# PantoMatrix/PantoMatrix

Hardware: NVIDIA H100
Metric: motion_frames_per_sec (higher is better)
Workload: dtype fp16x3 (two fp16 operand planes, 3 products, f32 accumulate)

## Files before the change

### include/pm_emage.h

```cpp
#ifndef PM_EMAGE_H
#define PM_EMAGE_H
#include <stdint.h>
#ifdef __cplusplus
extern "C" {
#endif

#define PM_ABI_VERSION 6
#define PM_FMT_F16 0x100
#define PM_TC_TILE_SHIFT 16
#define PM_TC_STORE_LOOP (1 << 24)
int pm_abi_version(void);
int pm_memset_async(void* ptr, int value, long long bytes, void* stream);
int pm_device_cc(void);

int pm_tapgemm_f32(const float* A, long long a_bs, int lda, int batch, int rows_in, int cin,
                   const float* W, const float* bias, int taps, int stride, int pad,
                   int rows_out, int cout,
                   const float* residual, long long r_bs, int ldr,
                   int act, float slope,
                   float* out, long long o_bs, int ldo, void* stream);

int pm_tapgemm_tc(const uint16_t* A, long long a_ps, long long a_bs, int lda, int batch, int rows_in, int cin,
                  const uint16_t* W, long long w_ps, int w_rows, int ldw, int taps, int pad, int nsplit,
                  const float* bias, int rows_out, int cout,
                  const float* residual, long long r_bs, int ldr,
                  int act, int act_cols, float slope, float acc_scale,
                  float* out_f32, long long o_bs, int ldo,
                  uint16_t* out_bf16, long long ob_ps, long long ob_bs, int ldob, int out_nsplit,
                  const void* prefetch, long long prefetch_bytes, void* stream);

int pm_split_bf16(const float* x, long long x_bs, int ldx, int batch, int rows, int ch,
                  uint16_t* out, long long o_ps, long long o_bs, int ldo, int nsplit, void* stream);

int pm_wav_stem_f32(const float* audio, long long a_bs, long long a_ws, int batch, int windows, int n_samples,
                    const float* w1, const float* b1, const float* wd, const float* bd, int cout,
                    int ksize, int stride, int pad, int rows_out, float slope,
                    float* y1, float* sc,
                    uint16_t* planes, long long p_ps, int p_ld, int p_nsplit, void* stream);

int pm_add_layernorm_f32(const float* x, const float* r, const float* gamma, const float* beta,
                         float* out, long long rows, int ch, float eps,
                         uint16_t* planes, long long p_ps, int p_ld, int p_nsplit, void* stream);

int pm_attention_f32(const float* Q, int ldq, const float* K, int ldk, const float* V, int ldv,
                     float* O, int ldo, int batch, int heads, int tq, int tk, int head_dim,
                     uint16_t* planes, long long p_ps, int p_ld, int p_nsplit, void* stream);

int pm_attention_tc(const uint16_t* Q, long long q_ps, long long q_bs, int ldq, int q_cols, int q_col0,
                    const uint16_t* K, long long k_ps, long long k_bs, int ldk, int k_cols, int k_col0,
                    const uint16_t* V, long long v_ps, long long v_bs, int ldv, int v_cols, int v_col0,
                    float* O, int ldo, int batch, int heads, int tq, int tk, int head_dim,
                    uint16_t* planes, long long p_ps, int p_ld, int p_nsplit, void* stream);

int pm_add_rows_f32(const float* x, const float* pe, const float* spk, int first, int second,
                    float* out, int batch, int rows, int ch,
                    uint16_t* planes, long long p_ps, int p_ld, int p_nsplit, void* stream);
int pm_add2_f32(const float* a, long long lda, const float* b, long long ldb, float* out, long long ldo,
                long long rows, long long ch,
                uint16_t* planes, long long p_ps, int p_ld, int p_nsplit, void* stream);

int pm_window_input_f32(const float* motion, const float* mask, const float* seed, const float* mask_embedding,
                        float* out, int batch, int total_len, int start, int win_len, int pre, int ch, long long seed_bs,
                        uint16_t* planes, long long p_ps, int p_ld, int p_nsplit, void* stream);

int pm_l2_argmin_f32(const float* z, long long rows, int rows_per_batch, long long z_bs,
                     const float* codebook, const float* e2, int n_codes, int e_dim, long long* index, void* stream);
int pm_l2_argmin_tc(const float* z, long long rows, int rows_per_batch, long long z_bs,
                    const float* codebook, const float* e2, int n_codes, int e_dim, long long* index, int max_ctas,
                    void* stream);
int pm_l2_argmin_simt_f32(const float* z, long long rows, int rows_per_batch, long long z_bs,
                          const float* codebook, const float* e2, int n_codes, int e_dim, long long* index, void* stream);
int pm_row_argmax_f32(const float* x, long long rows, int ch, int ldx, int rows_per_batch, long long x_bs,
                      long long* index, int* nonfinite, void* stream);
int pm_gather_rows_f32(const float* codebook, long long n_table, const long long* index, long long rows, int ch,
                       float* out, uint16_t* planes, long long p_ps, int p_ld, int p_nsplit, void* stream);
int pm_row_sqnorm_f32(const float* x, int rows, int ch, float* out, void* stream);

int pm_pose_compose_f32(const float* face, const float* upper, const float* hands, const float* lower,
                        float* expression, float* axis_angle, float* motion4inf, long long bt, void* stream);

int pm_global_trans_f32(const float* rec, int ld, int vel_off, const float* ref_trans, int ref_bs, float dt,
                        float* trans, int batch, int t, void* stream);

int pm_resample_poly_f32(const void* pcm, int is_int16, long long in_bs, int batch, long long n_in, int channels,
                         const float* bank, int up, int down, int taps, long long n_pre_remove,
                         float* out, long long out_bs, void* stream);

int pm_lstm_bidir_f32(const float* xproj, long long x_bs, int ldx, const float* whh,
                      float* y, long long y_bs, int ldy, unsigned int* barrier,
                      int batch, int t, int hidden, void* stream);
int pm_lstm_cond_f32(const float* spk, long long n_spk, int spk_dim, const long long* speaker_id,
                     const float* seed, long long seed_bs, int seed_ld, int seed_len, int seed_frames, int pose_dims,
                     float* out, long long o_bs, int ldo, int batch, int t, void* stream);
int pm_rot6d_to_aa_f32(const float* rot6d, long long rows, int n_sel, const int* slot, float* out, void* stream);
int pm_softmax2_mix_f32(const float* sel, const float* c1, const float* c2, float* out, long long rows, int ch, int ldo,
                        void* stream);

int pm_smplx_fk_f32(const float* poses, long long pose_bs, long long pose_ts,
                    const float* betas, long long b_bs,
                    const float* expr, long long e_bs, long long e_ts,
                    const float* transl, long long t_bs, long long t_ts,
                    long long joint_mask, int batch, int t,
                    const float* j_template, const float* j_dirs, const float* pose_mean,
                    const int* parents, const int* level_order, const int* level_start, int n_levels,
                    float* joints, float* rel_transforms, float* feat, int ld_feat,
                    uint16_t* planes, long long p_ps, int p_ld, int p_nsplit, void* stream);
int pm_smplx_skin_f32(float* verts, long long ld, long long rows, int n_verts,
                      const int* row_ptr, const int* col, const float* val, const float* rel_transforms,
                      const float* transl, long long t_bs, long long t_ts, int t, void* stream);
int pm_motion_rep_f32(const float* poses, long long pose_bs, long long pose_ts, const float* joints,
                      int batch, int t, float dt, float two_dt, float* rep15d, void* stream);

int pm_mesh_vertex_f32(const float* verts0, long long v0_fs, const float* verts1, long long v1_fs,
                       int n_verts, int frames, float scale0, float ox0, float oy0, float oz0,
                       float scale1, float ox1, float oy1, float oz1, const int* faces,
                       const int* vf_ptr, const int* vf_face, int* xy, float* depth, float* normal,
                       int views, void* stream);
int pm_mesh_raster(const int* xy, const float* depth, int n_verts, const int* faces, int n_faces,
                   int frames, unsigned long long* vis, int views, void* stream);
int pm_mesh_shade_u8(const unsigned long long* vis, const int* xy, const float* normal, int n_verts,
                     const int* faces, int frames, unsigned char* out, long long out_fs, int views, void* stream);
int pm_time_upsample_f32(const float* x, long long x_bs, long long x_ts, int batch, int t, int channels, int k,
                         float* out, void* stream);

int pm_png_count(const unsigned char* frames, long long f_fs, int n_frames, int h, int w, long long* row_bits,
                 unsigned long long* row_adler, void* stream);
int pm_png_scan(int n_frames, int h, int w, long long* row_bits, const unsigned long long* row_adler,
                unsigned char* data, long long cap, long long* nbytes, void* stream);
int pm_png_emit(const unsigned char* frames, long long f_fs, int n_frames, int h, int w, const long long* row_off,
                unsigned char* data, long long cap, void* stream);
int pm_png_crc(int n_frames, int h, int w, unsigned char* data, long long cap, const long long* nbytes, void* stream);

int pm_h264_encode(const unsigned char* frames, long long f_fs, int n_frames, int clip_len, int h, int w, int qp,
                   unsigned char* scratch, long long slice_cap, int* slice_bytes, void* stream);
int pm_h264_encode_gop(const unsigned char* frames, long long f_fs, int n_frames, int clip_len, int h, int w, int qp,
                       unsigned char* scratch, long long slice_cap, int* slice_bytes, int gop, unsigned char* recon,
                       long long recon_stride, void* stream);
int pm_h264_encode_me(const unsigned char* frames, long long f_fs, int n_frames, int clip_len, int h, int w, int qp,
                      unsigned char* scratch, long long slice_cap, int* slice_bytes, int gop, unsigned char* recon,
                      long long recon_stride, int search, short* mv, long long mv_len, void* stream);
int pm_h264_gather(int n_frames, int h, int w, const unsigned char* scratch, long long slice_cap,
                   const int* slice_bytes, unsigned char* data, long long cap, long long* nbytes, void* stream);

int pm_flac_analyse(const void* pcm, long long clip_stride, int batch, int n, int channels, int bps, int* rec,
                    void* stream);
int pm_flac_emit(const void* pcm, long long clip_stride, int batch, int n, int channels, int bps, int rate,
                 const int* rec, unsigned char* data, long long cap, long long* nbytes, void* stream);

#ifdef __cplusplus
}
#endif
#endif
```

### pantomatrix_b200/_lib.py

```python
from __future__ import annotations

import ctypes as C
import os

_HERE = os.path.dirname(os.path.abspath(__file__))
LIB_PATH = os.environ.get("PM_EMAGE_LIB") or os.path.join(_HERE, "libpm_emage.so")

_p = C.c_void_p
_i = C.c_int
_ll = C.c_longlong
_f = C.c_float

SIGNATURES = {
    "pm_abi_version": [],
    "pm_device_cc": [],
    "pm_tapgemm_f32": [_p, _ll, _i, _i, _i, _i, _p, _p, _i, _i, _i, _i, _i, _p, _ll, _i, _i, _f, _p, _ll, _i, _p],
    "pm_tapgemm_tc": [_p, _ll, _ll, _i, _i, _i, _i, _p, _ll, _i, _i, _i, _i, _i, _p, _i, _i, _p, _ll, _i,
                      _i, _i, _f, _f, _p, _ll, _i, _p, _ll, _ll, _i, _i, _p, _ll, _p],
    "pm_split_bf16": [_p, _ll, _i, _i, _i, _i, _p, _ll, _ll, _i, _i, _p],
    "pm_wav_stem_f32": [_p, _ll, _ll, _i, _i, _i, _p, _p, _p, _p, _i, _i, _i, _i, _i, _f, _p, _p, _p, _ll, _i, _i, _p],
    "pm_add_layernorm_f32": [_p, _p, _p, _p, _p, _ll, _i, _f, _p, _ll, _i, _i, _p],
    "pm_attention_f32": [_p, _i, _p, _i, _p, _i, _p, _i, _i, _i, _i, _i, _i, _p, _ll, _i, _i, _p],
    "pm_attention_tc": [_p, _ll, _ll, _i, _i, _i, _p, _ll, _ll, _i, _i, _i, _p, _ll, _ll, _i, _i, _i,
                        _p, _i, _i, _i, _i, _i, _i, _p, _ll, _i, _i, _p],
    "pm_add_rows_f32": [_p, _p, _p, _i, _i, _p, _i, _i, _i, _p, _ll, _i, _i, _p],
    "pm_add2_f32": [_p, _ll, _p, _ll, _p, _ll, _ll, _ll, _p, _ll, _i, _i, _p],
    "pm_window_input_f32": [_p, _p, _p, _p, _p, _i, _i, _i, _i, _i, _i, _ll, _p, _ll, _i, _i, _p],
    "pm_l2_argmin_f32": [_p, _ll, _i, _ll, _p, _p, _i, _i, _p, _p],
    "pm_row_argmax_f32": [_p, _ll, _i, _i, _i, _ll, _p, _p, _p],
    "pm_l2_argmin_tc": [_p, _ll, _i, _ll, _p, _p, _i, _i, _p, _i, _p],
    "pm_l2_argmin_simt_f32": [_p, _ll, _i, _ll, _p, _p, _i, _i, _p, _p],
    "pm_memset_async": [_p, _i, _ll, _p],
    "pm_gather_rows_f32": [_p, _ll, _p, _ll, _i, _p, _p, _ll, _i, _i, _p],
    "pm_row_sqnorm_f32": [_p, _i, _i, _p, _p],
    "pm_pose_compose_f32": [_p, _p, _p, _p, _p, _p, _p, _ll, _p],
    "pm_global_trans_f32": [_p, _i, _i, _p, _i, _f, _p, _i, _i, _p],
    "pm_lstm_bidir_f32": [_p, _ll, _i, _p, _p, _ll, _i, _p, _i, _i, _i, _p],
    "pm_lstm_cond_f32": [_p, _ll, _i, _p, _p, _ll, _i, _i, _i, _i, _p, _ll, _i, _i, _i, _p],
    "pm_rot6d_to_aa_f32": [_p, _ll, _i, _p, _p, _p],
    "pm_softmax2_mix_f32": [_p, _p, _p, _p, _ll, _i, _i, _p],
    "pm_resample_poly_f32": [_p, _i, _ll, _i, _ll, _i, _p, _i, _i, _i, _ll, _p, _ll, _p],
    "pm_smplx_fk_f32": [_p, _ll, _ll, _p, _ll, _p, _ll, _ll, _p, _ll, _ll, _ll, _i, _i, _p, _p, _p, _p, _p, _p, _i,
                        _p, _p, _p, _i, _p, _ll, _i, _i, _p],
    "pm_smplx_skin_f32": [_p, _ll, _ll, _i, _p, _p, _p, _p, _p, _ll, _ll, _i, _p],
    "pm_motion_rep_f32": [_p, _ll, _ll, _p, _i, _i, _f, _f, _p, _p],
    "pm_mesh_vertex_f32": [_p, _ll, _p, _ll, _i, _i, _f, _f, _f, _f, _f, _f, _f, _f, _p, _p, _p, _p, _p, _p, _i, _p],
    "pm_mesh_raster": [_p, _p, _i, _p, _i, _i, _p, _i, _p],
    "pm_mesh_shade_u8": [_p, _p, _p, _i, _p, _i, _p, _ll, _i, _p],
    "pm_time_upsample_f32": [_p, _ll, _ll, _i, _i, _i, _i, _p, _p],
    "pm_png_count": [_p, _ll, _i, _i, _i, _p, _p, _p],
    "pm_png_scan": [_i, _i, _i, _p, _p, _p, _ll, _p, _p],
    "pm_png_emit": [_p, _ll, _i, _i, _i, _p, _p, _ll, _p],
    "pm_png_crc": [_i, _i, _i, _p, _ll, _p, _p],
    "pm_h264_encode": [_p, _ll, _i, _i, _i, _i, _i, _p, _ll, _p, _p],
    "pm_h264_encode_gop": [_p, _ll, _i, _i, _i, _i, _i, _p, _ll, _p, _i, _p, _ll, _p],
    "pm_h264_encode_me": [_p, _ll, _i, _i, _i, _i, _i, _p, _ll, _p, _i, _p, _ll, _i, _p, _ll, _p],
    "pm_h264_gather": [_i, _i, _i, _p, _ll, _p, _p, _ll, _p, _p],
    "pm_flac_analyse": [_p, _ll, _i, _i, _i, _i, _p, _p],
    "pm_flac_emit": [_p, _ll, _i, _i, _i, _i, _i, _p, _p, _ll, _p, _p],
}

_lib = None


class PmError(RuntimeError):
    pass


def load() -> C.CDLL:
    global _lib
    if _lib is None:
        if not os.path.exists(LIB_PATH):
            raise PmError(
                f"{LIB_PATH} not found: build it with `python -m pantomatrix_b200.build` "
                "(there is no CPU or PyTorch fallback for the EMAGE hot path)")
        lib = C.CDLL(LIB_PATH)
        for name, args in SIGNATURES.items():
            fn = getattr(lib, name)
            fn.argtypes = args
            fn.restype = C.c_int
        _lib = lib
    return _lib


def call(name: str, *args) -> None:
    rc = getattr(load(), name)(*args)
    if rc != 0:
        kind = "bad argument / unsupported shape" if rc < 0 else "cudaError"
        raise PmError(f"{name} failed: {kind} {rc}")
```

### pantomatrix_b200/csrc/pm_attention_tc.cu

```cuda
#include "pm_common.cuh"
#include "pm_tc_ptx.cuh"
#include "../../include/pm_emage.h"

namespace {

constexpr int T = 64;
constexpr int HD = 192;
constexpr int KB = HD / 64;
constexpr int BLK = T * 128;
constexpr int NTHREADS = 128;
constexpr float P_SCALE = 1024.f;

struct Smem {
  static constexpr int Q = 0;
  static constexpr int K = Q + 2 * KB * BLK;
  static constexpr int V = K + 2 * KB * BLK;
  static constexpr int P = V + 2 * KB * BLK;
  static constexpr int BARS = P + 2 * BLK;
  static constexpr int TOTAL = BARS + (KB + 1) * 8;
};

#ifdef PM_ATTN_TIMING
__device__ unsigned long long pm_attn_stamps[16];
#define AT_STAMP(i) do { if (blockIdx.x == 0 && (threadIdx.x & 31) == 0) pm_attn_stamps[i] = (unsigned long long)clock64(); } while (0)
#else
#define AT_STAMP(i) do {} while (0)
#endif

struct AttnParams {
  int heads, tq, tk;
  int qc0, kc0, vc0;
  float scale;
  float* out; int ldo;
  PmPlanes planes;
};

__global__ void __launch_bounds__(NTHREADS, 1) attention_tc_kernel(const __grid_constant__ CUtensorMap map_q,
                                                                   const __grid_constant__ CUtensorMap map_k,
                                                                   const __grid_constant__ CUtensorMap map_v,
                                                                   const AttnParams p) {
  extern __shared__ __align__(1024) uint8_t smem_raw[];
  uint8_t* sm = reinterpret_cast<uint8_t*>((reinterpret_cast<uintptr_t>(smem_raw) + 1023) & ~uintptr_t(1023));
  const uint32_t sm_u = smem_u32(sm);
  const uint32_t bars = sm_u + Smem::BARS;
  const uint32_t qk_full = bars, v_full = bars + 8 * KB;
  const int warp = threadIdx.x >> 5, lane = threadIdx.x & 31;
  const int b = blockIdx.x / p.heads, h = blockIdx.x % p.heads;
  if (warp == 0) AT_STAMP(0);

  if (threadIdx.x == 0) {
    for (int kb = 0; kb < KB; ++kb) mbar_init(qk_full + 8 * kb, 1);
    mbar_init(v_full, 1);
    asm volatile("fence.mbarrier_init.release.cluster;" ::: "memory");
  }
  __syncthreads();
  if (warp == 0) AT_STAMP(1);
  if (warp == 0) {
    if (elect_one()) {
      asm volatile("prefetch.tensormap [%0];" ::"l"(&map_q) : "memory");
      asm volatile("prefetch.tensormap [%0];" ::"l"(&map_k) : "memory");
      asm volatile("prefetch.tensormap [%0];" ::"l"(&map_v) : "memory");
      for (int kb = 0; kb < KB; ++kb) {
        mbar_expect_tx(qk_full + 8 * kb, 4 * BLK);
        for (int pl = 0; pl < 2; ++pl) {
          tma_load_4d(sm_u + Smem::Q + (pl * KB + kb) * BLK, &map_q, qk_full + 8 * kb, p.qc0 + h * HD + kb * 64, 0, b, pl);
          tma_load_4d(sm_u + Smem::K + (pl * KB + kb) * BLK, &map_k, qk_full + 8 * kb, p.kc0 + h * HD + kb * 64, 0, b, pl);
        }
      }
      mbar_expect_tx(v_full, 2 * KB * BLK);
      for (int pl = 0; pl < 2; ++pl)
        for (int nb = 0; nb < KB; ++nb)
          tma_load_4d(sm_u + Smem::V + (pl * KB + nb) * BLK, &map_v, v_full, p.vc0 + h * HD + nb * 64, 0, b, pl);
    }
    __syncwarp();
  }

  const int r0 = warp * 16 + (lane >> 2), t2 = 2 * (lane & 3);
  const int pa[3] = {0, 1, 0}, pb[3] = {1, 0, 0};

  float sr[32];
#pragma unroll
  for (int i = 0; i < 32; ++i) sr[i] = 0.f;
#pragma unroll
  for (int kb = 0; kb < KB; ++kb) {
    mbar_wait(qk_full + 8 * kb, 0);
    if (warp == 0) AT_STAMP(8 + kb);
    wgmma_fence();
#pragma unroll
    for (int t = 0; t < 3; ++t)
#pragma unroll
      for (int k = 0; k < 4; ++k)
        wgmma_m64n64k16<false>(sr, gmma_desc(GMMA_DESC_K_SW128, sm_u + Smem::Q + (pa[t] * KB + kb) * BLK + 32 * k),
                               gmma_desc(GMMA_DESC_K_SW128, sm_u + Smem::K + (pb[t] * KB + kb) * BLK + 32 * k));
    wgmma_commit();
  }
  wgmma_wait<0>();
  wgmma_fence_regs(sr);
  if (warp == 0) AT_STAMP(2);

  float inv[2];
  {
    const float sl2 = p.scale * 1.4426950408889634f;
#pragma unroll
    for (int hr = 0; hr < 2; ++hr) {
      float m = -INFINITY;
#pragma unroll
      for (int i = 0; i < 8; ++i)
#pragma unroll
        for (int u = 0; u < 2; ++u) {
          const int j = 8 * i + t2 + u;
          const float v = j < p.tk ? sr[4 * i + 2 * hr + u] * sl2 : -INFINITY;
          sr[4 * i + 2 * hr + u] = v;
          m = fmaxf(m, v);
        }
      m = fmaxf(m, __shfl_xor_sync(0xffffffffu, m, 1));
      m = fmaxf(m, __shfl_xor_sync(0xffffffffu, m, 2));
      float sum = 0.f;
#pragma unroll
      for (int i = 0; i < 8; ++i)
#pragma unroll
        for (int u = 0; u < 2; ++u) {
          const int j = 8 * i + t2 + u;
          float e = 0.f;
          if (j < p.tk) asm("ex2.approx.ftz.f32 %0, %1;" : "=f"(e) : "f"(sr[4 * i + 2 * hr + u] - m));
          sum += e;
          sr[4 * i + 2 * hr + u] = e * P_SCALE;
        }
      sum += __shfl_xor_sync(0xffffffffu, sum, 1);
      sum += __shfl_xor_sync(0xffffffffu, sum, 2);
      inv[hr] = 1.f / (sum * (P_SCALE * PM_F16_ACT_SCALE));
    }
#pragma unroll
    for (int hr = 0; hr < 2; ++hr) {
      const int row = r0 + 8 * hr;
      const uint32_t dst = sm_u + Smem::P + (row >> 3) * 1024 + (row & 7) * 128;
#pragma unroll
      for (int i = 0; i < 8; ++i) {
        const float a0 = sr[4 * i + 2 * hr], a1 = sr[4 * i + 2 * hr + 1];
        const float f0 = pm_f16_head(a0), f1 = pm_f16_head(a1);
        const __half2 h0 = __floats2half2_rn(f0, f1);
        const __half2 h1 = __floats2half2_rn(a0 - f0, a1 - f1);
        const uint32_t off = (uint32_t)(((i ^ (row & 7)) << 4) + 2 * t2);
        asm volatile("st.shared.b32 [%0], %1;" ::"r"(dst + off), "r"(*reinterpret_cast<const uint32_t*>(&h0)) : "memory");
        asm volatile("st.shared.b32 [%0], %1;" ::"r"(dst + BLK + off), "r"(*reinterpret_cast<const uint32_t*>(&h1)) : "memory");
      }
    }
    fence_proxy_async_smem();
    __syncthreads();
    if (warp == 0) AT_STAMP(3);
  }

  float orr[96];
#pragma unroll
  for (int i = 0; i < 96; ++i) orr[i] = 0.f;
  mbar_wait(v_full, 0);
  wgmma_fence();
  {
    constexpr uint64_t DESC_MN = gmma_desc_mn_sw128(BLK);
#pragma unroll
    for (int t = 0; t < 3; ++t)
#pragma unroll
      for (int k = 0; k < 4; ++k)
        wgmma_m64n192k16<false, 1>(orr, gmma_desc(GMMA_DESC_K_SW128, sm_u + Smem::P + pa[t] * BLK + 32 * k),
                                   gmma_desc(DESC_MN, sm_u + Smem::V + pb[t] * KB * BLK + 2048 * k));
  }
  wgmma_commit();
  wgmma_wait<0>();
  wgmma_fence_regs(orr);
  if (warp == 0) AT_STAMP(4);

  const bool pair_ok = p.planes.ptr && ((p.planes.ld & 1) == 0) && ((p.planes.ps & 1) == 0) &&
                       ((reinterpret_cast<uintptr_t>(p.planes.ptr) & 3) == 0);
#pragma unroll
  for (int hr = 0; hr < 2; ++hr) {
    const int row = r0 + 8 * hr;
    if (row >= p.tq) continue;
    const long long grow = (long long)b * p.tq + row;
    __half* const prow = reinterpret_cast<__half*>(p.planes.ptr) + grow * p.planes.ld + h * HD;
    float* const frow = p.out ? p.out + grow * p.ldo + h * HD : nullptr;
#pragma unroll
    for (int i = 0; i < HD / 8; ++i) {
      const int c = 8 * i + t2;
      const float x0 = orr[4 * i + 2 * hr] * inv[hr], x1 = orr[4 * i + 2 * hr + 1] * inv[hr];
      if (frow) *reinterpret_cast<float2*>(frow + c) = make_float2(x0, x1);
      if (p.planes.ptr) {
        if (pair_ok) {
          const float a0 = x0 * PM_F16_ACT_SCALE, a1 = x1 * PM_F16_ACT_SCALE;
          const bool two = p.planes.nsplit > 1;
          const float f0 = two ? pm_f16_head(a0) : a0, f1 = two ? pm_f16_head(a1) : a1;
          *reinterpret_cast<__half2*>(prow + c) = __floats2half2_rn(f0, f1);
          if (two) *reinterpret_cast<__half2*>(prow + p.planes.ps + c) = __floats2half2_rn(a0 - f0, a1 - f1);
        } else {
          pm_store_planes_t<true>(p.planes, grow, h * HD + c, x0);
          pm_store_planes_t<true>(p.planes, grow, h * HD + c + 1, x1);
        }
      }
    }
  }
  if (warp == 0) AT_STAMP(5);
#ifdef PM_ATTN_TIMING
  __syncthreads();
#endif
  if (warp == 0) AT_STAMP(7);
}

constexpr size_t kSmem = Smem::TOTAL + 1024;

bool plane_map(CUtensorMap* m, const uint16_t* base, long long ps, long long bs, int ld, int cols, int rows, int batch) {
  cuuint64_t dims[4] = {(cuuint64_t)cols, (cuuint64_t)rows, (cuuint64_t)batch, 2};
  cuuint64_t strides[3] = {(cuuint64_t)ld * 2, (cuuint64_t)bs * 2, (cuuint64_t)ps * 2};
  cuuint32_t box[4] = {64, (cuuint32_t)T, 1, 1};
  return encode_map(m, base, 4, dims, strides, box, true);
}

}

extern "C" int pm_attention_tc(const uint16_t* Q, long long q_ps, long long q_bs, int ldq, int q_cols, int q_col0,
                               const uint16_t* K, long long k_ps, long long k_bs, int ldk, int k_cols, int k_col0,
                               const uint16_t* V, long long v_ps, long long v_bs, int ldv, int v_cols, int v_col0,
                               float* O, int ldo, int batch, int heads, int tq, int tk, int head_dim,
                               uint16_t* planes, long long p_ps, int p_ld, int p_nsplit, void* stream) {
  PM_REQUIRE(Q && K && V && (O || planes) && batch >= 0 && heads > 0);
  PM_TAKE_FMT(p_nsplit, f16);
  PM_REQUIRE(!planes || (f16 && p_nsplit <= 2));
  PM_REQUIRE(pm_planes_ok(planes, p_ps, p_ld, p_nsplit, heads * head_dim, false));
  if (head_dim != HD || tq > T || tk > T || tq <= 0 || tk <= 0) return PM_EUNSUPPORTED;
  PM_REQUIRE(!O || (ldo & 3) == 0);
  for (const void* ptr : {(const void*)Q, (const void*)K, (const void*)V}) PM_REQUIRE((reinterpret_cast<uintptr_t>(ptr) & 15) == 0);
  PM_REQUIRE((ldq & 7) == 0 && (ldk & 7) == 0 && (ldv & 7) == 0 && (q_ps & 7) == 0 && (k_ps & 7) == 0 && (v_ps & 7) == 0);
  PM_REQUIRE(batch <= 1 || ((q_bs & 7) == 0 && (k_bs & 7) == 0 && (v_bs & 7) == 0));
  PM_REQUIRE(q_col0 >= 0 && k_col0 >= 0 && v_col0 >= 0 && q_col0 + heads * HD <= q_cols && k_col0 + heads * HD <= k_cols &&
             v_col0 + heads * HD <= v_cols && q_cols <= ldq && k_cols <= ldk && v_cols <= ldv);
  if (batch == 0) return PM_OK;
  CUtensorMap mq, mk, mv;
  if (!plane_map(&mq, Q, q_ps, q_bs, ldq, q_cols, tq, batch) || !plane_map(&mk, K, k_ps, k_bs, ldk, k_cols, tk, batch) ||
      !plane_map(&mv, V, v_ps, v_bs, ldv, v_cols, tk, batch))
    return PM_EBADARG;
  AttnParams p;
  p.heads = heads; p.tq = tq; p.tk = tk; p.qc0 = q_col0; p.kc0 = k_col0; p.vc0 = v_col0;
  p.scale = 1.0f / (sqrtf((float)head_dim) * PM_F16_ACT_SCALE * PM_F16_ACT_SCALE);
  p.out = O; p.ldo = ldo;
  p.planes = PmPlanes{reinterpret_cast<__nv_bfloat16*>(planes), p_ps, p_ld, p_nsplit};
  static unsigned long long configured = 0;
  if (pm_first_use_on_device(configured)) {
    cudaError_t e = cudaFuncSetAttribute(attention_tc_kernel, cudaFuncAttributeMaxDynamicSharedMemorySize, (int)kSmem);
    if (e != cudaSuccess) { configured = 0; return (int)e; }
  }
  attention_tc_kernel<<<batch * heads, NTHREADS, kSmem, (cudaStream_t)stream>>>(mq, mk, mv, p);
  PM_LAUNCH_CHECK();
}

#ifdef PM_ATTN_TIMING
extern "C" int pm_attn_timing_read(unsigned long long* host) {
  cudaError_t e = cudaDeviceSynchronize();
  if (e != cudaSuccess) return (int)e;
  return (int)cudaMemcpyFromSymbol(host, pm_attn_stamps, sizeof(unsigned long long) * 16);
}
#endif
```

### pantomatrix_b200/csrc/pm_audio.cu

```cuda
#include "pm_common.cuh"
#include "../../include/pm_emage.h"

namespace {

constexpr int kThreads = 256;
constexpr int kMaxStage = 16384;
constexpr long long kTileOutputs = 4096;

template <bool I16, int C>
__device__ __forceinline__ float pm_mix(const void* clip, long long i, int channels) {
  if constexpr (C > 0) channels = C;
  const long long e = i * channels;
  auto at = [&](int c) -> float {
    if constexpr (I16) return (float)__ldg(reinterpret_cast<const int16_t*>(clip) + e + c) * (1.0f / 32768.0f);
    else return __ldg(reinterpret_cast<const float*>(clip) + e + c);
  };
  if constexpr (C == 1) return __fadd_rn(0.0f, at(0));
  if constexpr (C == 2) return __fmul_rn(__fadd_rn(__fadd_rn(0.0f, at(0)), at(1)), 0.5f);
  if (channels == 1) return __fadd_rn(0.0f, at(0));
  float s;
  if (channels == 8) {
    s = __fadd_rn(__fadd_rn(__fadd_rn(at(0), at(1)), __fadd_rn(at(2), at(3))),
                  __fadd_rn(__fadd_rn(at(4), at(5)), __fadd_rn(at(6), at(7))));
    s = __fadd_rn(0.0f, s);
  } else {
    s = 0.0f;
    for (int c = 0; c < channels; ++c) s = __fadd_rn(s, at(c));
  }
  return __fdiv_rn(s, (float)channels);
}

template <bool I16, int C = 0>
__device__ __forceinline__ float pm_mix_or_zero(const void* clip, long long i, long long n_in, int channels) {
  return (i >= 0 && i < n_in) ? pm_mix<I16, C>(clip, i, channels) : 0.0f;
}

constexpr int kStageUnroll = 8;
template <bool I16, int C>
__device__ __forceinline__ void pm_stage(float* stage, const void* clip, long long lo, long long hi, long long n_in,
                                         int channels) {
  for (long long base = lo + threadIdx.x; base <= hi; base += (long long)kThreads * kStageUnroll) {
    float v[kStageUnroll];
#pragma unroll
    for (int u = 0; u < kStageUnroll; ++u) v[u] = pm_mix_or_zero<I16, C>(clip, base + u * kThreads, n_in, channels);
#pragma unroll
    for (int u = 0; u < kStageUnroll; ++u)
      if (base + u * kThreads <= hi) stage[base + u * kThreads - lo] = v[u];
  }
}

template <bool I16, bool STAGED>
__global__ void __launch_bounds__(kThreads)
resample_poly_kernel(const void* __restrict__ pcm, long long in_bs, long long n_in, int channels,
                     const float* __restrict__ bank, int up, int down, int taps, long long n_pre_remove,
                     float* __restrict__ out, long long out_bs, long long n_out, int rows) {
  extern __shared__ float stage[];
  const int b = blockIdx.y;
  const void* clip = I16 ? (const void*)(reinterpret_cast<const int16_t*>(pcm) + b * in_bs)
                         : (const void*)(reinterpret_cast<const float*>(pcm) + b * in_bs);
  float* y = out + b * out_bs;
  const long long m0 = (long long)blockIdx.x * up * rows;
  const long long m_end = min(m0 + (long long)up * rows, n_out);
  const long long lo = (m0 + n_pre_remove) * down / up - (taps - 1);
  const long long hi = (m_end - 1 + n_pre_remove) * down / up;
  if constexpr (STAGED) {
    if (channels == 1) pm_stage<I16, 1>(stage, clip, lo, hi, n_in, channels);
    else if (channels == 2) pm_stage<I16, 2>(stage, clip, lo, hi, n_in, channels);
    else pm_stage<I16, 0>(stage, clip, lo, hi, n_in, channels);
    __syncthreads();
  }
  const int lane = threadIdx.x & 31, warp = threadIdx.x >> 5;
  const int groups = (rows + 31) >> 5;
  for (int unit = warp; unit < up * groups; unit += kThreads / 32) {
    const int r = unit / groups;
    const int g = (unit - r * groups) * 32 + lane;
    const long long m = m0 + r + (long long)up * g;
    if (g >= rows || m >= m_end) continue;
    const long long t = (m + n_pre_remove) * down;
    const long long q = t / up;
    const float* h = bank + (t - q * up) * taps;
    float acc = 0.0f;
    if constexpr (STAGED) {
      const float* x = stage + (q - lo);
#pragma unroll 4
      for (int j = taps - 1; j >= 0; --j) acc = fmaf(__ldg(h + j), x[-j], acc);
    } else {
      for (int j = taps - 1; j >= 0; --j) acc = fmaf(__ldg(h + j), pm_mix_or_zero<I16>(clip, q - j, n_in, channels), acc);
    }
    y[m] = acc;
  }
}

template <bool I16, bool STAGED>
int launch(const void* pcm, long long in_bs, int batch, long long n_in, int channels, const float* bank, int up,
           int down, int taps, long long n_pre_remove, float* out, long long out_bs, long long n_out, int rows,
           size_t smem, cudaStream_t st) {
  static unsigned long long configured = 0;
  auto kern = resample_poly_kernel<I16, STAGED>;
  if (STAGED && pm_first_use_on_device(configured)) {
    const cudaError_t e = cudaFuncSetAttribute(kern, cudaFuncAttributeMaxDynamicSharedMemorySize, kMaxStage * 4);
    if (e != cudaSuccess) return (int)e;
  }
  const long long tiles = (n_out + (long long)up * rows - 1) / ((long long)up * rows);
  kern<<<dim3((unsigned)tiles, (unsigned)batch), kThreads, smem, st>>>(pcm, in_bs, n_in, channels, bank, up, down, taps,
                                                                       n_pre_remove, out, out_bs, n_out, rows);
  PM_LAUNCH_CHECK();
}

}

extern "C" int pm_resample_poly_f32(const void* pcm, int is_int16, long long in_bs, int batch, long long n_in,
                                    int channels, const float* bank, int up, int down, int taps,
                                    long long n_pre_remove, float* out, long long out_bs, void* stream) {
  if (channels < 1 || channels > 8) return PM_EUNSUPPORTED;
  PM_REQUIRE(batch >= 0 && batch <= 65535 && n_in >= 0);
  PM_REQUIRE(up >= 1 && down >= 1 && taps >= 1 && n_pre_remove >= 0);
  PM_REQUIRE(is_int16 == 0 || is_int16 == 1);
  if (n_in == 0 || batch == 0) return PM_OK;
  PM_REQUIRE(pcm && bank && out);
  const long long n_out = (n_in * up + down - 1) / down;
  PM_REQUIRE(batch <= 1 || (in_bs >= n_in * channels && out_bs >= n_out));
  long long rows = (kTileOutputs + up - 1) / up;
  rows = (rows + 31) / 32 * 32;
  const auto span = [&](long long g) { return g * down + taps + 1; };
  while (rows > 32 && span(rows) > kMaxStage) rows -= 32;
  while (rows > 1 && span(rows) > kMaxStage) --rows;
  const bool staged = span(rows) <= kMaxStage;
  if (!staged) rows = 32;
  PM_REQUIRE((n_out + (long long)up * rows - 1) / ((long long)up * rows) <= 0x7fffffffLL);
  const size_t smem = staged ? (size_t)span(rows) * sizeof(float) : 0;
  cudaStream_t st = (cudaStream_t)stream;
  const int r = (int)rows;
  if (is_int16) {
    return staged ? launch<true, true>(pcm, in_bs, batch, n_in, channels, bank, up, down, taps, n_pre_remove, out, out_bs, n_out, r, smem, st)
                  : launch<true, false>(pcm, in_bs, batch, n_in, channels, bank, up, down, taps, n_pre_remove, out, out_bs, n_out, r, smem, st);
  }
  return staged ? launch<false, true>(pcm, in_bs, batch, n_in, channels, bank, up, down, taps, n_pre_remove, out, out_bs, n_out, r, smem, st)
                : launch<false, false>(pcm, in_bs, batch, n_in, channels, bank, up, down, taps, n_pre_remove, out, out_bs, n_out, r, smem, st);
}
```

### pantomatrix_b200/csrc/pm_common.cuh

```cuda
#pragma once
#include <cuda_bf16.h>
#include <cuda_fp16.h>
#include <cuda_runtime.h>
#include <stdint.h>

#define PM_OK 0
#define PM_EBADARG (-1)
#define PM_EUNSUPPORTED (-2)

#define PM_LAUNCH_CHECK()                                  \
  do {                                                     \
    cudaError_t _e = cudaGetLastError();                   \
    return _e == cudaSuccess ? PM_OK : (int)_e;            \
  } while (0)

#define PM_REQUIRE(cond) \
  do {                   \
    if (!(cond)) return PM_EBADARG; \
  } while (0)

static inline int pm_cdiv(long long a, long long b) { return (int)((a + b - 1) / b); }

static inline bool pm_first_use_on_device(unsigned long long& mask) {
  int d = 0;
  if (cudaGetDevice(&d) != cudaSuccess || d < 0 || d >= 64) return true;
  if ((mask >> d) & 1ull) return false;
  mask |= 1ull << d;
  return true;
}

enum PmAct { PM_ACT_NONE = 0, PM_ACT_RELU = 1, PM_ACT_LEAKY = 2 };

__device__ __forceinline__ float pm_act(float v, int act, float slope) {
  if (act == PM_ACT_RELU) return v > 0.f ? v : 0.f;
  if (act == PM_ACT_LEAKY) return v > 0.f ? v : v * slope;
  return v;
}

__device__ __forceinline__ void pm_put_bits(unsigned* w, long long pos, unsigned v, int nb) {
  if (nb == 0) return;
  const unsigned long long x = (unsigned long long)v << (64 - (int)(pos & 31) - nb);
  atomicOr(w + (pos >> 5), __byte_perm((unsigned)(x >> 32), 0, 0x0123));
  if ((unsigned)x) atomicOr(w + (pos >> 5) + 1, __byte_perm((unsigned)x, 0, 0x0123));
}

__device__ __forceinline__ float pm_warp_sum(float v) {
#pragma unroll
  for (int o = 16; o > 0; o >>= 1) v += __shfl_xor_sync(0xffffffffu, v, o);
  return v;
}

__device__ __forceinline__ float pm_warp_max(float v) {
#pragma unroll
  for (int o = 16; o > 0; o >>= 1) v = fmaxf(v, __shfl_xor_sync(0xffffffffu, v, o));
  return v;
}

struct PmPlanes {
  __nv_bfloat16* ptr;
  long long ps;
  int ld;
  int nsplit;
};

__device__ __forceinline__ void pm_split3(float v, __nv_bfloat16 (&p)[3]) {
  p[0] = __float2bfloat16_rn(v);
  float r = v - __bfloat162float(p[0]);
  p[1] = __float2bfloat16_rn(r);
  r -= __bfloat162float(p[1]);
  p[2] = __float2bfloat16_rn(r);
}

#ifndef PM_FMT_F16
#define PM_FMT_F16 0x100
#endif
#define PM_F16_ACT_SCALE 64.0f
#define PM_TAKE_FMT(nsplit_var, flag_var)                          \
  const bool flag_var = ((nsplit_var) & PM_FMT_F16) != 0;          \
  (nsplit_var) &= 0xff

__device__ __forceinline__ float pm_f16_head(float v) {
  return __uint_as_float((__float_as_uint(v) + 0x00001000u) & 0xFFFFE000u);
}

template <bool F16, int NS = 0>
__device__ __forceinline__ void pm_split_pair_t(float x, float y, int nsplit, uint32_t (&w)[3]) {
  if constexpr (NS > 0) nsplit = NS;
  if constexpr (F16) {
    x = __fmul_rn(x, PM_F16_ACT_SCALE);
    y = __fmul_rn(y, PM_F16_ACT_SCALE);
    if (nsplit == 2) {
      const float fx = pm_f16_head(x), fy = pm_f16_head(y);
      const __half2 a = __floats2half2_rn(fx, fy), b = __floats2half2_rn(x - fx, y - fy);
      w[0] = *reinterpret_cast<const uint32_t*>(&a);
      w[1] = *reinterpret_cast<const uint32_t*>(&b);
      return;
    }
#pragma unroll
    for (int pl = 0; pl < 3; ++pl) {
      if (pl < nsplit) {
        const __half2 h = __floats2half2_rn(x, y);
        w[pl] = *reinterpret_cast<const uint32_t*>(&h);
        x -= __low2float(h); y -= __high2float(h);
      }
    }
  } else {
#pragma unroll
    for (int pl = 0; pl < 3; ++pl) {
      if (pl < nsplit) {
        const __nv_bfloat162 h = __floats2bfloat162_rn(x, y);
        w[pl] = *reinterpret_cast<const uint32_t*>(&h);
        x -= __low2float(h); y -= __high2float(h);
      }
    }
  }
}

template <bool F16>
__device__ __forceinline__ void pm_store_planes_t(const PmPlanes& P, long long row, int c, float v) {
  uint16_t* o = reinterpret_cast<uint16_t*>(P.ptr) + row * P.ld + c;
  uint32_t w[3];
  pm_split_pair_t<F16>(v, 0.f, P.nsplit, w);
#pragma unroll
  for (int pl = 0; pl < 3; ++pl)
    if (pl < P.nsplit) o[(long long)pl * P.ps] = (uint16_t)w[pl];
}
__device__ __forceinline__ void pm_store_planes(const PmPlanes& P, long long row, int c, float v) {
  pm_store_planes_t<false>(P, row, c, v);
}

template <bool F16>
__device__ __forceinline__ void pm_store_planes4_t(const PmPlanes& P, long long row, int c, float4 v) {
  __nv_bfloat16* o = P.ptr + row * P.ld + c;
  uint32_t lo[3], hi[3];
  pm_split_pair_t<F16>(v.x, v.y, P.nsplit, lo);
  pm_split_pair_t<F16>(v.z, v.w, P.nsplit, hi);
#pragma unroll
  for (int pl = 0; pl < 3; ++pl)
    if (pl < P.nsplit) *reinterpret_cast<uint2*>(o + (long long)pl * P.ps) = make_uint2(lo[pl], hi[pl]);
}
__device__ __forceinline__ void pm_store_planes4(const PmPlanes& P, long long row, int c, float4 v) {
  pm_store_planes4_t<false>(P, row, c, v);
}

static inline bool pm_planes_ok(const void* ptr, long long ps, int ld, int nsplit, int ch, bool vec4) {
  if (!ptr) return true;
  if (nsplit < 1 || nsplit > 3 || ld < ch) return false;
  if (vec4 && ((ld & 3) || (ps & 3) || (reinterpret_cast<uintptr_t>(ptr) & 7))) return false;
  return true;
}
```

### pantomatrix_b200/csrc/pm_elementwise.cu

```cuda
#include "pm_common.cuh"
#include "../../include/pm_emage.h"

namespace {

constexpr int STEM_ROWS = 192;
constexpr int STEM_THREADS = 256;

template <bool F16>
__device__ __forceinline__ void stem_store_planes2(const PmPlanes& P, long long row, int c, float a, float b) {
  if constexpr (F16) {
    if (P.nsplit == 2) {
      __half* o = reinterpret_cast<__half*>(P.ptr) + row * P.ld + c;
      a *= PM_F16_ACT_SCALE; b *= PM_F16_ACT_SCALE;
      const float a0 = pm_f16_head(a), b0 = pm_f16_head(b);
      *reinterpret_cast<__half2*>(o) = __floats2half2_rn(a0, b0);
      *reinterpret_cast<__half2*>(o + P.ps) = __floats2half2_rn(a - a0, b - b0);
      return;
    }
  }
  pm_store_planes_t<F16>(P, row, c, a);
  pm_store_planes_t<F16>(P, row, c + 1, b);
}

template <int KS, int COUT, bool F16>
__global__ void __launch_bounds__(STEM_THREADS, 2) wav_stem_kernel(
    const float* __restrict__ audio, long long a_bs, long long a_ws, int batch, int n_samples,
    const float* __restrict__ w1, const float* __restrict__ b1, const float* __restrict__ wd,
    const float* __restrict__ bd, int stride, int pad, int rows_out, float slope,
    float* __restrict__ y1, float* __restrict__ sc, const PmPlanes P) {
  extern __shared__ float sx[];
  constexpr int LPR = COUT / 2;
  constexpr int RW = 32 / LPR;
  constexpr int RPI = 3 * RW * (STEM_THREADS / 32);
  static_assert(STEM_ROWS % RPI == 0, "tile must be whole iterations");
  const int seq = blockIdx.y;
  const int w = seq / batch, b = seq % batch;
  const float* __restrict__ x = audio + (long long)b * a_bs + (long long)w * a_ws;
  const int l0 = blockIdx.x * STEM_ROWS;
  const int span = (STEM_ROWS - 1) * stride + KS;
  for (int i = threadIdx.x; i < span; i += STEM_THREADS) {
    const int s = l0 * stride - pad + i;
    sx[i] = (s >= 0 && s < n_samples) ? x[s] : 0.f;
  }
  const int lane = threadIdx.x & 31, warp = threadIdx.x >> 5;
  const int cp = lane % LPR, rs = lane / LPR;
  const int c0 = 2 * cp;
  float wa0[KS], wa1[KS], wb0[KS], wb1[KS];
#pragma unroll
  for (int k = 0; k < KS; ++k) {
    wa0[k] = __ldg(w1 + c0 * KS + k);
    wa1[k] = __ldg(w1 + (c0 + 1) * KS + k);
    wb0[k] = __ldg(wd + c0 * KS + k);
    wb1[k] = __ldg(wd + (c0 + 1) * KS + k);
  }
  const float ba0 = __ldg(b1 + c0), ba1 = __ldg(b1 + c0 + 1), bb0 = __ldg(bd + c0), bb1 = __ldg(bd + c0 + 1);
  __syncthreads();
#pragma unroll 1
  for (int it = 0; it < STEM_ROWS / RPI; ++it) {
    const int r0 = (it * (STEM_THREADS / 32) + warp) * 3 * RW + rs * 3;
    if (l0 + r0 >= rows_out) continue;
    const float* xr = sx + r0 * stride;
    float acc[3][4];
#pragma unroll
    for (int j = 0; j < 3; ++j) acc[j][0] = acc[j][1] = acc[j][2] = acc[j][3] = 0.f;
    if (stride == 5) {
      float xv[2 * 5 + KS];
#pragma unroll
      for (int i = 0; i < 2 * 5 + KS; ++i) xv[i] = xr[i];
#pragma unroll
      for (int j = 0; j < 3; ++j) {
#pragma unroll
        for (int k = 0; k < KS; ++k) {
          const float v = xv[5 * j + k];
          acc[j][0] = fmaf(v, wa0[k], acc[j][0]);
          acc[j][1] = fmaf(v, wa1[k], acc[j][1]);
          acc[j][2] = fmaf(v, wb0[k], acc[j][2]);
          acc[j][3] = fmaf(v, wb1[k], acc[j][3]);
        }
      }
    } else {
#pragma unroll
      for (int j = 0; j < 3; ++j) {
#pragma unroll
        for (int k = 0; k < KS; ++k) {
          const float v = xr[j * stride + k];
          acc[j][0] = fmaf(v, wa0[k], acc[j][0]);
          acc[j][1] = fmaf(v, wa1[k], acc[j][1]);
          acc[j][2] = fmaf(v, wb0[k], acc[j][2]);
          acc[j][3] = fmaf(v, wb1[k], acc[j][3]);
        }
      }
    }
#pragma unroll
    for (int j = 0; j < 3; ++j) {
      const int l = l0 + r0 + j;
      if (l >= rows_out) break;
      float a0 = acc[j][0] + ba0, a1 = acc[j][1] + ba1;
      a0 = a0 > 0.f ? a0 : a0 * slope;
      a1 = a1 > 0.f ? a1 : a1 * slope;
      const long long row = (long long)seq * rows_out + l;
      *reinterpret_cast<float2*>(sc + row * COUT + c0) = make_float2(acc[j][2] + bb0, acc[j][3] + bb1);
      if (y1) *reinterpret_cast<float2*>(y1 + row * COUT + c0) = make_float2(a0, a1);
      if (P.ptr) stem_store_planes2<F16>(P, row, c0, a0, a1);
    }
  }
}

template <int VEC, bool F16>
__global__ void __launch_bounds__(256) add_layernorm_kernel(
    const float* __restrict__ x, const float* __restrict__ r, const float* __restrict__ gamma,
    const float* __restrict__ beta, float* __restrict__ out, long long rows, float eps, PmPlanes P) {
  const int lane = threadIdx.x & 31;
  const long long row = (long long)blockIdx.x * (blockDim.x >> 5) + (threadIdx.x >> 5);
  if (row >= rows) return;
  constexpr int CH = VEC * 128;
  const float4* __restrict__ xr = reinterpret_cast<const float4*>(x + row * CH);
  const float4* __restrict__ rr = r ? reinterpret_cast<const float4*>(r + row * CH) : nullptr;
  float4 v[VEC];
  float s = 0.f;
#pragma unroll
  for (int i = 0; i < VEC; ++i) {
    v[i] = xr[lane + 32 * i];
    if (rr) {
      const float4 t = rr[lane + 32 * i];
      v[i].x += t.x; v[i].y += t.y; v[i].z += t.z; v[i].w += t.w;
    }
    s += (v[i].x + v[i].y) + (v[i].z + v[i].w);
  }
  const float mean = pm_warp_sum(s) * (1.f / CH);
  float q = 0.f;
#pragma unroll
  for (int i = 0; i < VEC; ++i) {
    const float a = v[i].x - mean, b = v[i].y - mean, c = v[i].z - mean, d = v[i].w - mean;
    q += (a * a + b * b) + (c * c + d * d);
  }
  const float rstd = rsqrtf(pm_warp_sum(q) * (1.f / CH) + eps);
  const float4* __restrict__ g4 = reinterpret_cast<const float4*>(gamma);
  const float4* __restrict__ b4 = reinterpret_cast<const float4*>(beta);
  float4* __restrict__ o4 = out ? reinterpret_cast<float4*>(out + row * CH) : nullptr;
#pragma unroll
  for (int i = 0; i < VEC; ++i) {
    const float4 g = g4[lane + 32 * i], bb = b4[lane + 32 * i];
    float4 o;
    o.x = (v[i].x - mean) * rstd * g.x + bb.x;
    o.y = (v[i].y - mean) * rstd * g.y + bb.y;
    o.z = (v[i].z - mean) * rstd * g.z + bb.z;
    o.w = (v[i].w - mean) * rstd * g.w + bb.w;
    if (o4) o4[lane + 32 * i] = o;
    if (P.ptr) pm_store_planes4_t<F16>(P, row, (lane + 32 * i) * 4, o);
  }
}

__device__ __forceinline__ float4 pick_row(int code, const float* pe, const float* spk, int b, int t, int ch, int c4) {
  if (code == 1) return reinterpret_cast<const float4*>(pe + (long long)t * ch)[c4];
  if (code == 2) return reinterpret_cast<const float4*>(spk + (long long)b * ch)[c4];
  return make_float4(0.f, 0.f, 0.f, 0.f);
}

template <bool F16>
__global__ void __launch_bounds__(256) add_rows_kernel(
    const float* __restrict__ x, const float* __restrict__ pe, const float* __restrict__ spk,
    int first, int second, float* __restrict__ out, int batch, int rows, int ch, PmPlanes P) {
  const int ch4 = ch >> 2;
  const long long total = (long long)batch * rows * ch4;
  for (long long i = (long long)blockIdx.x * blockDim.x + threadIdx.x; i < total;
       i += (long long)gridDim.x * blockDim.x) {
    const int c4 = (int)(i % ch4);
    const long long bt = i / ch4;
    const int t = (int)(bt % rows), b = (int)(bt / rows);
    float4 v = x ? reinterpret_cast<const float4*>(x)[i] : make_float4(0.f, 0.f, 0.f, 0.f);
    if (first) {
      const float4 a = pick_row(first, pe, spk, b, t, ch, c4);
      v.x += a.x; v.y += a.y; v.z += a.z; v.w += a.w;
    }
    if (second) {
      const float4 a = pick_row(second, pe, spk, b, t, ch, c4);
      v.x += a.x; v.y += a.y; v.z += a.z; v.w += a.w;
    }
    if (out) reinterpret_cast<float4*>(out)[i] = v;
    if (P.ptr) pm_store_planes4_t<F16>(P, bt, c4 * 4, v);
  }
}

template <bool F16>
__global__ void __launch_bounds__(256) add2_kernel(const float* __restrict__ a, long long lda,
                                                   const float* __restrict__ b, long long ldb,
                                                   float* __restrict__ out, long long ldo, long long rows,
                                                   long long ch, long long nv, PmPlanes P) {
  const long long i0 = (long long)blockIdx.x * blockDim.x + threadIdx.x, step = (long long)gridDim.x * blockDim.x;
  for (long long i = i0; i < rows * nv; i += step) {
    const long long r = rows == 1 ? 0 : i / nv, c = (i - r * nv) * 4;
    const float4 u = *reinterpret_cast<const float4*>(a + r * lda + c);
    const float4 v = *reinterpret_cast<const float4*>(b + r * ldb + c);
    const float4 o = make_float4(u.x + v.x, u.y + v.y, u.z + v.z, u.w + v.w);
    if (out) *reinterpret_cast<float4*>(out + r * ldo + c) = o;
    if (P.ptr) pm_store_planes4_t<F16>(P, r, (int)c, o);
  }
  const long long nt = ch - 4 * nv;
  for (long long i = i0; i < rows * nt; i += step) {
    const long long r = i / nt, c = 4 * nv + (i - r * nt);
    const float o = a[r * lda + c] + b[r * ldb + c];
    if (out) out[r * ldo + c] = o;
    if (P.ptr) pm_store_planes_t<F16>(P, r, (int)c, o);
  }
}

template <bool F16>
__global__ void __launch_bounds__(256) window_input_kernel(
    const float* __restrict__ motion, const float* __restrict__ mask, const float* __restrict__ seed,
    const float* __restrict__ mask_embedding, float* __restrict__ out,
    int batch, int total_len, int start, int win_len, int pre, int ch, long long seed_bs, PmPlanes P) {
  const long long total = (long long)batch * win_len * ch;
  for (long long i = (long long)blockIdx.x * blockDim.x + threadIdx.x; i < total;
       i += (long long)gridDim.x * blockDim.x) {
    const int c = (int)(i % ch);
    const long long bf = i / ch;
    const int f = (int)(bf % win_len), b = (int)(bf / win_len);
    const long long src = ((long long)b * total_len + start + f) * ch + c;
    float m = mask ? mask[src] : 1.f;
    float v = motion ? motion[src] : ((c < ch - 7 && (c % 6 == 0 || c % 6 == 4)) ? 1.f : 0.f);
    if (f < pre) {
      if (m != 0.f && seed) v = seed[(long long)b * seed_bs + (long long)f * ch + c];
      m = 0.f;
    }
    const float o = (m == 1.f) ? mask_embedding[c] : v;
    if (out) out[i] = o;
    if (P.ptr) pm_store_planes_t<F16>(P, bf, c, o);
  }
}

inline int grid_for(long long work, int threads) {
  long long g = (work + threads - 1) / threads;
  const long long cap = 148LL * 16;
  return (int)(g < 1 ? 1 : (g > cap ? cap : g));
}

}

extern "C" int pm_wav_stem_f32(const float* audio, long long a_bs, long long a_ws, int batch, int windows,
                               int n_samples, const float* w1, const float* b1, const float* wd,
                               const float* bd, int cout, int ksize, int stride, int pad, int rows_out,
                               float slope, float* y1, float* sc,
                               uint16_t* planes, long long p_ps, int p_ld, int p_nsplit, void* stream) {
  PM_REQUIRE(audio && w1 && b1 && wd && bd && sc && (y1 || planes));
  PM_REQUIRE(batch > 0 && windows > 0 && n_samples > 0 && cout > 0 && stride > 0 && rows_out > 0);
  PM_TAKE_FMT(p_nsplit, f16);
  PM_REQUIRE(pm_planes_ok(planes, p_ps, p_ld, p_nsplit, cout, false));
  PM_REQUIRE(!planes || ((p_ld & 1) == 0 && (p_ps & 1) == 0 && (reinterpret_cast<uintptr_t>(planes) & 3) == 0));
  PM_REQUIRE((reinterpret_cast<uintptr_t>(sc) & 7) == 0 && (!y1 || (reinterpret_cast<uintptr_t>(y1) & 7) == 0));
  if (ksize != 15 || (cout != 32 && cout != 64)) return PM_EUNSUPPORTED;
  PM_REQUIRE((long long)batch * windows <= 65535);
  const size_t smem = (size_t)((STEM_ROWS - 1) * stride + ksize) * sizeof(float);
  PM_REQUIRE(smem <= 48 * 1024);
  const PmPlanes P{reinterpret_cast<__nv_bfloat16*>(planes), p_ps, p_ld, planes ? p_nsplit : 0};
  dim3 grid(pm_cdiv(rows_out, STEM_ROWS), batch * windows);
  cudaStream_t st = (cudaStream_t)stream;
#define PM_STEM(CO, F)                                                                                          \
  wav_stem_kernel<15, CO, F><<<grid, STEM_THREADS, smem, st>>>(audio, a_bs, a_ws, batch, n_samples, w1, b1, wd, bd, \
                                                               stride, pad, rows_out, slope, y1, sc, P)
  if (cout == 64) { if (f16) PM_STEM(64, true); else PM_STEM(64, false); }
  else { if (f16) PM_STEM(32, true); else PM_STEM(32, false); }
#undef PM_STEM
  PM_LAUNCH_CHECK();
}

extern "C" int pm_add_layernorm_f32(const float* x, const float* r, const float* gamma, const float* beta,
                                    float* out, long long rows, int ch, float eps,
                                    uint16_t* planes, long long p_ps, int p_ld, int p_nsplit, void* stream) {
  PM_REQUIRE(x && gamma && beta && (out || planes) && rows >= 0);
  PM_TAKE_FMT(p_nsplit, f16);
  PM_REQUIRE(pm_planes_ok(planes, p_ps, p_ld, p_nsplit, ch, true));
  const PmPlanes P{reinterpret_cast<__nv_bfloat16*>(planes), p_ps, p_ld, p_nsplit};
  if (rows == 0) return PM_OK;
  const int warps = 8;
  const unsigned grid = (unsigned)((rows + warps - 1) / warps);
  cudaStream_t st = (cudaStream_t)stream;
  switch (ch) {
    case 256:
      if (f16) add_layernorm_kernel<2, true><<<grid, warps * 32, 0, st>>>(x, r, gamma, beta, out, rows, eps, P);
      else add_layernorm_kernel<2, false><<<grid, warps * 32, 0, st>>>(x, r, gamma, beta, out, rows, eps, P);
      break;
    case 512:
      if (f16) add_layernorm_kernel<4, true><<<grid, warps * 32, 0, st>>>(x, r, gamma, beta, out, rows, eps, P);
      else add_layernorm_kernel<4, false><<<grid, warps * 32, 0, st>>>(x, r, gamma, beta, out, rows, eps, P);
      break;
    case 768:
      if (f16) add_layernorm_kernel<6, true><<<grid, warps * 32, 0, st>>>(x, r, gamma, beta, out, rows, eps, P);
      else add_layernorm_kernel<6, false><<<grid, warps * 32, 0, st>>>(x, r, gamma, beta, out, rows, eps, P);
      break;
    case 1024:
      if (f16) add_layernorm_kernel<8, true><<<grid, warps * 32, 0, st>>>(x, r, gamma, beta, out, rows, eps, P);
      else add_layernorm_kernel<8, false><<<grid, warps * 32, 0, st>>>(x, r, gamma, beta, out, rows, eps, P);
      break;
    default: return PM_EUNSUPPORTED;
  }
  PM_LAUNCH_CHECK();
}

extern "C" int pm_add_rows_f32(const float* x, const float* pe, const float* spk, int first, int second,
                               float* out, int batch, int rows, int ch,
                               uint16_t* planes, long long p_ps, int p_ld, int p_nsplit, void* stream) {
  PM_REQUIRE((out || planes) && batch >= 0 && rows >= 0 && ch > 0 && (ch & 3) == 0);
  PM_TAKE_FMT(p_nsplit, f16);
  PM_REQUIRE(pm_planes_ok(planes, p_ps, p_ld, p_nsplit, ch, true));
  const PmPlanes P{reinterpret_cast<__nv_bfloat16*>(planes), p_ps, p_ld, p_nsplit};
  PM_REQUIRE(first >= 0 && first <= 2 && second >= 0 && second <= 2);
  PM_REQUIRE((first != 1 && second != 1) || pe);
  PM_REQUIRE((first != 2 && second != 2) || spk);
  const long long total = (long long)batch * rows * (ch >> 2);
  if (total == 0) return PM_OK;
  if (f16) add_rows_kernel<true><<<grid_for(total, 256), 256, 0, (cudaStream_t)stream>>>(x, pe, spk, first, second, out,
                                                                                  batch, rows, ch, P);
  else add_rows_kernel<false><<<grid_for(total, 256), 256, 0, (cudaStream_t)stream>>>(x, pe, spk, first, second, out,
                                                                               batch, rows, ch, P);
  PM_LAUNCH_CHECK();
}

extern "C" int pm_add2_f32(const float* a, long long lda, const float* b, long long ldb, float* out, long long ldo,
                           long long rows, long long ch,
                           uint16_t* planes, long long p_ps, int p_ld, int p_nsplit, void* stream) {
  PM_REQUIRE(a && b && (out || planes) && rows >= 0 && ch > 0);
  PM_REQUIRE(rows <= 1 || (lda >= ch && ldb >= ch && (!out || ldo >= ch)));
  PM_REQUIRE(!planes || ((ch & 3) == 0 && ch <= 0x7fffffffLL));
  PM_TAKE_FMT(p_nsplit, f16);
  PM_REQUIRE(pm_planes_ok(planes, p_ps, p_ld, p_nsplit, (int)(planes ? ch : 1), true));
  const PmPlanes P{reinterpret_cast<__nv_bfloat16*>(planes), p_ps, p_ld, p_nsplit};
  if (rows == 0) return PM_OK;
  const auto a16 = [](const void* p) { return (reinterpret_cast<uintptr_t>(p) & 15) == 0; };
  const bool vec = a16(a) && a16(b) && (!out || a16(out)) &&
                   (rows == 1 || ((lda & 3) == 0 && (ldb & 3) == 0 && (!out || (ldo & 3) == 0)));
  const long long nv = vec ? ch / 4 : 0;
  const int grid = grid_for(rows * (nv + (ch - 4 * nv)), 256);
  cudaStream_t st = (cudaStream_t)stream;
  if (f16) add2_kernel<true><<<grid, 256, 0, st>>>(a, lda, b, ldb, out, ldo, rows, ch, nv, P);
  else add2_kernel<false><<<grid, 256, 0, st>>>(a, lda, b, ldb, out, ldo, rows, ch, nv, P);
  PM_LAUNCH_CHECK();
}

extern "C" int pm_window_input_f32(const float* motion, const float* mask, const float* seed,
                                   const float* mask_embedding, float* out, int batch, int total_len,
                                   int start, int win_len, int pre, int ch, long long seed_bs,
                                   uint16_t* planes, long long p_ps, int p_ld, int p_nsplit, void* stream) {
  PM_REQUIRE(mask_embedding && (out || planes));
  PM_TAKE_FMT(p_nsplit, f16);
  PM_REQUIRE(pm_planes_ok(planes, p_ps, p_ld, p_nsplit, ch, false));
  const PmPlanes P{reinterpret_cast<__nv_bfloat16*>(planes), p_ps, p_ld, p_nsplit};
  PM_REQUIRE(batch >= 0 && win_len >= 0 && start >= 0 && start + win_len <= total_len && pre >= 0 && ch > 0);
  const long long total = (long long)batch * win_len * ch;
  if (total == 0) return PM_OK;
  if (f16) window_input_kernel<true><<<grid_for(total, 256), 256, 0, (cudaStream_t)stream>>>(
      motion, mask, seed, mask_embedding, out, batch, total_len, start, win_len, pre, ch, seed_bs, P);
  else window_input_kernel<false><<<grid_for(total, 256), 256, 0, (cudaStream_t)stream>>>(
      motion, mask, seed, mask_embedding, out, batch, total_len, start, win_len, pre, ch, seed_bs, P);
  PM_LAUNCH_CHECK();
}
```

### pantomatrix_b200/csrc/pm_misc.cu

```cuda
#include "pm_common.cuh"
#include "../../include/pm_emage.h"

extern "C" int pm_abi_version(void) { return PM_ABI_VERSION; }

extern "C" int pm_memset_async(void* ptr, int value, long long bytes, void* stream) {
  PM_REQUIRE(ptr && bytes >= 0);
  if (bytes == 0) return PM_OK;
  const cudaError_t e = cudaMemsetAsync(ptr, value, (size_t)bytes, (cudaStream_t)stream);
  return e == cudaSuccess ? PM_OK : (int)e;
}

extern "C" int pm_device_cc(void) {
  int dev = 0, major = 0, minor = 0;
  if (cudaGetDevice(&dev) != cudaSuccess) return -1;
  if (cudaDeviceGetAttribute(&major, cudaDevAttrComputeCapabilityMajor, dev) != cudaSuccess) return -1;
  if (cudaDeviceGetAttribute(&minor, cudaDevAttrComputeCapabilityMinor, dev) != cudaSuccess) return -1;
  return major * 10 + minor;
}
```

### pantomatrix_b200/csrc/pm_pose.cu

```cuda
#include "pm_common.cuh"
#include "../../include/pm_emage.h"

namespace {

__constant__ int8_t kJointPart[55] = {
    1, 1, 1, 0, 1, 1, 0, 1, 1, 0, 1, 1, 0, 0, 0, 0, 0, 0, 0, 0, 0, 0, 3, 4, 4,
    2, 2, 2, 2, 2, 2, 2, 2, 2, 2, 2, 2, 2, 2, 2, 2, 2, 2, 2, 2, 2, 2, 2, 2, 2, 2, 2, 2, 2, 2};
__constant__ int8_t kJointSlot[55] = {
    0, 1, 2, 0, 3, 4, 1, 5, 6, 2, 7, 8, 3, 4, 5, 6, 7, 8, 9, 10, 11, 12, 0, 0, 0,
    0, 1, 2, 3, 4, 5, 6, 7, 8, 9, 10, 11, 12, 13, 14, 15, 16, 17, 18, 19, 20, 21, 22, 23, 24, 25, 26, 27, 28, 29};

__device__ __forceinline__ float sqrt_pos(float x) { return x > 0.f ? sqrtf(x) : 0.f; }
__device__ __forceinline__ float sign_like(float a, float b) { return ((a < 0.f) != (b < 0.f)) ? -a : a; }

__device__ __forceinline__ float sin_half_over_angle(float half, float ang) {
  return fabsf(ang) < 1e-6f ? 0.5f - (ang * ang) / 48.f : sinf(half) / ang;
}

__device__ void rot6d_to_aa(const float d[6], float aa[3]) {
  float n1 = fmaxf(sqrtf(d[0] * d[0] + d[1] * d[1] + d[2] * d[2]), 1e-12f);
  const float b1x = d[0] / n1, b1y = d[1] / n1, b1z = d[2] / n1;
  const float dot = b1x * d[3] + b1y * d[4] + b1z * d[5];
  float b2x = d[3] - dot * b1x, b2y = d[4] - dot * b1y, b2z = d[5] - dot * b1z;
  float n2 = fmaxf(sqrtf(b2x * b2x + b2y * b2y + b2z * b2z), 1e-12f);
  b2x /= n2; b2y /= n2; b2z /= n2;
  const float b3x = b1y * b2z - b1z * b2y;
  const float b3y = b1z * b2x - b1x * b2z;
  const float b3z = b1x * b2y - b1y * b2x;
  const float m00 = b1x, m11 = b2y, m22 = b3z;
  const float w = 0.5f * sqrt_pos(1.f + m00 + m11 + m22);
  float x = 0.5f * sqrt_pos(1.f + m00 - m11 - m22);
  float y = 0.5f * sqrt_pos(1.f - m00 + m11 - m22);
  float z = 0.5f * sqrt_pos(1.f - m00 - m11 + m22);
  x = sign_like(x, b3y - b2z);
  y = sign_like(y, b1z - b3x);
  z = sign_like(z, b2x - b1y);
  const float n = sqrtf(x * x + y * y + z * z);
  const float half = atan2f(n, w);
  const float ang = 2.f * half;
  const float s = sin_half_over_angle(half, ang);
  aa[0] = x / s; aa[1] = y / s; aa[2] = z / s;
}

__device__ void aa_to_rot6d(const float aa[3], float o[6]) {
  const float ang = sqrtf(aa[0] * aa[0] + aa[1] * aa[1] + aa[2] * aa[2]);
  const float half = 0.5f * ang;
  const float s = sin_half_over_angle(half, ang);
  const float r = cosf(half), i = aa[0] * s, j = aa[1] * s, k = aa[2] * s;
  const float two_s = 2.0f / (r * r + i * i + j * j + k * k);
  o[0] = 1.f - two_s * (j * j + k * k);
  o[1] = two_s * (i * j - k * r);
  o[2] = two_s * (i * k + j * r);
  o[3] = two_s * (i * j + k * r);
  o[4] = 1.f - two_s * (i * i + k * k);
  o[5] = two_s * (j * k - i * r);
}

__global__ void __launch_bounds__(256) pose_compose_kernel(
    const float* __restrict__ face, const float* __restrict__ upper, const float* __restrict__ hands,
    const float* __restrict__ lower, float* __restrict__ expression, float* __restrict__ axis_angle,
    float* __restrict__ motion4inf, long long bt) {
  const long long total = bt * 64;
  for (long long i = (long long)blockIdx.x * blockDim.x + threadIdx.x; i < total;
       i += (long long)gridDim.x * blockDim.x) {
    const long long r = i >> 6;
    const int w = (int)(i & 63);
    if (w < 55) {
      const int part = kJointPart[w], slot = kJointSlot[w];
      const float* src = nullptr;
      if (part == 0 && upper) src = upper + r * 78 + slot * 6;
      else if (part == 1 && lower) src = lower + r * 61 + slot * 6;
      else if (part == 2 && hands) src = hands + r * 180 + slot * 6;
      else if (part == 3 && face) src = face + r * 106;
      float aa[3] = {0.f, 0.f, 0.f};
      if (src) {
        float d[6];
#pragma unroll
        for (int c = 0; c < 6; ++c) d[c] = src[c];
        rot6d_to_aa(d, aa);
      }
      float o[6];
      aa_to_rot6d(aa, o);
#pragma unroll
      for (int c = 0; c < 3; ++c) axis_angle[r * 165 + w * 3 + c] = aa[c];
#pragma unroll
      for (int c = 0; c < 6; ++c) motion4inf[r * 337 + w * 6 + c] = o[c];
    } else if (w == 55) {
#pragma unroll
      for (int c = 0; c < 7; ++c) motion4inf[r * 337 + 330 + c] = lower ? lower[r * 61 + 54 + c] : 0.f;
    } else {
      for (int c = w - 56; c < 100; c += 8) expression[r * 100 + c] = face ? face[r * 106 + 6 + c] : 0.f;
    }
  }
}

__global__ void __launch_bounds__(64) global_trans_kernel(const float* __restrict__ rec, int ld, int vel_off,
                                                          const float* __restrict__ ref_trans, int ref_bs, float dt,
                                                          float* __restrict__ trans, int t) {
  const int b = blockIdx.x;
  const float* __restrict__ v = rec + (long long)b * t * ld + vel_off;
  float* __restrict__ o = trans + (long long)b * t * 3;
  if (threadIdx.x < 2) {
    const int ax = threadIdx.x * 2;
    float pos = ref_trans[(long long)b * ref_bs + ax];
    o[ax] = pos;
    for (int i = 1; i < t; ++i) {
      pos = v[(long long)(i - 1) * ld + ax] * dt + pos;
      o[(long long)i * 3 + ax] = pos;
    }
  } else {
    for (int i = threadIdx.x - 2; i < t; i += blockDim.x - 2) o[(long long)i * 3 + 1] = v[(long long)i * ld + 1];
  }
}

__global__ void __launch_bounds__(256) rot6d_to_aa_kernel(const float* __restrict__ rot6d, long long rows, int n_sel,
                                                          const int* __restrict__ slot, float* __restrict__ out) {
  const long long total = rows * 55;
  for (long long i = (long long)blockIdx.x * blockDim.x + threadIdx.x; i < total; i += (long long)gridDim.x * blockDim.x) {
    const long long r = i / 55;
    const int j = (int)(i % 55);
    const int sl = slot[j];
    float aa[3] = {0.f, 0.f, 0.f};
    if (sl >= 0) {
      float d[6];
#pragma unroll
      for (int c = 0; c < 6; ++c) d[c] = rot6d[(r * n_sel + sl) * 6 + c];
      rot6d_to_aa(d, aa);
    }
#pragma unroll
    for (int c = 0; c < 3; ++c) out[r * 165 + j * 3 + c] = aa[c];
  }
}

__global__ void __launch_bounds__(256) softmax2_mix_kernel(const float* __restrict__ sel, const float* __restrict__ c1,
                                                           const float* __restrict__ c2, float* __restrict__ out,
                                                           long long rows, int ch, int ldo) {
  const long long total = rows * ch;
  for (long long i = (long long)blockIdx.x * blockDim.x + threadIdx.x; i < total; i += (long long)gridDim.x * blockDim.x) {
    const long long r = i / ch;
    const int c = (int)(i % ch);
    const float a = sel[2 * r], b = sel[2 * r + 1];
    const float m = fmaxf(a, b);
    const float ea = expf(a - m), eb = expf(b - m);
    const float s = ea + eb;
    out[r * ldo + c] = (ea / s) * c1[i] + (eb / s) * c2[i];
  }
}

__global__ void __launch_bounds__(256) motion_rep_kernel(const float* __restrict__ poses, long long pose_bs,
                                                         long long pose_ts, const float* __restrict__ joints,
                                                         long long rows, int t, float dt, float two_dt,
                                                         float* __restrict__ rep) {
  const long long total = rows * 55;
  for (long long i = (long long)blockIdx.x * blockDim.x + threadIdx.x; i < total; i += (long long)gridDim.x * blockDim.x) {
    const long long r = i / 55;
    const int j = (int)(i % 55);
    const long long b = r / t;
    const int tt = (int)(r % t);
    const int hi = tt + 1 < t ? tt + 1 : tt, lo = tt > 0 ? tt - 1 : tt;
    const float den = (tt == 0 || tt == t - 1) ? dt : two_dt;
    const float* jh = joints + ((b * t + hi) * 55 + j) * 3;
    const float* jl = joints + ((b * t + lo) * 55 + j) * 3;
    const float* p = poses + b * pose_bs + (long long)tt * pose_ts + 3 * j;
    const float* ph = poses + b * pose_bs + (long long)hi * pose_ts + 3 * j;
    const float* pl = poses + b * pose_bs + (long long)lo * pose_ts + 3 * j;
    float* o = rep + r * 825 + j * 15;
    const float aa[3] = {p[0], p[1], p[2]};
    float r6[6];
    aa_to_rot6d(aa, r6);
#pragma unroll
    for (int c = 0; c < 3; ++c) {
      o[c] = joints[(r * 55 + j) * 3 + c];
      o[3 + c] = (jh[c] - jl[c]) / den;
      o[12 + c] = (ph[c] - pl[c]) / den;
    }
#pragma unroll
    for (int c = 0; c < 6; ++c) o[6 + c] = r6[c];
  }
}

}

extern "C" int pm_motion_rep_f32(const float* poses, long long pose_bs, long long pose_ts, const float* joints,
                                 int batch, int t, float dt, float two_dt, float* rep15d, void* stream) {
  PM_REQUIRE(poses && joints && rep15d && batch >= 0 && t >= 2 && dt > 0.f && two_dt > 0.f);
  const long long rows = (long long)batch * t;
  if (rows == 0) return PM_OK;
  long long g = (rows * 55 + 255) / 256;
  if (g > 148 * 16) g = 148 * 16;
  motion_rep_kernel<<<(unsigned)g, 256, 0, (cudaStream_t)stream>>>(poses, pose_bs, pose_ts, joints, rows, t, dt, two_dt,
                                                                  rep15d);
  PM_LAUNCH_CHECK();
}

extern "C" int pm_rot6d_to_aa_f32(const float* rot6d, long long rows, int n_sel, const int* slot, float* out, void* stream) {
  PM_REQUIRE(rot6d && slot && out && rows >= 0 && n_sel > 0 && n_sel <= 55);
  if (rows == 0) return PM_OK;
  long long g = (rows * 55 + 255) / 256;
  if (g > 148 * 16) g = 148 * 16;
  rot6d_to_aa_kernel<<<(unsigned)g, 256, 0, (cudaStream_t)stream>>>(rot6d, rows, n_sel, slot, out);
  PM_LAUNCH_CHECK();
}

extern "C" int pm_softmax2_mix_f32(const float* sel, const float* c1, const float* c2, float* out, long long rows,
                                   int ch, int ldo, void* stream) {
  PM_REQUIRE(sel && c1 && c2 && out && rows >= 0 && ch > 0 && ldo >= ch);
  if (rows == 0) return PM_OK;
  long long g = (rows * ch + 255) / 256;
  if (g > 148 * 16) g = 148 * 16;
  softmax2_mix_kernel<<<(unsigned)g, 256, 0, (cudaStream_t)stream>>>(sel, c1, c2, out, rows, ch, ldo);
  PM_LAUNCH_CHECK();
}

extern "C" int pm_pose_compose_f32(const float* face, const float* upper, const float* hands, const float* lower,
                                   float* expression, float* axis_angle, float* motion4inf, long long bt,
                                   void* stream) {
  PM_REQUIRE(expression && axis_angle && motion4inf && bt >= 0);
  if (bt == 0) return PM_OK;
  long long g = (bt * 64 + 255) / 256;
  if (g > 148 * 16) g = 148 * 16;
  pose_compose_kernel<<<(unsigned)g, 256, 0, (cudaStream_t)stream>>>(face, upper, hands, lower, expression,
                                                                    axis_angle, motion4inf, bt);
  PM_LAUNCH_CHECK();
}

extern "C" int pm_global_trans_f32(const float* rec, int ld, int vel_off, const float* ref_trans, int ref_bs, float dt,
                                   float* trans, int batch, int t, void* stream) {
  PM_REQUIRE(rec && ref_trans && trans && batch >= 0 && t >= 0 && ld >= vel_off + 3 && ref_bs >= 0);
  if (batch == 0 || t == 0) return PM_OK;
  global_trans_kernel<<<batch, 64, 0, (cudaStream_t)stream>>>(rec, ld, vel_off, ref_trans, ref_bs, dt, trans, t);
  PM_LAUNCH_CHECK();
}
```

### pantomatrix_b200/csrc/pm_tapgemm_tc.cu

```cuda
#include <cuda.h>
#include <stdio.h>
#include <stdlib.h>

#include <cstring>
#include <type_traits>
#include "pm_common.cuh"
#include "../../include/pm_emage.h"


namespace {

constexpr int BM = 128;
constexpr int BK = 64;
constexpr int MMA_K = 16;
constexpr int A_TILE_BYTES = BM * BK * 2;
constexpr int PRODUCER_THREADS = 128;
constexpr int CONSUMER_THREADS = 256;
constexpr int NUM_THREADS = PRODUCER_THREADS + CONSUMER_THREADS;
constexpr int PRODUCER_REGS = 40, CONSUMER_REGS = 232;
static_assert(PRODUCER_THREADS * PRODUCER_REGS + CONSUMER_THREADS * CONSUMER_REGS == (65536 / NUM_THREADS & ~7) * NUM_THREADS,
              "the setmaxnreg split must use exactly the launch's register pool");
constexpr int STAMP_WARP = PRODUCER_THREADS / 32;
constexpr int MAX_STAGES = 8;
constexpr int RING_KB = 200;

struct TcParams {
  int taps, pad, nsplit, kblocks;
  int rows_out, cout, batch;
  int R, NB;
  int w_rows;
  const float* bias;
  const float* residual; long long r_bs; int ldr;
  int res_tma;
  int tma_out;
  int act, act_cols; float slope;
  float* out_f32; long long o_bs; int ldo;
  __nv_bfloat16* out_bf16; long long ob_ps, ob_bs; int ldob; int out_nsplit;
  int stages;
  int res_slot0, rot;
  const uint8_t* prefetch; long long prefetch_bytes;
  float acc_scale;
};

#ifdef PM_TC_TIMING
__device__ unsigned long long pm_tc_stamps[4096 * 8];
#define PM_STAMP(i)                                                                                              \
  do {                                                                                                           \
    if ((threadIdx.x & 31) == 0) {                                                                               \
      const unsigned cta_ = (blockIdx.z * gridDim.y + blockIdx.y) * gridDim.x + blockIdx.x;                      \
      if (cta_ < 4096) pm_tc_stamps[cta_ * 8 + (i)] = (unsigned long long)clock64();                             \
    }                                                                                                            \
  } while (0)
#else
#define PM_STAMP(i) do {} while (0)
#endif

#include "pm_tc_ptx.cuh"

template <int BN, bool F16>
__device__ __forceinline__ void mma_k16(float (&d)[BN / 2], uint64_t a, uint64_t b) {
  static_assert(BN == 64 || BN == 128, "64- or 128-column tiles (see pm_tapgemm_tc)");
  if constexpr (BN == 64) wgmma_m64n64k16<!F16>(d, a, b);
  else wgmma_m64n128k16<!F16>(d, a, b);
}

template <int BN, bool F16, int NSPLIT>
__device__ __forceinline__ void mma_kblock(float (&main)[BN / 2], float (&corr)[BN / 2], uint64_t a0, uint64_t w0) {
  constexpr uint64_t A_PL = A_TILE_BYTES >> 4, W_PL = (BN * BK * 2) >> 4, K_ST = (MMA_K * 2) >> 4;
  if constexpr (NSPLIT == 3) {
#pragma unroll
    for (int k = 0; k < BK / MMA_K; ++k) mma_k16<BN, F16>(corr, a0 + k * K_ST, w0 + 2 * W_PL + k * K_ST);
#pragma unroll
    for (int k = 0; k < BK / MMA_K; ++k) mma_k16<BN, F16>(corr, a0 + A_PL + k * K_ST, w0 + W_PL + k * K_ST);
#pragma unroll
    for (int k = 0; k < BK / MMA_K; ++k) mma_k16<BN, F16>(corr, a0 + 2 * A_PL + k * K_ST, w0 + k * K_ST);
  }
  if constexpr (NSPLIT >= 2) {
#pragma unroll
    for (int k = 0; k < BK / MMA_K; ++k) mma_k16<BN, F16>(corr, a0 + k * K_ST, w0 + W_PL + k * K_ST);
#pragma unroll
    for (int k = 0; k < BK / MMA_K; ++k) mma_k16<BN, F16>(corr, a0 + A_PL + k * K_ST, w0 + k * K_ST);
  }
#pragma unroll
  for (int k = 0; k < BK / MMA_K; ++k) mma_k16<BN, F16>(main, a0 + k * K_ST, w0 + k * K_ST);
}

template <int BN, bool F16, int NSPLIT>
__global__ void __launch_bounds__(NUM_THREADS, 1) tapgemm_tc_kernel(const __grid_constant__ CUtensorMap map_a,
                                                                  const __grid_constant__ CUtensorMap map_w,
                                                                  const __grid_constant__ CUtensorMap map_r,
                                                                  const __grid_constant__ CUtensorMap map_o,
                                                                  const __grid_constant__ CUtensorMap map_p,
                                                                  const TcParams p) {
  constexpr int W_TILE_BYTES = BN * BK * 2;
  constexpr int NACC = BN / 2;
  constexpr int ST = BN + 8;
  constexpr int RES_BYTES = BM * BN * 4;

  extern __shared__ __align__(1024) uint8_t smem_raw[];
  uint8_t* tiles = smem_raw + ((1024u - (smem_u32(smem_raw) & 1023u)) & 1023u);
  const int stage_bytes = p.nsplit * (A_TILE_BYTES + W_TILE_BYTES);
  const int ring_bytes = p.stages * stage_bytes > BM * ST * 4 ? p.stages * stage_bytes : BM * ST * 4;
  uint64_t* bars = reinterpret_cast<uint64_t*>(tiles + ring_bytes);
  uint64_t* full_bar = bars;
  uint64_t* empty_bar = bars + MAX_STAGES;
  uint64_t* epi_bar = bars + 2 * MAX_STAGES;
  float* bias_s = reinterpret_cast<float*>(bars + 2 * MAX_STAGES + 2);

  const int warp = threadIdx.x >> 5, lane = threadIdx.x & 31;
  if (warp == STAMP_WARP) PM_STAMP(0);
  const int l0 = blockIdx.x * p.R;
  const int n0 = blockIdx.y * BN;
  const int b0 = blockIdx.z * p.NB;
  const int n_iter = p.taps * p.kblocks;

  if (threadIdx.x == 0) {
    asm volatile("prefetch.tensormap [%0];" ::"l"(&map_a) : "memory");
    asm volatile("prefetch.tensormap [%0];" ::"l"(&map_w) : "memory");
    if (p.res_tma) asm volatile("prefetch.tensormap [%0];" ::"l"(&map_r) : "memory");
    if (p.tma_out && p.out_f32) asm volatile("prefetch.tensormap [%0];" ::"l"(&map_o) : "memory");
    if (p.tma_out && p.out_nsplit) asm volatile("prefetch.tensormap [%0];" ::"l"(&map_p) : "memory");
    for (int s = 0; s < p.stages; ++s) {
      mbar_init(smem_u32(&full_bar[s]), 1);
      mbar_init(smem_u32(&empty_bar[s]), 2);
    }
    mbar_init(smem_u32(epi_bar), p.res_tma ? 2 : 1);
    asm volatile("fence.mbarrier_init.release.cluster;" ::: "memory");
  }
  __syncthreads();
  if (warp == STAMP_WARP) PM_STAMP(1);

  if (warp < PRODUCER_THREADS / 32) {
    setmaxnreg_dec<PRODUCER_REGS>();
    if (warp == 1 && lane == 0 && p.prefetch) {
      const long long ncta = (long long)gridDim.x * gridDim.y * gridDim.z;
      const long long cta = ((long long)blockIdx.z * gridDim.y + blockIdx.y) * gridDim.x + blockIdx.x;
      long long share = ((p.prefetch_bytes + ncta - 1) / ncta + 127) & ~127LL;
      long long off = cta * share;
      long long end = off + share < p.prefetch_bytes ? off + share : p.prefetch_bytes;
      end &= ~15LL;
      for (; off < end; off += 16384) {
        const uint32_t n = (uint32_t)(end - off < 16384 ? end - off : 16384);
        asm volatile("cp.async.bulk.prefetch.L2.global [%0], %1;" ::"l"(p.prefetch + off), "r"(n) : "memory");
      }
    }
    if (warp == 2) {
      for (int c = lane; c < BN; c += 32) bias_s[c] = p.bias && n0 + c < p.cout ? __ldg(p.bias + n0 + c) : 0.f;
      __syncwarp();
      if (lane == 0) mbar_arrive(smem_u32(epi_bar));
    }
    if (warp != 0) return;
    const uint32_t tx = (uint32_t)stage_bytes;
    int s = 0, q = p.rot, tap = 0, kb = 0;
    uint32_t ph = 0;
    for (int it = 0; it < n_iter; ++it) {
      mbar_wait_fast(smem_u32(&empty_bar[s]), ph ^ 1u);
      if (elect_one()) {
        const uint32_t bar = smem_u32(&full_bar[s]);
        uint8_t* st = tiles + (size_t)q * stage_bytes;
        mbar_expect_tx(bar, tx);
        for (int pl = 0; pl < p.nsplit; ++pl) {
          tma_load_4d(smem_u32(st + pl * A_TILE_BYTES), &map_a, bar, kb * BK, l0 + tap - p.pad, b0, pl);
          tma_load_3d(smem_u32(st + p.nsplit * A_TILE_BYTES + pl * W_TILE_BYTES), &map_w, bar, kb * BK, tap * p.w_rows + n0, pl);
        }
      }
      __syncwarp();
      if (++s == p.stages) { s = 0; ph ^= 1u; }
      if (++q == p.stages) q = 0;
      if (++kb == p.kblocks) { kb = 0; ++tap; }
    }
    if (p.res_tma) {
      for (int j = p.res_slot0; j < p.stages; ++j) {
        mbar_wait_fast(smem_u32(&empty_bar[s]), ph ^ 1u);
        if (++s == p.stages) { s = 0; ph ^= 1u; }
      }
      if (elect_one()) {
        const uint32_t bar = smem_u32(epi_bar);
        mbar_expect_tx(bar, (uint32_t)RES_BYTES);
        const int nbox = p.tma_out ? BN / 32 : 1;
        for (int j = 0; j < nbox; ++j)
          tma_load_3d(smem_u32(tiles + ring_bytes - RES_BYTES + j * (RES_BYTES / nbox)), &map_r, bar, n0 + j * (BN / nbox), l0, b0);
      }
      __syncwarp();
    }
    return;
  }

  setmaxnreg_inc<CONSUMER_REGS>();
  const int ct = threadIdx.x - PRODUCER_THREADS;
  const int wg = ct >> 7;
  float acc0[NACC], acc1[NACC], accc[NACC];
#pragma unroll
  for (int i = 0; i < NACC; ++i) { acc0[i] = 0.f; acc1[i] = 0.f; accc[i] = 0.f; }
  {
    const uint32_t tiles_u32 = smem_u32(tiles);
    int s = 0, q = p.rot;
    uint32_t ph = 0;
    int prev = -1;
    auto kblock = [&](float (&main)[NACC]) {
      mbar_wait_fast(smem_u32(&full_bar[s]), ph);
      if (prev < 0 && warp == STAMP_WARP) PM_STAMP(2);
      const uint32_t a_base = tiles_u32 + (uint32_t)q * (uint32_t)stage_bytes + (uint32_t)wg * (64 * 128);
      const uint32_t w_base = tiles_u32 + (uint32_t)q * (uint32_t)stage_bytes + (uint32_t)(NSPLIT * A_TILE_BYTES);
      wgmma_fence();
      mma_kblock<BN, F16, NSPLIT>(main, accc, gmma_desc(GMMA_DESC_K_SW128, a_base), gmma_desc(GMMA_DESC_K_SW128, w_base));
      wgmma_commit();
      wgmma_wait<1>();
      if (prev >= 0 && ct % 128 == 0) mbar_arrive(smem_u32(&empty_bar[prev]));
      prev = s;
      if (++s == p.stages) { s = 0; ph ^= 1u; }
      if (++q == p.stages) q = 0;
    };
    int it = 0;
    for (; it + 1 < n_iter; it += 2) {
      kblock(acc0);
      kblock(acc1);
    }
    if (it < n_iter) kblock(acc0);
    if (warp == STAMP_WARP) PM_STAMP(3);
    wgmma_wait<0>();
    if (warp == STAMP_WARP) PM_STAMP(4);
    wgmma_fence_regs(acc0);
    wgmma_fence_regs(acc1);
    wgmma_fence_regs(accc);
  }
  named_bar_sync(1, CONSUMER_THREADS);
  if (p.tma_out) {
    const int wq = warp & 3, t4 = lane & 3, sw = lane >> 2;
    const int r0 = wg * 64 + wq * 16 + sw;
    const float act_slope = p.act == PM_ACT_NONE ? 1.f : (p.act == PM_ACT_RELU ? 0.f : p.slope);
    const float* res_s = reinterpret_cast<const float*>(tiles + ring_bytes - RES_BYTES);
    auto off32 = [&](int r, int i) { return (i >> 2) * (BM * 32) + r * 32 + (((2 * (i & 3) + (t4 >> 1)) ^ sw) << 2) + 2 * (t4 & 1); };
    mbar_wait_fast(smem_u32(epi_bar), 0);
#pragma unroll
    for (int i = 0; i < NACC / 4; ++i) {
      const int c = 8 * i + 2 * t4, n = n0 + c;
      const float2 bc = *reinterpret_cast<const float2*>(bias_s + c);
#pragma unroll
      for (int h = 0; h < 2; ++h) {
        const int j = 4 * i + 2 * h;
        float v0 = acc0[j] + acc1[j], v1 = acc0[j + 1] + acc1[j + 1];
        v0 += accc[j];
        v1 += accc[j + 1];
        if constexpr (F16) { v0 = __fmul_rn(v0, p.acc_scale); v1 = __fmul_rn(v1, p.acc_scale); }
        if (p.bias) { v0 += bc.x; v1 += bc.y; }
        if (p.residual) {
          const float2 t = *reinterpret_cast<const float2*>(res_s + off32(r0 + 8 * h, i));
          v0 += t.x; v1 += t.y;
        }
        acc0[j] = v0 < 0.f ? (n < p.act_cols ? act_slope : 1.f) * v0 : v0;
        acc0[j + 1] = v1 < 0.f ? (n + 1 < p.act_cols ? act_slope : 1.f) * v1 : v1;
      }
    }
    float* of_s = reinterpret_cast<float*>(tiles);
    uint8_t* pl_s = tiles + (p.out_f32 ? BM * BN * 4 : 0);
    constexpr int PLANE_BYTES = BM * BN * 2;
    if (p.out_f32) {
#pragma unroll
      for (int i = 0; i < NACC / 4; ++i)
#pragma unroll
        for (int h = 0; h < 2; ++h)
          *reinterpret_cast<float2*>(of_s + off32(r0 + 8 * h, i)) = make_float2(acc0[4 * i + 2 * h], acc0[4 * i + 2 * h + 1]);
      fence_proxy_async_smem();
      named_bar_sync(1, CONSUMER_THREADS);
      if (ct == 0) {
        for (int j = 0; j < BN / 32 && n0 + 32 * j < p.cout; ++j)
          tma_store_3d(&map_o, smem_u32(of_s + j * (BM * 32)), n0 + 32 * j, l0, b0);
        bulk_commit();
      }
    }
    auto planes = [&](auto ons) {
      constexpr int ONS = decltype(ons)::value;
#pragma unroll
      for (int i = 0; i < NACC / 4; ++i)
#pragma unroll
        for (int h = 0; h < 2; ++h) {
          uint32_t w[3];
          pm_split_pair_t<F16, ONS>(acc0[4 * i + 2 * h], acc0[4 * i + 2 * h + 1], p.out_nsplit, w);
          const int o = (i >> 3) * (BM * 128) + (r0 + 8 * h) * 128 + (((i & 7) ^ sw) << 4) + 4 * t4;
#pragma unroll
          for (int pl = 0; pl < 3; ++pl)
            if (pl < (ONS ? ONS : p.out_nsplit)) *reinterpret_cast<uint32_t*>(pl_s + pl * PLANE_BYTES + o) = w[pl];
        }
    };
    if (p.out_nsplit) {
      if (p.out_nsplit == NSPLIT) planes(std::integral_constant<int, NSPLIT>{});
      else planes(std::integral_constant<int, 0>{});
      fence_proxy_async_smem();
      named_bar_sync(1, CONSUMER_THREADS);
      if (ct == 0) {
        for (int pl = 0; pl < p.out_nsplit; ++pl)
          for (int j = 0; j < BN / 64 && n0 + 64 * j < p.cout; ++j)
            tma_store_4d(&map_p, smem_u32(pl_s + pl * PLANE_BYTES + j * (BM * 128)), n0 + 64 * j, l0, b0, pl);
        bulk_commit();
      }
    }
    if (warp == STAMP_WARP) PM_STAMP(5);
    if (ct == 0) bulk_wait_read0();
    if (warp == STAMP_WARP) PM_STAMP(6);
    return;
  }
  {
    const int wq = warp & 3, t4 = lane & 3;
    const int r0 = wg * 64 + wq * 16 + (lane >> 2);
    float* stg = reinterpret_cast<float*>(tiles);
#pragma unroll
    for (int i = 0; i < NACC / 4; ++i) {
      const int c = 8 * i + 2 * t4;
#pragma unroll
      for (int h = 0; h < 2; ++h) {
        float v0 = acc0[4 * i + 2 * h] + acc1[4 * i + 2 * h];
        float v1 = acc0[4 * i + 2 * h + 1] + acc1[4 * i + 2 * h + 1];
        v0 += accc[4 * i + 2 * h];
        v1 += accc[4 * i + 2 * h + 1];
        if constexpr (F16) { v0 *= p.acc_scale; v1 *= p.acc_scale; }
        *reinterpret_cast<float2*>(stg + (r0 + 8 * h) * ST + c) = make_float2(v0, v1);
      }
    }
  }
  named_bar_sync(1, CONSUMER_THREADS);

  const bool vec_f = p.out_f32 && ((p.ldo & 3) == 0) && ((reinterpret_cast<uintptr_t>(p.out_f32) & 15) == 0) && ((p.o_bs & 3) == 0);
  const bool vec_b = p.out_bf16 && ((p.ldob & 3) == 0) && ((reinterpret_cast<uintptr_t>(p.out_bf16) & 7) == 0) &&
                     ((p.ob_bs & 3) == 0) && ((p.ob_ps & 3) == 0);
  const bool all_vec = (!p.out_f32 || vec_f) && (!p.residual || p.res_tma) && (!p.out_bf16 || vec_b);
  const float act_slope = p.act == PM_ACT_NONE ? 1.f : (p.act == PM_ACT_RELU ? 0.f : p.slope);
  const int r_shift = 31 - __clz(p.R);
  constexpr int C4 = BN / 4;
  const float* stg = reinterpret_cast<const float*>(tiles);
  const float* res_s = reinterpret_cast<const float*>(tiles + ring_bytes - RES_BYTES);
  mbar_wait_fast(smem_u32(epi_bar), 0);
#pragma unroll 1
  for (int item = ct; item < BM * C4; item += CONSUMER_THREADS) {
    const int rt = item / C4, c = (item % C4) * 4;
    const int b = b0 + (rt >> r_shift), l = l0 + (rt & (p.R - 1));
    const int n = n0 + c;
    if (b >= p.batch || l >= p.rows_out || n >= p.cout) continue;
    const float4 x4 = *reinterpret_cast<const float4*>(stg + rt * ST + c);
    const long long of = (long long)b * p.o_bs + (long long)l * p.ldo;
    const long long orr = (long long)b * p.r_bs + (long long)l * p.ldr;
    const PmPlanes P{p.out_bf16 ? p.out_bf16 + (long long)b * p.ob_bs + (long long)l * p.ldob : nullptr,
                     p.ob_ps, p.ldob, p.out_nsplit};
    if (all_vec && n + 4 <= p.cout) {
      float4 x = x4;
      if (p.bias) {
        const float4 t = *reinterpret_cast<const float4*>(bias_s + c);
        x.x += t.x; x.y += t.y; x.z += t.z; x.w += t.w;
      }
      if (p.residual) {
        const float4 t = *reinterpret_cast<const float4*>(res_s + rt * BN + c);
        x.x += t.x; x.y += t.y; x.z += t.z; x.w += t.w;
      }
      x.x = x.x < 0.f ? (n < p.act_cols ? act_slope : 1.f) * x.x : x.x;
      x.y = x.y < 0.f ? (n + 1 < p.act_cols ? act_slope : 1.f) * x.y : x.y;
      x.z = x.z < 0.f ? (n + 2 < p.act_cols ? act_slope : 1.f) * x.z : x.z;
      x.w = x.w < 0.f ? (n + 3 < p.act_cols ? act_slope : 1.f) * x.w : x.w;
      if (p.out_f32) *reinterpret_cast<float4*>(p.out_f32 + of + n) = x;
      if (P.ptr) pm_store_planes4_t<F16>(P, 0, n, x);
    } else {
      const float xs[4] = {x4.x, x4.y, x4.z, x4.w};
#pragma unroll
      for (int k = 0; k < 4; ++k) {
        if (n + k >= p.cout) break;
        float y = xs[k];
        if (p.bias) y += bias_s[c + k];
        if (p.residual) y += p.residual[orr + n + k];
        y = y < 0.f ? (n + k < p.act_cols ? act_slope : 1.f) * y : y;
        if (p.out_f32) p.out_f32[of + n + k] = y;
        if (P.ptr) pm_store_planes_t<F16>(P, 0, n + k, y);
      }
    }
  }
  if (warp == STAMP_WARP) PM_STAMP(5);
#ifdef PM_TC_TIMING
  named_bar_sync(1, CONSUMER_THREADS);
#endif
  if (warp == STAMP_WARP) PM_STAMP(6);
}

template <bool VEC, bool F16>
__global__ void __launch_bounds__(256) split_bf16_kernel(const float* __restrict__ x, long long x_bs, int ldx, int rows,
                                                         int ch, __nv_bfloat16* __restrict__ out, long long o_ps,
                                                         long long o_bs, int ldo, int nsplit) {
  const int b = blockIdx.y;
  const float* __restrict__ xb = x + (long long)b * x_bs;
  __nv_bfloat16* __restrict__ ob = out + (long long)b * o_bs;
  if (VEC) {
    const int ch4 = ch >> 2;
    const long long total = (long long)rows * ch4;
    for (long long i = (long long)blockIdx.x * blockDim.x + threadIdx.x; i < total; i += (long long)gridDim.x * blockDim.x) {
      const int r = (int)(i / ch4), c4 = (int)(i - (long long)r * ch4);
      const float4 v = *reinterpret_cast<const float4*>(xb + (long long)r * ldx + 4 * c4);
      const PmPlanes P{ob, o_ps, ldo, nsplit};
      pm_store_planes4_t<F16>(P, r, 4 * c4, v);
    }
  } else {
    const long long total = (long long)rows * ch;
    for (long long i = (long long)blockIdx.x * blockDim.x + threadIdx.x; i < total; i += (long long)gridDim.x * blockDim.x) {
      const int r = (int)(i / ch), c = (int)(i - (long long)r * ch);
      const PmPlanes P{ob, o_ps, ldo, nsplit};
      pm_store_planes_t<F16>(P, r, c, xb[(long long)r * ldx + c]);
    }
  }
}

constexpr int stage_bytes_of(int bn, int nsplit) { return nsplit * (A_TILE_BYTES + bn * BK * 2); }
constexpr int stages_of(int bn, int nsplit) {
  return RING_KB * 1024 / stage_bytes_of(bn, nsplit) < MAX_STAGES ? RING_KB * 1024 / stage_bytes_of(bn, nsplit) : MAX_STAGES;
}
constexpr int ring_bytes_of(int bn, int nsplit) { return stages_of(bn, nsplit) * stage_bytes_of(bn, nsplit); }
constexpr bool tma_out_fits(int bn, int nsplit, bool f32, int out_nsplit, bool residual) {
  return (f32 ? BM * bn * 4 : 0) + out_nsplit * BM * bn * 2 + (residual ? BM * bn * 4 : 0) <= ring_bytes_of(bn, nsplit);
}

template <int BN, bool F16, int NSPLIT>
int launch(const CUtensorMap& ma, const CUtensorMap& mw, const CUtensorMap& mr, const CUtensorMap& mo,
           const CUtensorMap& mp, TcParams& p, dim3 grid, cudaStream_t st) {
  constexpr int stage_bytes = stage_bytes_of(BN, NSPLIT);
  constexpr int stages = stages_of(BN, NSPLIT);
  static_assert(stages >= 2, "the operand ring needs two stages");
  constexpr int staging = BM * (BN + 8) * 4, res_bytes = BM * BN * 4;
  static_assert(staging + res_bytes <= stages * stage_bytes && res_bytes <= (stages - 1) * stage_bytes,
                "staging and residual tiles must fit the ring side by side");
  static_assert(tma_out_fits(BN, NSPLIT, true, 2, true), "fp32, two plane and residual tiles must fit the ring");
  static_assert(BN * 4 * BM % 1024 == 0 && stage_bytes % 1024 == 0, "128B-swizzled TMA boxes need 1024-byte alignment");
  p.stages = stages;
  p.res_slot0 = (stages * stage_bytes - res_bytes) / stage_bytes;
  p.rot = (p.res_slot0 - 1 - (p.taps * p.kblocks - 1) % stages + stages) % stages;
  const size_t smem = (size_t)stages * stage_bytes + 1024  + (2 * MAX_STAGES + 2) * sizeof(uint64_t) + BN * sizeof(float);
  static unsigned long long configured = 0;
  if (pm_first_use_on_device(configured)) {
    cudaError_t e = cudaFuncSetAttribute(tapgemm_tc_kernel<BN, F16, NSPLIT>, cudaFuncAttributeMaxDynamicSharedMemorySize, 227 * 1024);
    if (e != cudaSuccess) { configured = 0; return (int)e; }
  }
  tapgemm_tc_kernel<BN, F16, NSPLIT><<<grid, NUM_THREADS, smem, st>>>(ma, mw, mr, mo, mp, p);
  PM_LAUNCH_CHECK();
}

template <int BN>
int launch_fmt(const CUtensorMap* m, TcParams& p, dim3 grid, cudaStream_t st, bool f16) {
  if (f16) {
    if (p.nsplit == 1) return launch<BN, true, 1>(m[0], m[1], m[2], m[3], m[4], p, grid, st);
    if (p.nsplit == 2) return launch<BN, true, 2>(m[0], m[1], m[2], m[3], m[4], p, grid, st);
    return launch<BN, true, 3>(m[0], m[1], m[2], m[3], m[4], p, grid, st);
  }
  if (p.nsplit == 1) return launch<BN, false, 1>(m[0], m[1], m[2], m[3], m[4], p, grid, st);
  if (p.nsplit == 2) return launch<BN, false, 2>(m[0], m[1], m[2], m[3], m[4], p, grid, st);
  return launch<BN, false, 3>(m[0], m[1], m[2], m[3], m[4], p, grid, st);
}

int pick_bn(long long row_tiles, int cout, int w_rows, int sms) {
  if (cout <= 64 || w_rows % 128) return 64;
  const long long waves64 = (row_tiles * pm_cdiv(cout, 64) + sms - 1) / sms;
  const long long waves128 = (row_tiles * pm_cdiv(cout, 128) + sms - 1) / sms;
  return waves128 * 14 <= waves64 * 10 ? 128 : 64;
}

}

extern "C" int pm_tapgemm_tc(const uint16_t* A, long long a_ps, long long a_bs, int lda, int batch, int rows_in, int cin,
                             const uint16_t* W, long long w_ps, int w_rows, int ldw, int taps, int pad, int nsplit,
                             const float* bias, int rows_out, int cout,
                             const float* residual, long long r_bs, int ldr,
                             int act, int act_cols, float slope, float acc_scale,
                             float* out_f32, long long o_bs, int ldo,
                             uint16_t* out_bf16, long long ob_ps, long long ob_bs, int ldob, int out_nsplit,
                             const void* prefetch, long long prefetch_bytes, void* stream) {
  PM_REQUIRE(A && W && (out_f32 || out_bf16));
  const int tile = (nsplit >> PM_TC_TILE_SHIFT) & 0xff;
  const bool store_loop = (nsplit & PM_TC_STORE_LOOP) != 0;
  PM_TAKE_FMT(nsplit, f16);
  PM_TAKE_FMT(out_nsplit, out_f16);
  PM_REQUIRE(!out_bf16 || out_f16 == f16);
  PM_REQUIRE(f16 || acc_scale == 1.0f);
  PM_REQUIRE(!prefetch || (prefetch_bytes >= 0 && (reinterpret_cast<uintptr_t>(prefetch) & 15) == 0));
  PM_REQUIRE(batch > 0 && rows_in > 0 && rows_out > 0 && cin > 0 && cout > 0 && taps > 0);
  PM_REQUIRE(nsplit >= 1 && nsplit <= 3 && (!out_bf16 || (out_nsplit >= 1 && out_nsplit <= 3)));
  PM_REQUIRE(act >= PM_ACT_NONE && act <= PM_ACT_LEAKY);
  PM_REQUIRE((reinterpret_cast<uintptr_t>(A) & 15) == 0 && (reinterpret_cast<uintptr_t>(W) & 15) == 0);
  PM_REQUIRE((lda & 7) == 0 && (ldw & 7) == 0 && lda >= cin && ldw >= cin && w_rows >= cout);
  PM_REQUIRE(batch == 1 || (a_bs & 7) == 0);
  PM_REQUIRE(nsplit == 1 || ((a_ps & 7) == 0 && (w_ps & 7) == 0));
  PM_REQUIRE(!out_f32 || ldo >= cout);
  PM_REQUIRE(!out_bf16 || ldob >= cout);
  PM_REQUIRE(!residual || ldr >= cout);

  int R = 128;
  if (rows_out <= 64 && batch > 1) { R = 16; while (R < rows_out) R <<= 1; }
  const int NB = 128 / R;
  PM_REQUIRE(tile <= 2 && w_rows % 64 == 0 && (tile != 2 || w_rows % 128 == 0));
  int BNsel = tile == 1 ? 64 : 128;
  if (tile == 0) {
    int dev = 0, sms = 0;
    cudaError_t e = cudaGetDevice(&dev);
    if (e == cudaSuccess) e = cudaDeviceGetAttribute(&sms, cudaDevAttrMultiProcessorCount, dev);
    if (e != cudaSuccess) return (int)e;
    BNsel = pick_bn((long long)pm_cdiv(rows_out, R) * pm_cdiv(batch, NB), cout, w_rows, sms);
  }

  TcParams p;
  p.taps = taps; p.pad = pad; p.nsplit = nsplit; p.kblocks = (cin + BK - 1) / BK;
  p.rows_out = rows_out; p.cout = cout; p.batch = batch; p.R = R; p.NB = NB; p.w_rows = w_rows;
  p.bias = bias; p.residual = residual; p.r_bs = r_bs; p.ldr = ldr;
  p.act = act; p.act_cols = act_cols <= 0 ? cout : act_cols; p.slope = slope;
  p.out_f32 = out_f32; p.o_bs = o_bs; p.ldo = ldo;
  p.out_bf16 = reinterpret_cast<__nv_bfloat16*>(out_bf16); p.ob_ps = ob_ps; p.ob_bs = ob_bs; p.ldob = ldob;
  p.out_nsplit = out_bf16 ? out_nsplit : 0;
  p.stages = 0;
  p.prefetch = static_cast<const uint8_t*>(prefetch);
  p.prefetch_bytes = prefetch ? prefetch_bytes : 0;
  p.acc_scale = acc_scale;
  CUtensorMap m[5];
  std::memset(m, 0, sizeof(m));
  CUtensorMap &ma = m[0], &mw = m[1], &mr = m[2], &mo = m[3], &mp = m[4];
  {
    const long long bs_el = batch > 1 ? a_bs : (long long)rows_in * lda;
    const long long ps_el = nsplit > 1 ? a_ps : bs_el * batch;
    cuuint64_t dims[4] = {(cuuint64_t)cin, (cuuint64_t)rows_in, (cuuint64_t)batch, (cuuint64_t)nsplit};
    cuuint64_t strides[3] = {(cuuint64_t)lda * 2, (cuuint64_t)bs_el * 2, (cuuint64_t)ps_el * 2};
    cuuint32_t box[4] = {(cuuint32_t)BK, (cuuint32_t)R, (cuuint32_t)NB, 1};
    if (!encode_map(&ma, A, 4, dims, strides, box, f16)) return PM_EBADARG;
  }
  {
    const long long ps_el = nsplit > 1 ? w_ps : (long long)taps * w_rows * ldw;
    cuuint64_t dims[3] = {(cuuint64_t)cin, (cuuint64_t)taps * w_rows, (cuuint64_t)nsplit};
    cuuint64_t strides[2] = {(cuuint64_t)ldw * 2, (cuuint64_t)ps_el * 2};
    cuuint32_t box[3] = {(cuuint32_t)BK, (cuuint32_t)BNsel, 1};
    if (!encode_map(&mw, W, 3, dims, strides, box, f16)) return PM_EBADARG;
  }
  const bool res_ok = residual && (reinterpret_cast<uintptr_t>(residual) & 15) == 0 && (ldr & 3) == 0 && (batch == 1 || (r_bs & 3) == 0);
  bool tma_out = !store_loop && (!residual || res_ok) && tma_out_fits(BNsel, nsplit, out_f32, p.out_nsplit, residual);
  if (tma_out && out_f32) {
    tma_out = (reinterpret_cast<uintptr_t>(out_f32) & 15) == 0 && (ldo & 3) == 0 && (batch == 1 || (o_bs & 3) == 0);
    const long long bs_el = batch > 1 ? o_bs : (long long)rows_out * ldo;
    cuuint64_t dims[3] = {(cuuint64_t)cout, (cuuint64_t)rows_out, (cuuint64_t)batch};
    cuuint64_t strides[2] = {(cuuint64_t)ldo * 4, (cuuint64_t)bs_el * 4};
    cuuint32_t box[3] = {32, (cuuint32_t)R, (cuuint32_t)NB};
    tma_out = tma_out && encode_tiled(&mo, CU_TENSOR_MAP_DATA_TYPE_FLOAT32, CU_TENSOR_MAP_SWIZZLE_128B, out_f32, 3, dims, strides, box);
  }
  if (tma_out && out_bf16) {
    tma_out = (reinterpret_cast<uintptr_t>(out_bf16) & 15) == 0 && (ldob & 7) == 0 && (batch == 1 || (ob_bs & 7) == 0) &&
              (out_nsplit == 1 || (ob_ps & 7) == 0);
    const long long bs_el = batch > 1 ? ob_bs : (long long)rows_out * ldob;
    const long long ps_el = out_nsplit > 1 ? ob_ps : bs_el * batch;
    cuuint64_t dims[4] = {(cuuint64_t)cout, (cuuint64_t)rows_out, (cuuint64_t)batch, (cuuint64_t)out_nsplit};
    cuuint64_t strides[3] = {(cuuint64_t)ldob * 2, (cuuint64_t)bs_el * 2, (cuuint64_t)ps_el * 2};
    cuuint32_t box[4] = {64, (cuuint32_t)R, (cuuint32_t)NB, 1};
    tma_out = tma_out && encode_map(&mp, out_bf16, 4, dims, strides, box, f16);
  }
  p.res_tma = false;
  for (int swz = tma_out; res_ok && !p.res_tma && swz >= 0; --swz) {
    const long long bs_el = batch > 1 ? r_bs : (long long)rows_out * ldr;
    cuuint64_t dims[3] = {(cuuint64_t)cout, (cuuint64_t)rows_out, (cuuint64_t)batch};
    cuuint64_t strides[2] = {(cuuint64_t)ldr * 4, (cuuint64_t)bs_el * 4};
    cuuint32_t box[3] = {swz ? 32u : (cuuint32_t)BNsel, (cuuint32_t)R, (cuuint32_t)NB};
    p.res_tma = encode_tiled(&mr, CU_TENSOR_MAP_DATA_TYPE_FLOAT32, swz ? CU_TENSOR_MAP_SWIZZLE_128B : CU_TENSOR_MAP_SWIZZLE_NONE,
                             residual, 3, dims, strides, box);
    if (!p.res_tma) tma_out = false;
  }
  p.tma_out = tma_out;
  dim3 grid(pm_cdiv(rows_out, R), pm_cdiv(cout, BNsel), pm_cdiv(batch, NB));
  PM_REQUIRE(grid.z <= 65535 && grid.y <= 65535);
  const cudaStream_t st = (cudaStream_t)stream;
  if (BNsel == 128) return launch_fmt<128>(m, p, grid, st, f16);
  return launch_fmt<64>(m, p, grid, st, f16);
}

#ifdef PM_TC_TIMING
extern "C" int pm_tc_timing_reset() {
  cudaError_t e = cudaDeviceSynchronize();
  if (e != cudaSuccess) return (int)e;
  void* d = nullptr;
  e = cudaGetSymbolAddress(&d, pm_tc_stamps);
  if (e != cudaSuccess) return (int)e;
  return (int)cudaMemset(d, 0, sizeof(unsigned long long) * 4096 * 8);
}
extern "C" int pm_tc_timing_read(unsigned long long* host) {
  cudaError_t e = cudaDeviceSynchronize();
  if (e != cudaSuccess) return (int)e;
  return (int)cudaMemcpyFromSymbol(host, pm_tc_stamps, sizeof(unsigned long long) * 4096 * 8);
}
#endif

extern "C" int pm_split_bf16(const float* x, long long x_bs, int ldx, int batch, int rows, int ch,
                             uint16_t* out, long long o_ps, long long o_bs, int ldo, int nsplit, void* stream) {
  PM_TAKE_FMT(nsplit, f16);
  PM_REQUIRE(x && out && batch >= 0 && rows >= 0 && ch > 0 && ldx >= ch && ldo >= ch && nsplit >= 1 && nsplit <= 3);
  if ((long long)batch * rows == 0) return PM_OK;
  PM_REQUIRE(batch <= 65535);
  const bool vec = (ch & 3) == 0 && (ldx & 3) == 0 && (x_bs & 3) == 0 && (ldo & 3) == 0 && (o_bs & 3) == 0 &&
                   (o_ps & 3) == 0 && (reinterpret_cast<uintptr_t>(x) & 15) == 0 && (reinterpret_cast<uintptr_t>(out) & 7) == 0;
  const long long work = (long long)rows * (vec ? ch / 4 : ch);
  long long gx = (work + 255) / 256;
  const long long cap = batch >= 132 * 4 ? 1 : (132 * 8 + batch - 1) / batch;
  if (gx > cap) gx = cap;
  dim3 grid((unsigned)gx, batch);
  __nv_bfloat16* o = reinterpret_cast<__nv_bfloat16*>(out);
  cudaStream_t st = (cudaStream_t)stream;
  if (f16) {
    if (vec) split_bf16_kernel<true, true><<<grid, 256, 0, st>>>(x, x_bs, ldx, rows, ch, o, o_ps, o_bs, ldo, nsplit);
    else split_bf16_kernel<false, true><<<grid, 256, 0, st>>>(x, x_bs, ldx, rows, ch, o, o_ps, o_bs, ldo, nsplit);
  } else {
    if (vec) split_bf16_kernel<true, false><<<grid, 256, 0, st>>>(x, x_bs, ldx, rows, ch, o, o_ps, o_bs, ldo, nsplit);
    else split_bf16_kernel<false, false><<<grid, 256, 0, st>>>(x, x_bs, ldx, rows, ch, o, o_ps, o_bs, ldo, nsplit);
  }
  PM_LAUNCH_CHECK();
}
```

### pantomatrix_b200/csrc/pm_vq.cu

```cuda
#include "pm_common.cuh"
#include "../../include/pm_emage.h"

namespace {

constexpr int ED = 256;
constexpr int EDP = ED + 1;
constexpr int RT = 64;
constexpr int CT = 64;
constexpr int NT = 256;

__global__ void __launch_bounds__(NT) l2_argmin_kernel(
    const float* __restrict__ z, long long rows, int rows_per_batch, long long z_bs, const float* __restrict__ codebook,
    const float* __restrict__ e2, int n_codes, long long* __restrict__ index) {
  extern __shared__ float smem[];
  float* Zs = smem;
  float* Es = Zs + RT * EDP;
  float* z2s = Es + CT * EDP;
  const int tid = threadIdx.x;
  const long long r0 = (long long)blockIdx.x * RT;

  for (int i = tid; i < RT * (ED / 4); i += NT) {
    const int r = i / (ED / 4), c4 = i % (ED / 4);
    float4 v = make_float4(0.f, 0.f, 0.f, 0.f);
    if (r0 + r < rows) {
      const unsigned g = (unsigned)(r0 + r), gb = g / (unsigned)rows_per_batch;
      const float* zr = rows_per_batch == 0x7fffffff ? z + (r0 + r) * ED
                                                     : z + (long long)gb * z_bs + (long long)(g - gb * (unsigned)rows_per_batch) * ED;
      v = *reinterpret_cast<const float4*>(zr + c4 * 4);
    }
    float* d = Zs + r * EDP + c4 * 4;
    d[0] = v.x; d[1] = v.y; d[2] = v.z; d[3] = v.w;
  }
  __syncthreads();
  {
    const int warp = tid >> 5, lane = tid & 31;
    for (int r = warp; r < RT; r += NT / 32) {
      float s = 0.f;
#pragma unroll
      for (int i = 0; i < ED / 32; ++i) { const float v = Zs[r * EDP + lane + 32 * i]; s = fmaf(v, v, s); }
      s = pm_warp_sum(s);
      if (lane == 0) z2s[r] = s;
    }
  }

  const int ti = tid >> 4, tj = tid & 15;
  float best[4];
  int bestk[4];
#pragma unroll
  for (int a = 0; a < 4; ++a) { best[a] = INFINITY; bestk[a] = 0x7fffffff; }

  for (int k0 = 0; k0 < n_codes; k0 += CT) {
    __syncthreads();
    for (int i = tid; i < CT * (ED / 4); i += NT) {
      const int r = i / (ED / 4), c4 = i % (ED / 4);
      const float4 v = *reinterpret_cast<const float4*>(codebook + (long long)(k0 + r) * ED + c4 * 4);
      float* d = Es + r * EDP + c4 * 4;
      d[0] = v.x; d[1] = v.y; d[2] = v.z; d[3] = v.w;
    }
    __syncthreads();
    float acc[4][4];
#pragma unroll
    for (int a = 0; a < 4; ++a)
#pragma unroll
      for (int c = 0; c < 4; ++c) acc[a][c] = 0.f;
    const float* zp = Zs + (ti * 4) * EDP;
    const float* ep = Es + (tj * 4) * EDP;
#pragma unroll 4
    for (int d = 0; d < ED; ++d) {
      float zv[4], ev[4];
#pragma unroll
      for (int a = 0; a < 4; ++a) { zv[a] = zp[a * EDP + d]; ev[a] = ep[a * EDP + d]; }
#pragma unroll
      for (int a = 0; a < 4; ++a)
#pragma unroll
        for (int c = 0; c < 4; ++c) acc[a][c] = fmaf(zv[a], ev[c], acc[a][c]);
    }
#pragma unroll
    for (int c = 0; c < 4; ++c) {
      const int k = k0 + tj * 4 + c;
      const float ek = __ldg(e2 + k);
#pragma unroll
      for (int a = 0; a < 4; ++a) {
        const float dist = __fsub_rn(__fadd_rn(z2s[ti * 4 + a], ek), __fmul_rn(2.f, acc[a][c]));
        if (dist < best[a] || (dist == best[a] && k < bestk[a])) { best[a] = dist; bestk[a] = k; }
      }
    }
  }
#pragma unroll
  for (int a = 0; a < 4; ++a) {
#pragma unroll
    for (int o = 8; o > 0; o >>= 1) {
      const float ob = __shfl_xor_sync(0xffffffffu, best[a], o);
      const int ok = __shfl_xor_sync(0xffffffffu, bestk[a], o);
      if (ob < best[a] || (ob == best[a] && ok < bestk[a])) { best[a] = ob; bestk[a] = ok; }
    }
    const long long r = r0 + ti * 4 + a;
    if (tj == 0 && r < rows) index[r] = bestk[a] == 0x7fffffff ? 0 : bestk[a];
  }
}

constexpr size_t kL2Smem = (size_t)(RT * EDP + CT * EDP + RT) * sizeof(float);

__global__ void __launch_bounds__(256) row_argmax_kernel(const float* __restrict__ x, long long rows, int ch,
                                                         int ldx, int rows_per_batch, long long x_bs,
                                                         long long* __restrict__ index, int* __restrict__ nonfinite) {
  const int lane = threadIdx.x & 31;
  const long long row = (long long)blockIdx.x * (blockDim.x >> 5) + (threadIdx.x >> 5);
  if (row >= rows) return;
  const unsigned rb = (unsigned)row / (unsigned)rows_per_batch;
  const float* __restrict__ xr = rows_per_batch == 0x7fffffff ? x + row * ldx
                                                              : x + (long long)rb * x_bs + (long long)((unsigned)row - rb * (unsigned)rows_per_batch) * ldx;
  float best = -INFINITY;
  int bk = 0x7fffffff;
  bool bad = false;
  for (int c = lane; c < ch; c += 32) {
    const float v = xr[c];
    bad |= !isfinite(v);
    if (v > best || bk == 0x7fffffff) { best = v; bk = c; }
  }
  if (nonfinite && __any_sync(0xffffffffu, bad) && lane == 0) atomicExch(nonfinite, 1);
#pragma unroll
  for (int o = 16; o > 0; o >>= 1) {
    const float ob = __shfl_xor_sync(0xffffffffu, best, o);
    const int ok = __shfl_xor_sync(0xffffffffu, bk, o);
    if (ob > best || (ob == best && ok < bk)) { best = ob; bk = ok; }
  }
  if (lane == 0) index[row] = bk;
}

template <bool F16>
__global__ void __launch_bounds__(256) gather_rows_kernel(const float* __restrict__ codebook, long long n_table,
                                                          const long long* __restrict__ index, long long rows,
                                                          int ch4, float* __restrict__ out, PmPlanes P) {
  const long long total = rows * ch4;
  for (long long i = (long long)blockIdx.x * blockDim.x + threadIdx.x; i < total;
       i += (long long)gridDim.x * blockDim.x) {
    const long long r = i / ch4;
    const int c4 = (int)(i % ch4);
    long long k = index[r];
    k = k < 0 ? 0 : (k >= n_table ? n_table - 1 : k);
    const float4 v = reinterpret_cast<const float4*>(codebook)[k * ch4 + c4];
    if (out) reinterpret_cast<float4*>(out)[i] = v;
    if (P.ptr) pm_store_planes4_t<F16>(P, r, c4 * 4, v);
  }
}

__global__ void __launch_bounds__(256) row_sqnorm_kernel(const float* __restrict__ x, int rows, int ch,
                                                         float* __restrict__ out) {
  const int lane = threadIdx.x & 31;
  const int row = blockIdx.x * (blockDim.x >> 5) + (threadIdx.x >> 5);
  if (row >= rows) return;
  float s = 0.f;
  for (int c = lane; c < ch; c += 32) { const float v = x[(long long)row * ch + c]; s = fmaf(v, v, s); }
  s = pm_warp_sum(s);
  if (lane == 0) out[row] = s;
}

}

extern "C" int pm_l2_argmin_simt_f32(const float* z, long long rows, int rows_per_batch, long long z_bs,
                                     const float* codebook, const float* e2,
                                     int n_codes, int e_dim, long long* index, void* stream) {
  PM_REQUIRE(z && codebook && e2 && index && rows >= 0);
  if (rows_per_batch <= 0 || z_bs == (long long)rows_per_batch * ED) { rows_per_batch = 0x7fffffff; z_bs = 0; }
  PM_REQUIRE((z_bs & 3) == 0 && (rows_per_batch == 0x7fffffff || rows < 0x7fffffffLL));
  if (e_dim != ED || n_codes <= 0 || n_codes % CT != 0) return PM_EUNSUPPORTED;
  if (rows == 0) return PM_OK;
  {
    cudaError_t e = cudaFuncSetAttribute(l2_argmin_kernel, cudaFuncAttributeMaxDynamicSharedMemorySize, (int)kL2Smem);
    if (e != cudaSuccess) return (int)e;
  }
  const long long grid = (rows + RT - 1) / RT;
  PM_REQUIRE(grid <= 0x7fffffffLL);
  l2_argmin_kernel<<<(unsigned)grid, NT, kL2Smem, (cudaStream_t)stream>>>(z, rows, rows_per_batch, z_bs, codebook, e2, n_codes, index);
  PM_LAUNCH_CHECK();
}

extern "C" int pm_l2_argmin_f32(const float* z, long long rows, int rows_per_batch, long long z_bs,
                                const float* codebook, const float* e2,
                                int n_codes, int e_dim, long long* index, void* stream) {
  if (n_codes == 256 && e_dim == 256 && z && codebook && (reinterpret_cast<uintptr_t>(z) & 15) == 0 &&
      (reinterpret_cast<uintptr_t>(codebook) & 15) == 0)
    return pm_l2_argmin_tc(z, rows, rows_per_batch, z_bs, codebook, e2, n_codes, e_dim, index, 0, stream);
  return pm_l2_argmin_simt_f32(z, rows, rows_per_batch, z_bs, codebook, e2, n_codes, e_dim, index, stream);
}

extern "C" int pm_row_argmax_f32(const float* x, long long rows, int ch, int ldx, int rows_per_batch, long long x_bs,
                                 long long* index, int* nonfinite, void* stream) {
  PM_REQUIRE(x && index && rows >= 0 && ch > 0 && ldx >= ch);
  if (rows == 0) return PM_OK;
  if (rows_per_batch <= 0 || x_bs == (long long)rows_per_batch * ldx) { rows_per_batch = 0x7fffffff; x_bs = 0; }
  PM_REQUIRE(rows_per_batch == 0x7fffffff || rows < 0x7fffffffLL);
  row_argmax_kernel<<<(unsigned)((rows + 7) / 8), 256, 0, (cudaStream_t)stream>>>(x, rows, ch, ldx, rows_per_batch, x_bs,
                                                                                  index, nonfinite);
  PM_LAUNCH_CHECK();
}

extern "C" int pm_gather_rows_f32(const float* codebook, long long n_table, const long long* index, long long rows, int ch,
                                  float* out, uint16_t* planes, long long p_ps, int p_ld, int p_nsplit,
                                  void* stream) {
  PM_REQUIRE(codebook && index && (out || planes) && rows >= 0 && n_table > 0 && ch > 0 && (ch & 3) == 0);
  PM_TAKE_FMT(p_nsplit, f16);
  PM_REQUIRE(pm_planes_ok(planes, p_ps, p_ld, p_nsplit, ch, true));
  const PmPlanes P{reinterpret_cast<__nv_bfloat16*>(planes), p_ps, p_ld, p_nsplit};
  if (rows == 0) return PM_OK;
  long long g = (rows * (ch >> 2) + 255) / 256;
  if (g > 148 * 16) g = 148 * 16;
  if (f16) gather_rows_kernel<true><<<(unsigned)g, 256, 0, (cudaStream_t)stream>>>(codebook, n_table, index, rows, ch >> 2, out, P);
  else gather_rows_kernel<false><<<(unsigned)g, 256, 0, (cudaStream_t)stream>>>(codebook, n_table, index, rows, ch >> 2, out, P);
  PM_LAUNCH_CHECK();
}

extern "C" int pm_row_sqnorm_f32(const float* x, int rows, int ch, float* out, void* stream) {
  PM_REQUIRE(x && out && rows >= 0 && ch > 0);
  if (rows == 0) return PM_OK;
  row_sqnorm_kernel<<<(rows + 7) / 8, 256, 0, (cudaStream_t)stream>>>(x, rows, ch, out);
  PM_LAUNCH_CHECK();
}
```

### pantomatrix_b200/csrc/pm_vq_tc.cu

```cuda
#include "pm_common.cuh"
#include "pm_tc_ptx.cuh"
#include "../../include/pm_emage.h"

namespace {

constexpr int ED = 256;
constexpr int NC = 256;
constexpr int TM = 128;
constexpr int CONSUMER_WARPS = 8, LOAD_WARPS = 4;
constexpr int NTHREADS = 32 * (CONSUMER_WARPS + LOAD_WARPS);
constexpr int KB_A = TM * 128;
constexpr int KB_B = NC * 128;
constexpr int MAXC = 8;

#ifdef PM_VQ_TIMING
__device__ unsigned long long pm_vq_stamps[16];
#define VQ_T(var) const long long var = clock64()
#define VQ_ADD(i, t0)                                                                                     \
  do {                                                                                                    \
    if (blockIdx.x == 0 && (threadIdx.x & 31) == 0) atomicAdd(&pm_vq_stamps[i], (unsigned long long)(clock64() - (t0))); \
  } while (0)
#define VQ_CNT(i, n)                                                                                      \
  do {                                                                                                    \
    if (blockIdx.x == 0 && (threadIdx.x & 31) == 0) atomicAdd(&pm_vq_stamps[i], (unsigned long long)(n)); \
  } while (0)
#else
#define VQ_T(var) do {} while (0)
#define VQ_ADD(i, t0) do {} while (0)
#define VQ_CNT(i, n) do {} while (0)
#endif

struct Smem {
  static constexpr int B = 0;
  static constexpr int A = B + 4 * KB_B;
  static constexpr int E2 = A + 4 * KB_A;
  static constexpr int INFO = E2 + NC * 4;
  static constexpr int CAND = INFO + 2 * TM * 8;
  static constexpr int CNT = CAND + TM * MAXC;
  static constexpr int BARS = CNT + TM * 4;
  static constexpr int MISC = BARS + 2 * 8;
  static constexpr int TOTAL = MISC + 16;
};

__device__ __forceinline__ uint32_t sw128(int row, int byte_in_row) {
  return (uint32_t)((row >> 3) * 1024 + (row & 7) * 128 + ((((byte_in_row >> 4) ^ (row & 7)) << 4) | (byte_in_row & 15)));
}
__device__ __forceinline__ void sts64(uint32_t addr, uint32_t a, uint32_t b) {
  asm volatile("st.shared.v2.b32 [%0], {%1, %2};" ::"r"(addr), "r"(a), "r"(b) : "memory");
}
__device__ __forceinline__ void sts8(uint32_t addr, uint32_t v) {
  asm volatile("st.shared.u8 [%0], %1;" ::"r"(addr), "r"(v) : "memory");
}
__device__ __forceinline__ uint32_t lds8(uint32_t addr) {
  uint32_t v;
  asm volatile("ld.shared.u8 %0, [%1];" : "=r"(v) : "r"(addr) : "memory");
  return v;
}
__device__ __forceinline__ float lds32f(uint32_t addr) {
  float v;
  asm volatile("ld.shared.f32 %0, [%1];" : "=f"(v) : "r"(addr) : "memory");
  return v;
}
__device__ __forceinline__ float2 lds64f(uint32_t addr) {
  float2 v;
  asm volatile("ld.shared.v2.f32 {%0, %1}, [%2];" : "=f"(v.x), "=f"(v.y) : "r"(addr) : "memory");
  return v;
}
__device__ __forceinline__ uint32_t pack_h2(float a, float b) {
  const __half2 h = __floats2half2_rn(a, b);
  return *reinterpret_cast<const uint32_t*>(&h);
}
__device__ __forceinline__ float pow2i(int s) { return __uint_as_float((uint32_t)(s + 127) << 23); }
__device__ __forceinline__ int scale_exp(float m) {
  const int ex = (int)(__float_as_uint(m) >> 23) & 0xFF;
  if (ex == 0 || ex == 255) return 0;
  int s = 140 - ex;
  return s < -100 ? -100 : (s > 100 ? 100 : s);
}

__global__ void __launch_bounds__(NTHREADS, 1) l2_argmin_tc_kernel(
    const float* __restrict__ z, long long rows, int rows_per_batch, long long z_bs, const float* __restrict__ codebook,
    const float* __restrict__ e2, long long* __restrict__ index) {
  auto row_ptr = [&](long long g) -> const float* {
    if (rows_per_batch == 0) return z + g * ED;
    const unsigned gb = (unsigned)g / (unsigned)rows_per_batch, gl = (unsigned)g - gb * (unsigned)rows_per_batch;
    return z + (long long)gb * z_bs + (long long)gl * ED;
  };
  extern __shared__ __align__(1024) uint8_t smem_raw[];
  uint8_t* sm = reinterpret_cast<uint8_t*>((reinterpret_cast<uintptr_t>(smem_raw) + 1023) & ~uintptr_t(1023));
  const uint32_t sm_u = smem_u32(sm);
  float* e2s = reinterpret_cast<float*>(sm + Smem::E2);
  const uint32_t e2s_u = sm_u + Smem::E2, info_u = sm_u + Smem::INFO, cands_u = sm_u + Smem::CAND;
  int* cnt = reinterpret_cast<int*>(sm + Smem::CNT);
  const uint32_t bars = sm_u + Smem::BARS;
  const uint32_t a_full = bars, a_empty = bars + 8;
  float* misc_f = reinterpret_cast<float*>(sm + Smem::MISC);

  const int tid = threadIdx.x, warp = tid >> 5, lane = tid & 31;
  const long long n_tiles = (rows + TM - 1) / TM;
  VQ_T(t_kernel);

  if (tid == 0) {
    mbar_init(a_full, LOAD_WARPS);
    mbar_init(a_empty, 2);
    asm volatile("fence.mbarrier_init.release.cluster;" ::: "memory");
  }
  if (warp == 0) {
    float m = 0.f;
    for (int k = lane; k < NC; k += 32) { const float v = __ldg(e2 + k); e2s[k] = v; m = fmaxf(m, v); }
    m = pm_warp_max(m);
    if (lane == 0) misc_f[0] = m;
  }
  __syncthreads();
  const float e2max = misc_f[0];
  const float emax = sqrtf(e2max);
  const int s_cb = scale_exp(emax);
  {
    const float sc = pow2i(s_cb);
    for (int i = tid; i < NC * (ED / 4); i += NTHREADS) {
      const int k = i >> 6, c4 = i & 63;
      const float4 v = __ldg(reinterpret_cast<const float4*>(codebook) + i);
      const int kb = c4 >> 4, byte = (c4 & 15) * 8;
      sts64(sm_u + Smem::B + kb * KB_B + sw128(k, byte), pack_h2(v.x * sc, v.y * sc), pack_h2(v.z * sc, v.w * sc));
    }
  }
  fence_proxy_async_smem();
  __syncthreads();

  if (warp >= CONSUMER_WARPS) {
    const int lw = warp - CONSUMER_WARPS;
    const float bound_c = 2.0f * 0.0009765625f * 1.02f * emax;
    const float inv_cb = pow2i(-s_cb);
    const bool dense = rows_per_batch == 0;
    auto batch_base = [&](long long tl, int q) { return z + (tl * TM + lw * 32 + q * 8) * ED; };
    int it = 0;
    for (long long tile = blockIdx.x; tile < n_tiles; tile += gridDim.x, ++it) {
      const long long r0 = tile * TM;
      const int slot = it & 1;
      const bool full = dense && r0 + TM <= rows;
      if (lane == 0) {
        const long long nt = tile + gridDim.x;
        if (dense && nt * TM + TM <= rows)
          asm volatile("cp.async.bulk.prefetch.L2.global [%0], %1;" ::"l"(batch_base(nt, 0)), "r"(32 * ED * 4) : "memory");
      }
#pragma unroll 1
      for (int q = 0; q < 4; ++q) {
        const int rb = lw * 32 + q * 8;
        VQ_T(t_ld);
        float4 v[8][2];
        if (full) {
          const float4* p = reinterpret_cast<const float4*>(batch_base(tile, q)) + lane;
#pragma unroll
          for (int j = 0; j < 8; ++j) {
            v[j][0] = ldg_stream4(p + j * (ED / 4));
            v[j][1] = ldg_stream4(p + j * (ED / 4) + 32);
          }
        } else {
#pragma unroll
          for (int j = 0; j < 8; ++j) {
            const long long g = r0 + rb + j;
            if (g < rows) {
              const float4* p = reinterpret_cast<const float4*>(row_ptr(g));
              v[j][0] = ldg_stream4(p + lane);
              v[j][1] = ldg_stream4(p + 32 + lane);
            } else {
              v[j][0] = v[j][1] = make_float4(0.f, 0.f, 0.f, 0.f);
            }
          }
        }
        float ss[8];
#pragma unroll
        for (int j = 0; j < 8; ++j) {
          const float4 a = v[j][0], b = v[j][1];
          ss[j] = fmaf(a.x, a.x, fmaf(a.y, a.y, fmaf(a.z, a.z, fmaf(a.w, a.w, fmaf(b.x, b.x, fmaf(b.y, b.y, fmaf(b.z, b.z, b.w * b.w)))))));
        }
        {
          const bool h16 = lane & 16, h8 = lane & 8, h4 = lane & 4;
#pragma unroll
          for (int i = 0; i < 4; ++i) {
            const float recv = __shfl_xor_sync(0xffffffffu, h16 ? ss[i] : ss[i + 4], 16);
            ss[i] = (h16 ? ss[i + 4] : ss[i]) + recv;
          }
#pragma unroll
          for (int i = 0; i < 2; ++i) {
            const float recv = __shfl_xor_sync(0xffffffffu, h8 ? ss[i] : ss[i + 2], 8);
            ss[i] = (h8 ? ss[i + 2] : ss[i]) + recv;
          }
          const float recv = __shfl_xor_sync(0xffffffffu, h4 ? ss[0] : ss[1], 4);
          ss[0] = (h4 ? ss[1] : ss[0]) + recv;
          ss[0] += __shfl_xor_sync(0xffffffffu, ss[0], 2);
          ss[0] += __shfl_xor_sync(0xffffffffu, ss[0], 1);
        }
        const float ss_own = ss[0];
        int s_own = 0;
        {
          const int ex = (int)(__float_as_uint(ss_own) >> 23) & 0xFF;
          if (ex != 0 && ex != 255) {
            s_own = 13 - ((ex - 127) >> 1);
            s_own = s_own < -100 ? -100 : (s_own > 100 ? 100 : s_own);
          }
        }
        const float sc_own = pow2i(s_own);
        if (lw == 0) VQ_ADD(0, t_ld);
        VQ_T(t_we);
        if (q == 0) mbar_wait_relaxed<20>(a_empty, (uint32_t)(it & 1) ^ 1u);
        if (lw == 0) VQ_ADD(1, t_we);
        VQ_T(t_cv);
        if ((lane & 3) == 0) {
          const float mult = -2.0f * pow2i(-s_own) * inv_cb;
          const float tau = 2.0f * bound_c * sqrtf(ss_own) + 2.4e-7f * 16.f * (ss_own + e2max);
          sts64(info_u + (uint32_t)(slot * TM + rb + (lane >> 2)) * 8, __float_as_uint(mult), __float_as_uint(tau));
        }
        const uint32_t dst0 = sm_u + Smem::A + (lane >> 4) * KB_A + (uint32_t)((rb >> 3) * 1024);
#pragma unroll
        for (int j = 0; j < 8; ++j) {
          const float sc = __shfl_sync(0xffffffffu, sc_own, 4 * j);
          const uint32_t dst = dst0 + (uint32_t)(j * 128 + ((((lane & 15) >> 1) ^ j) << 4) + (lane & 1) * 8);
          sts64(dst, pack_h2(v[j][0].x * sc, v[j][0].y * sc), pack_h2(v[j][0].z * sc, v[j][0].w * sc));
          sts64(dst + 2 * KB_A, pack_h2(v[j][1].x * sc, v[j][1].y * sc), pack_h2(v[j][1].z * sc, v[j][1].w * sc));
        }
        if (lw == 0) VQ_ADD(2, t_cv);
      }
      fence_proxy_async_smem();
      __syncwarp();
      if (lane == 0) mbar_arrive(a_full);
    }
    return;
  }

  const int wg = warp >> 2, t2 = 2 * (lane & 3);
  const int rloc = (warp & 3) * 16 + (lane >> 2);
  const uint64_t b_desc = gmma_desc(GMMA_DESC_K_SW128, sm_u + Smem::B);
  const uint64_t a_desc = gmma_desc(GMMA_DESC_K_SW128, sm_u + Smem::A + wg * (64 * 128));
  int it = 0;
  for (long long tile = blockIdx.x; tile < n_tiles; tile += gridDim.x, ++it) {
    const int slot = it & 1;
    float acc[NC / 2];
#pragma unroll
    for (int i = 0; i < NC / 2; ++i) acc[i] = 0.f;
    VQ_T(t_m1);
    mbar_wait(a_full, (uint32_t)(it & 1));
    if (warp == 0) { VQ_ADD(4, t_m1); VQ_CNT(11, 1); }
    VQ_T(t_e1);
    wgmma_fence();
#pragma unroll
    for (int kb = 0; kb < 4; ++kb)
#pragma unroll
      for (int k = 0; k < 4; ++k)
        wgmma_m64n256k16<false>(acc, a_desc + (uint64_t)(kb * (KB_A >> 4) + k * 2), b_desc + (uint64_t)(kb * (KB_B >> 4) + k * 2));
    wgmma_commit();
    wgmma_wait<0>();
    wgmma_fence_regs(acc);
    float2 inf[2];
#pragma unroll
    for (int hr = 0; hr < 2; ++hr) inf[hr] = lds64f(info_u + (uint32_t)(slot * TM + wg * 64 + rloc + 8 * hr) * 8);
    named_bar_sync(1 + wg, 128);
    if ((tid & 127) == 0) mbar_arrive(a_empty);

    float m1[2] = {INFINITY, INFINITY};
    int k1[2] = {0, 0};
#pragma unroll
    for (int i = 0; i < NC / 8; ++i) {
      const float2 e = lds64f(e2s_u + (uint32_t)(8 * i + t2) * 4);
#pragma unroll
      for (int hr = 0; hr < 2; ++hr) {
        const float d0 = fmaf(inf[hr].x, acc[4 * i + 2 * hr], e.x), d1 = fmaf(inf[hr].x, acc[4 * i + 2 * hr + 1], e.y);
        if (d0 < m1[hr]) { m1[hr] = d0; k1[hr] = 8 * i + t2; }
        if (d1 < m1[hr]) { m1[hr] = d1; k1[hr] = 8 * i + t2 + 1; }
      }
    }
#pragma unroll
    for (int hr = 0; hr < 2; ++hr)
#pragma unroll
      for (int o = 1; o <= 2; o <<= 1) {
        const float om = __shfl_xor_sync(0xffffffffu, m1[hr], o);
        const int ok = __shfl_xor_sync(0xffffffffu, k1[hr], o);
        if (om < m1[hr] || (om == m1[hr] && ok < k1[hr])) { m1[hr] = om; k1[hr] = ok; }
      }
    if (warp == 0) VQ_ADD(7, t_e1);
    VQ_T(t_e2);
    const int row_w = (warp & 3) * 16 + (lane >> 2);
    const int crow0 = wg * 64 + row_w;
    if ((lane & 3) == 0) { cnt[crow0] = 0; cnt[crow0 + 8] = 0; }
    __syncwarp();
#pragma unroll
    for (int i = 0; i < NC / 8; ++i) {
      const float2 e = lds64f(e2s_u + (uint32_t)(8 * i + t2) * 4);
#pragma unroll
      for (int hr = 0; hr < 2; ++hr) {
        const float thr = m1[hr] + inf[hr].y;
#pragma unroll
        for (int u = 0; u < 2; ++u) {
          if (fmaf(inf[hr].x, acc[4 * i + 2 * hr + u], u ? e.y : e.x) <= thr) {
            const int n = atomicAdd(&cnt[crow0 + 8 * hr], 1);
            if (n < MAXC) sts8(cands_u + (uint32_t)((crow0 + 8 * hr) * MAXC + n), (uint32_t)(8 * i + t2 + u));
          }
        }
      }
    }
    __syncwarp();

    if (warp == 0) VQ_ADD(8, t_e2);
    VQ_T(t_e3);
    const long long gbase = tile * TM + wg * 64 + (warp & 3) * 16;
    unsigned rmask = 0;
    {
      const unsigned b0 = __ballot_sync(0xffffffffu, (lane & 3) == 0 && cnt[crow0] > 1 && gbase + (lane >> 2) < rows);
      const unsigned b1 = __ballot_sync(0xffffffffu, (lane & 3) == 0 && cnt[crow0 + 8] > 1 && gbase + (lane >> 2) + 8 < rows);
#pragma unroll
      for (int r = 0; r < 8; ++r) rmask |= (((b0 >> (4 * r)) & 1u) << r) | (((b1 >> (4 * r)) & 1u) << (r + 8));
    }
#ifdef PM_VQ_TIMING
    if (warp == 0) { VQ_CNT(12, __popc(rmask)); }
#endif
    const int grp = lane >> 3, gl = lane & 7;
    while (rmask) {
      const int r = __ffs(rmask) - 1;
      rmask &= rmask - 1;
      const int lrow = wg * 64 + (warp & 3) * 16 + r;
      const int nsrc = cnt[lrow];
      const bool all = nsrc > MAXC;
      const int ncand = all ? NC : nsrc;
      const float4* zr = reinterpret_cast<const float4*>(row_ptr(gbase + r));
      float4 zv[8];
#pragma unroll
      for (int i = 0; i < 8; ++i) zv[i] = __ldg(zr + gl + 8 * i);
      float z2 = 0.f;
#pragma unroll
      for (int i = 0; i < 8; ++i) z2 = fmaf(zv[i].x, zv[i].x, fmaf(zv[i].y, zv[i].y, fmaf(zv[i].z, zv[i].z, fmaf(zv[i].w, zv[i].w, z2))));
      z2 += __shfl_xor_sync(0xffffffffu, z2, 1);
      z2 += __shfl_xor_sync(0xffffffffu, z2, 2);
      z2 += __shfl_xor_sync(0xffffffffu, z2, 4);
      float best = INFINITY;
      int bk = NC;
      const uint32_t list = cands_u + (uint32_t)(lrow * MAXC);
#pragma unroll 1
      for (int base = 0; base < ncand; base += 4) {
        const int ci = base + grp;
        const bool valid = ci < ncand;
        const int c = all ? (ci & (NC - 1)) : (int)lds8(list + (valid ? ci : 0));
        const float4* er = reinterpret_cast<const float4*>(codebook + (long long)c * ED);
        float dot = 0.f;
#pragma unroll
        for (int i = 0; i < 8; ++i) {
          const float4 ev = __ldg(er + gl + 8 * i);
          dot = fmaf(zv[i].x, ev.x, fmaf(zv[i].y, ev.y, fmaf(zv[i].z, ev.z, fmaf(zv[i].w, ev.w, dot))));
        }
        dot += __shfl_xor_sync(0xffffffffu, dot, 1);
        dot += __shfl_xor_sync(0xffffffffu, dot, 2);
        dot += __shfl_xor_sync(0xffffffffu, dot, 4);
        float dd = __fsub_rn(__fadd_rn(z2, lds32f(e2s_u + (uint32_t)c * 4)), __fmul_rn(2.f, dot));
        int cc = c;
        if (!valid) { dd = INFINITY; cc = NC; }
#pragma unroll
        for (int o = 8; o <= 16; o <<= 1) {
          const float od = __shfl_xor_sync(0xffffffffu, dd, o);
          const int oc = __shfl_xor_sync(0xffffffffu, cc, o);
          if (od < dd || (od == dd && oc < cc)) { dd = od; cc = oc; }
        }
        if (dd < best || (dd == best && cc < bk)) { best = dd; bk = cc; }
      }
      if (bk < NC && (lane >> 2) == (r & 7)) k1[r >> 3] = bk;
    }
    if ((lane & 3) == 0) {
#pragma unroll
      for (int hr = 0; hr < 2; ++hr) {
        const long long g = gbase + (lane >> 2) + 8 * hr;
        if (g < rows) index[g] = (long long)k1[hr];
      }
    }
    if (warp == 0) VQ_ADD(9, t_e3);
    __syncwarp();
  }
  if (warp == 0) VQ_ADD(10, t_kernel);
}

constexpr size_t kSmem = Smem::TOTAL + 1024;

}

extern "C" int pm_l2_argmin_tc(const float* z, long long rows, int rows_per_batch, long long z_bs,
                               const float* codebook, const float* e2,
                               int n_codes, int e_dim, long long* index, int max_ctas, void* stream) {
  PM_REQUIRE(z && codebook && e2 && index && rows >= 0);
  if (rows_per_batch <= 0 || z_bs == (long long)rows_per_batch * ED) { rows_per_batch = 0; z_bs = 0; }
  PM_REQUIRE((z_bs & 3) == 0 && (rows_per_batch == 0 || rows < 0x7fffffffLL));
  if (e_dim != ED || n_codes != NC) return PM_EUNSUPPORTED;
  PM_REQUIRE((reinterpret_cast<uintptr_t>(z) & 15) == 0 && (reinterpret_cast<uintptr_t>(codebook) & 15) == 0);
  if (rows == 0) return PM_OK;
  int dev = 0, sms = 0;
  cudaError_t e = cudaGetDevice(&dev);
  if (e == cudaSuccess) e = cudaDeviceGetAttribute(&sms, cudaDevAttrMultiProcessorCount, dev);
  if (e != cudaSuccess) return (int)e;
  static unsigned long long configured = 0;
  if (pm_first_use_on_device(configured)) {
    e = cudaFuncSetAttribute(l2_argmin_tc_kernel, cudaFuncAttributeMaxDynamicSharedMemorySize, (int)kSmem);
    if (e != cudaSuccess) { configured = 0; return (int)e; }
  }
  const long long tiles = (rows + TM - 1) / TM;
  long long grid = tiles < sms ? tiles : sms;
  if (max_ctas > 0 && grid > max_ctas) grid = max_ctas;
  l2_argmin_tc_kernel<<<(unsigned)grid, NTHREADS, kSmem, (cudaStream_t)stream>>>(z, rows, rows_per_batch, z_bs, codebook, e2, index);
  PM_LAUNCH_CHECK();
}

#ifdef PM_VQ_TIMING
extern "C" int pm_vq_timing_reset() {
  cudaError_t e = cudaDeviceSynchronize();
  if (e != cudaSuccess) return (int)e;
  void* d = nullptr;
  e = cudaGetSymbolAddress(&d, pm_vq_stamps);
  if (e != cudaSuccess) return (int)e;
  return (int)cudaMemset(d, 0, sizeof(unsigned long long) * 16);
}
extern "C" int pm_vq_timing_read(unsigned long long* host) {
  cudaError_t e = cudaDeviceSynchronize();
  if (e != cudaSuccess) return (int)e;
  return (int)cudaMemcpyFromSymbol(host, pm_vq_stamps, sizeof(unsigned long long) * 16);
}
#endif
```

### pantomatrix_b200/ops.py

```python
from __future__ import annotations

import math

import torch

from . import _lib

ACT_NONE, ACT_RELU, ACT_LEAKY = 0, 1, 2
ROW_NONE, ROW_PE, ROW_SPK = 0, 1, 2

launch_count = 0

FMT_F16 = 0x100
TC_TILE_SHIFT = 16
TC_STORE_LOOP = 1 << 24
F16_ACT_SCALE = 64.0
_PLANE_DTYPE = torch.bfloat16


def set_plane_format(name: str) -> None:
    global _PLANE_DTYPE
    _PLANE_DTYPE = {"bf16": torch.bfloat16, "fp16": torch.float16}[name]


def plane_format() -> str:
    return "fp16" if _PLANE_DTYPE == torch.float16 else "bf16"


def _fmt_bit(t) -> int:
    return FMT_F16 if t.dtype == torch.float16 else 0


def _stream() -> int:
    return torch.cuda.current_stream().cuda_stream


def _ptr(t) -> int | None:
    return None if t is None else t.data_ptr()


def _chk(t: torch.Tensor, dtype=torch.float32):
    if not t.is_cuda:
        raise _lib.PmError("pantomatrix_b200 ops need CUDA tensors (no CPU fallback)")
    if t.dtype != dtype:
        raise _lib.PmError(f"expected {dtype}, got {t.dtype}")
    if t.dim() and t.stride(-1) != 1 and t.shape[-1] != 1:
        raise _lib.PmError("innermost dimension must be contiguous")
    return t


def _call(name, *args):
    global launch_count
    launch_count += 1
    _lib.call(name, *args)


def _bs_ld(t: torch.Tensor):
    return (t.stride(0) if t.shape[0] > 1 else t.shape[1] * t.stride(1)), t.stride(1)


def tapgemm(a, w, bias, *, rows_out=None, stride=1, pad=0, act=ACT_NONE, slope=0.0, residual=None, out=None):
    _chk(a), _chk(w)
    batch, rows_in, cin = a.shape
    taps, cout, cin_w = w.shape
    assert cin_w == cin and w.is_contiguous(), (w.shape, a.shape)
    if rows_out is None:
        rows_out = (rows_in + 2 * pad - taps) // stride + 1
    if out is None:
        out = torch.empty(batch, rows_out, cout, device=a.device, dtype=torch.float32)
    else:
        assert out.shape == (batch, rows_out, cout), (out.shape, (batch, rows_out, cout))
    _chk(out)
    if residual is not None:
        _chk(residual)
        assert residual.shape == out.shape
    if (taps == 1 and pad == 0 and stride == 1 and batch > 1 and a.stride(0) == rows_in * a.stride(1)
            and out.stride(0) == rows_out * out.stride(1)
            and (residual is None or residual.stride(0) == rows_out * residual.stride(1))):
        a = a.reshape(1, batch * rows_in, cin) if a.is_contiguous() else a.as_strided(
            (1, batch * rows_in, cin), (0, a.stride(1), 1), a.storage_offset())
        flat = lambda t: t.as_strided((1, batch * rows_out, cout), (0, t.stride(1), 1), t.storage_offset())
        out_v = flat(out)
        res_v = flat(residual) if residual is not None else None
        batch_k, rows_in_k, rows_out_k = 1, batch * rows_in, batch * rows_out
    else:
        out_v, res_v, batch_k, rows_in_k, rows_out_k = out, residual, batch, rows_in, rows_out
    a_bs, lda = _bs_ld(a)
    o_bs, ldo = _bs_ld(out_v)
    r_bs, ldr = _bs_ld(res_v) if res_v is not None else (0, 0)
    _call("pm_tapgemm_f32", a.data_ptr(), a_bs, lda, batch_k, rows_in_k, cin,
          w.data_ptr(), _ptr(bias), taps, stride, pad, rows_out_k, cout,
          _ptr(res_v), r_bs, ldr, act, float(slope), out_v.data_ptr(), o_bs, ldo, _stream())
    return out


def wav_stem(audio, a_bs, a_ws, batch, windows, n_samples, w1, b1, wd, bd, *, stride, pad, slope, offset=0, nsplit=0):
    _chk(audio)
    cout, ks = w1.shape
    rows_out = (n_samples + 2 * pad - ks) // stride + 1
    sc = torch.empty(batch * windows, rows_out, cout, device=audio.device, dtype=torch.float32)
    if nsplit:
        y1 = _new_planes(nsplit, (batch * windows, rows_out), cout, audio.device)
        y_ptr, pa = 0, (y1.t.data_ptr(), y1.t.stride(0), y1.t.stride(2), nsplit | _fmt_bit(y1.t))
    else:
        y1 = torch.empty_like(sc)
        y_ptr, pa = y1.data_ptr(), (0, 0, 0, 0)
    _call("pm_wav_stem_f32", audio.data_ptr() + 4 * offset, a_bs, a_ws, batch, windows, n_samples,
          w1.data_ptr(), b1.data_ptr(), wd.data_ptr(), bd.data_ptr(), cout, ks, stride, pad, rows_out,
          float(slope), y_ptr, sc.data_ptr(), *pa, _stream())
    return y1, sc


def resample_poly(pcm, bank, up, down, n_pre_remove, out=None):
    if pcm.dtype not in (torch.int16, torch.float32):
        raise _lib.PmError(f"resample_poly: PCM must be int16 or float32, got {pcm.dtype}")
    if pcm.dim() != 3:
        raise _lib.PmError(f"resample_poly: PCM must be (batch, n_in, channels), got shape {tuple(pcm.shape)}")
    _chk(pcm, pcm.dtype), _chk(bank)
    batch, n_in, channels = pcm.shape
    if n_in > 1 and pcm.stride(1) != channels:
        raise _lib.PmError("resample_poly: the samples of a clip must be dense (interleaved channels)")
    if not bank.is_contiguous() or bank.dim() != 2 or bank.shape[0] != up:
        raise _lib.PmError(f"resample_poly: bank must be a contiguous (up={up}, taps) tensor, got {tuple(bank.shape)}")
    n_out = -(-n_in * up // down)
    if out is None:
        out = torch.empty(batch, n_out, device=pcm.device, dtype=torch.float32)
    elif tuple(out.shape) != (batch, n_out):
        raise _lib.PmError(f"resample_poly: out must be {(batch, n_out)}, got {tuple(out.shape)}")
    _chk(out)
    _call("pm_resample_poly_f32", pcm.data_ptr(), int(pcm.dtype == torch.int16), pcm.stride(0) if batch > 1 else 0,
          batch, n_in, channels, bank.data_ptr(), int(up), int(down), bank.shape[1], int(n_pre_remove),
          out.data_ptr(), out.stride(0) if batch > 1 else 0, _stream())
    return out


class Act:
    __slots__ = ("f", "p")

    def __init__(self, f=None, p=None):
        self.f, self.p = f, p


def _new_planes(nsplit, lead_shape, ch, device, slack_rows=0, dtype=None):
    batch, rows = lead_shape
    dtype = dtype or _PLANE_DTYPE
    ld = _round_up(ch, 8)
    if slack_rows:
        buf = torch.empty(nsplit, batch * rows + slack_rows, ld, device=device, dtype=dtype)
        if buf.is_cuda:
            for i in range(nsplit):
                _lib.call("pm_memset_async", buf[i, batch * rows:].data_ptr(), 0, slack_rows * ld * buf.element_size(), _stream())
        else:
            buf[:, batch * rows:].zero_()
        t = buf[:, :batch * rows].view(nsplit, batch, rows, ld)
    else:
        t = torch.empty(nsplit, batch, rows, ld, device=device, dtype=dtype)
    return Planes(t, rows, ch, slack_rows)


def _pargs(pl):
    if pl is None:
        return None, 0, 0, 0
    return pl.t.data_ptr(), pl.t.stride(0), pl.t.stride(2), pl.t.shape[0] | _fmt_bit(pl.t)


def _result(f, pl, nsplit):
    return f if nsplit == 0 else Act(f, pl)


def add_layernorm(x, r, gamma, beta, eps=1e-5, nsplit=0, f32=True):
    _chk(x)
    assert x.is_contiguous() and (r is None or (r.is_contiguous() and r.shape == x.shape))
    ch = x.shape[-1]
    rows = x.numel() // ch
    out = torch.empty_like(x) if (f32 or not nsplit) else None
    pl = _new_planes(nsplit, (x.shape[0], rows // x.shape[0]), ch, x.device) if nsplit else None
    _call("pm_add_layernorm_f32", x.data_ptr(), _ptr(r), gamma.data_ptr(), beta.data_ptr(), _ptr(out),
          rows, ch, float(eps), *_pargs(pl), _stream())
    return _result(out, pl, nsplit)


def attention(q, k, v, batch, heads, tq, tk, head_dim, nsplit=0, f32=True):
    for t in (q, k, v):
        _chk(t)
    E = heads * head_dim
    out = torch.empty(batch * tq, E, device=q.device, dtype=torch.float32) if (f32 or not nsplit) else None
    pl = _new_planes(nsplit, (batch, tq), E, q.device) if nsplit else None
    _call("pm_attention_f32", q.data_ptr(), q.stride(0), k.data_ptr(), k.stride(0), v.data_ptr(), v.stride(0),
          _ptr(out), E, batch, heads, tq, tk, head_dim, *_pargs(pl), _stream())
    return _result(out, pl, nsplit)


def attention_tc(q, q_col0, k, k_col0, v, v_col0, batch, heads, tq, tk, head_dim, nsplit=2, f32=False):
    for pl, rows in ((q, tq), (k, tk), (v, tk)):
        assert pl.t.dtype == torch.float16 and pl.t.shape[0] == 2 and pl.t.shape[1] == batch and pl.rows == rows, \
            "attention_tc needs two-plane fp16 operands of (batch, rows, ch)"
    E = heads * head_dim
    dev = q.t.device
    out = torch.empty(batch * tq, E, device=dev, dtype=torch.float32) if (f32 or not nsplit) else None
    pl = _new_planes(nsplit, (batch, tq), E, dev, dtype=torch.float16) if nsplit else None
    _call("pm_attention_tc",
          q.t.data_ptr(), q.t.stride(0), q.t.stride(1), q.t.stride(2), q.ch, q_col0,
          k.t.data_ptr(), k.t.stride(0), k.t.stride(1), k.t.stride(2), k.ch, k_col0,
          v.t.data_ptr(), v.t.stride(0), v.t.stride(1), v.t.stride(2), v.ch, v_col0,
          _ptr(out), E, batch, heads, tq, tk, head_dim, *_pargs(pl), _stream())
    return _result(out, pl, nsplit)


def add_rows(x, pe, spk, first, second, batch, rows, ch, nsplit=0, f32=True):
    dev = (pe if pe is not None else spk).device
    out = torch.empty(batch, rows, ch, device=dev, dtype=torch.float32) if (f32 or not nsplit) else None
    if x is not None:
        _chk(x)
        assert x.is_contiguous() and x.numel() == batch * rows * ch
    pl = _new_planes(nsplit, (batch, rows), ch, dev) if nsplit else None
    _call("pm_add_rows_f32", _ptr(x), _ptr(pe), _ptr(spk), first, second, _ptr(out), batch, rows, ch, *_pargs(pl), _stream())
    return _result(out, pl, nsplit)


def add2(a, b, nsplit=0, f32=True):
    _chk(a), _chk(b)
    assert a.shape == b.shape, (a.shape, b.shape)
    n, ch = a.numel(), a.shape[-1]
    if not (a.is_contiguous() and b.is_contiguous()):
        assert nsplit == 0, "strided add2 writes fp32 only"
        out, pl = torch.empty(a.shape, device=a.device, dtype=torch.float32), None
        (rows, lda), ldb, ldo = _rows_ld(a), _rows_ld(b)[1], ch
    else:
        out = torch.empty_like(a) if (f32 or not nsplit) else None
        pl = _new_planes(nsplit, (a.shape[0], n // ch // a.shape[0]), ch, a.device) if nsplit else None
        rows, lda = (n // ch, ch) if nsplit else (1, n)
        ch = ldb = ldo = lda
    _call("pm_add2_f32", a.data_ptr(), lda, b.data_ptr(), ldb, _ptr(out), ldo, rows, ch, *_pargs(pl), _stream())
    return _result(out, pl, nsplit)


def _rows_ld(t):
    ch = t.shape[-1]
    rows = t.numel() // ch if ch else 0
    lead = [(n, s) for n, s in zip(t.shape[:-1], t.stride()[:-1]) if n > 1]
    ld = lead[-1][1] if lead else ch
    want = ld
    for n, s in reversed(lead):
        if s != want:
            raise _lib.PmError(f"rows of a {tuple(t.shape)} view with strides {t.stride()} are not evenly spaced")
        want = s * n
    return rows, ld


def lstm_cond(spk, speaker_id, seed, seed_len, seed_frames, pose_dims, out):
    _chk(spk), _chk(speaker_id, torch.int64), _chk(out)
    assert spk.is_contiguous() and speaker_id.is_contiguous()
    batch, t, cols = out.shape
    assert speaker_id.numel() == batch and cols == spk.shape[1] + pose_dims + 1, (speaker_id.shape, out.shape)
    o_bs, ldo = _bs_ld(out)
    s_bs = s_ld = 0
    if seed is not None:
        _chk(seed)
        assert seed.dim() == 3 and seed.shape[0] == batch and seed.shape[2] == pose_dims, (seed.shape, batch, pose_dims)
        if seed.numel() == 0:
            seed = None
        else:
            s_bs, s_ld = _bs_ld(seed)
    _call("pm_lstm_cond_f32", spk.data_ptr(), spk.shape[0], spk.shape[1], speaker_id.data_ptr(), _ptr(seed), s_bs, s_ld,
          int(seed_len), int(seed_frames), int(pose_dims), out.data_ptr(), o_bs, ldo, batch, t, _stream())
    return out


def window_input(motion, mask, seed, mask_embedding, start, win_len, pre, nsplit=0, f32=True, shape=None):
    batch, total_len, ch = motion.shape if motion is not None else shape
    for t in (motion, mask):
        if t is not None:
            _chk(t)
            assert t.is_contiguous() and t.shape == (batch, total_len, ch)
    seed_bs = 0
    if seed is not None:
        _chk(seed)
        assert seed.shape == (batch, pre, ch) and (pre <= 1 or seed.stride(1) == ch)
        seed_bs = seed.stride(0)
    dev = mask_embedding.device
    out = torch.empty(batch, win_len, ch, device=dev, dtype=torch.float32) if (f32 or not nsplit) else None
    pl = _new_planes(nsplit, (batch, win_len), ch, dev) if nsplit else None
    _call("pm_window_input_f32", _ptr(motion), _ptr(mask), _ptr(seed), mask_embedding.data_ptr(),
          _ptr(out), batch, total_len, start, win_len, pre, ch, seed_bs, *_pargs(pl), _stream())
    return _result(out, pl, nsplit)


def _batched_rows(x, ld):
    if x.dim() == 2:
        assert x.stride(0) == ld
        return x.shape[0], 0, 0
    assert x.dim() == 3 and (x.shape[1] == 1 or x.stride(1) == ld)
    return x.shape[0] * x.shape[1], x.shape[1], x.stride(0)


def l2_argmin(z, codebook, e2, engine="auto", max_ctas=0):
    _chk(z), _chk(codebook), _chk(e2)
    assert codebook.is_contiguous()
    n_codes, e_dim = codebook.shape
    if z.dim() > 3:
        z = z.reshape(-1, e_dim)
    rows, rpb, z_bs = _batched_rows(z, e_dim)
    idx = torch.empty(z.shape[:-1], device=z.device, dtype=torch.int64)
    if engine == "tc":
        _call("pm_l2_argmin_tc", z.data_ptr(), rows, rpb, z_bs, codebook.data_ptr(), e2.data_ptr(), n_codes, e_dim,
              idx.data_ptr(), int(max_ctas), _stream())
    elif engine == "simt":
        _call("pm_l2_argmin_simt_f32", z.data_ptr(), rows, rpb, z_bs, codebook.data_ptr(), e2.data_ptr(), n_codes, e_dim,
              idx.data_ptr(), _stream())
    else:
        _call("pm_l2_argmin_f32", z.data_ptr(), rows, rpb, z_bs, codebook.data_ptr(), e2.data_ptr(), n_codes, e_dim,
              idx.data_ptr(), _stream())
    return idx


def row_argmax(x, nonfinite=None):
    _chk(x)
    ch = x.shape[-1]
    if x.dim() > 3:
        x = x.reshape(-1, ch)
    ld = x.stride(-2) if x.shape[-2] > 1 else ch
    rows, rpb, x_bs = _batched_rows(x, ld)
    idx = torch.empty(x.shape[:-1], device=x.device, dtype=torch.int64)
    _call("pm_row_argmax_f32", x.data_ptr(), rows, ch, ld, rpb, x_bs, idx.data_ptr(), _ptr(nonfinite), _stream())
    return idx


def zero_flag(device):
    flag = torch.empty(1, device=device, dtype=torch.int32)
    _lib.call("pm_memset_async", flag.data_ptr(), 0, 4, _stream())
    return flag


def gather_rows(codebook, index, nsplit=0, f32=True):
    _chk(codebook), _chk(index, torch.int64)
    assert index.is_contiguous()
    ch = codebook.shape[1]
    out = torch.empty(*index.shape, ch, device=codebook.device, dtype=torch.float32) if (f32 or not nsplit) else None
    pl = None
    if nsplit:
        lead = (index.shape[0], index.numel() // index.shape[0]) if index.dim() > 1 else (1, index.numel())
        pl = _new_planes(nsplit, lead, ch, codebook.device)
    _call("pm_gather_rows_f32", codebook.data_ptr(), codebook.shape[0], index.data_ptr(), index.numel(), ch, _ptr(out),
          *_pargs(pl), _stream())
    return _result(out, pl, nsplit)


def row_sqnorm(x):
    _chk(x)
    out = torch.empty(x.shape[0], device=x.device, dtype=torch.float32)
    _call("pm_row_sqnorm_f32", x.data_ptr(), x.shape[0], x.shape[1], out.data_ptr(), _stream())
    return out


def pose_compose(face, upper, hands, lower, bs, t, device):
    for ten, dim in ((face, 106), (upper, 78), (hands, 180), (lower, 61)):
        if ten is not None:
            _chk(ten)
            assert ten.is_contiguous() and ten.shape == (bs, t, dim), (ten.shape, dim)
    expression = torch.empty(bs, t, 100, device=device, dtype=torch.float32)
    axis_angle = torch.empty(bs, t, 165, device=device, dtype=torch.float32)
    motion4inf = torch.empty(bs, t, 337, device=device, dtype=torch.float32)
    _call("pm_pose_compose_f32", _ptr(face), _ptr(upper), _ptr(hands), _ptr(lower), expression.data_ptr(),
          axis_angle.data_ptr(), motion4inf.data_ptr(), bs * t, _stream())
    return expression, axis_angle, motion4inf


def global_trans(rec, ref_trans, dt, vel_off=54):
    _chk(rec), _chk(ref_trans)
    assert rec.is_contiguous()
    bs, t, ld = rec.shape
    assert ref_trans.shape == (bs, 3)
    trans = torch.empty(bs, t, 3, device=rec.device, dtype=torch.float32)
    _call("pm_global_trans_f32", rec.data_ptr(), ld, vel_off, ref_trans.data_ptr(), ref_trans.stride(0), float(dt),
          trans.data_ptr(), bs, t, _stream())
    return trans




def _round_up(x, m):
    return (x + m - 1) // m * m


class Planes:
    __slots__ = ("t", "rows", "ch", "slack")

    def __init__(self, t, rows, ch, slack=0):
        self.t, self.rows, self.ch, self.slack = t, rows, ch, slack

    def flat(self):
        ns, b, r, ld = self.t.shape
        assert self.t.stride(1) == r * self.t.stride(2)
        return Planes(self.t.as_strided((ns, 1, b * r, ld), (self.t.stride(0), b * r * self.t.stride(2), self.t.stride(2), 1),
                                        self.t.storage_offset()), b * r, self.ch, self.slack)

    @property
    def nsplit(self):
        return self.t.shape[0]

    @property
    def batch(self):
        return self.t.shape[1]


def split_bf16(x, nsplit, slack_rows=0):
    _chk(x)
    batch, rows, ch = x.shape
    pl = _new_planes(nsplit, (batch, rows), ch, x.device, slack_rows)
    x_bs, ldx = _bs_ld(x)
    _call("pm_split_bf16", x.data_ptr(), x_bs, ldx, batch, rows, ch, pl.t.data_ptr(), pl.t.stride(0), pl.t.stride(1),
          pl.t.stride(2), nsplit | _fmt_bit(pl.t), _stream())
    return pl


class PackedW:
    __slots__ = ("t", "taps", "cout", "cin", "w_rows", "ldw", "acc_scale")

    def __init__(self, w, nsplit):
        taps, cout, cin = w.shape
        bn = 64 if cout <= 64 else 128
        self.taps, self.cout, self.cin = taps, cout, cin
        self.w_rows, self.ldw = _round_up(cout, bn), _round_up(cin, 8)
        full = torch.zeros(taps, self.w_rows, self.ldw, device=w.device, dtype=torch.float32)
        full[:, :cout, :cin] = w
        self.acc_scale = 1.0
        if _PLANE_DTYPE == torch.float16:
            m = float(full.abs().max())
            if m > 0.0 and math.isfinite(m):
                k = math.floor(math.log2(32768.0 / m))
                full = full * (2.0 ** k)
                self.acc_scale = 2.0 ** -k
            self.acc_scale /= F16_ACT_SCALE
        planes, rem = [], full
        for _ in range(nsplit):
            p = rem.to(_PLANE_DTYPE)
            planes.append(p)
            rem = rem - p.float()
        self.t = torch.stack(planes).contiguous()


def tapgemm_tc(a: Planes, w: PackedW, bias, *, rows_in=None, rows_out, pad=0, act=ACT_NONE, act_cols=0, slope=0.0,
               residual=None, want_f32=True, out_nsplit=0, out=None, a_view=None, out_slack=0, prefetch=None, tile=0,
               store_loop=False):
    t = a.t
    nsplit, batch = t.shape[0], t.shape[1]
    assert nsplit == w.t.shape[0] and t.dtype == w.t.dtype, "A and W must use the same split and plane format"
    fmt = _fmt_bit(t)
    rows_a, cin, lda = (a.rows, a.ch, t.stride(2)) if a_view is None else a_view
    if rows_in is not None:
        rows_a = rows_in
    assert cin == w.cin, (cin, w.cin)
    assert tile in (0, 64, 128), tile
    cout = w.cout
    dev = t.device
    out_f = None
    if want_f32:
        out_f = out if out is not None else torch.empty(batch, rows_out, cout, device=dev, dtype=torch.float32)
        assert out_f.shape == (batch, rows_out, cout)
    o_bs, ldo = _bs_ld(out_f) if out_f is not None else (0, 0)
    out_p = None
    if out_nsplit:
        out_p = _new_planes(out_nsplit, (batch, rows_out), cout, dev, out_slack, dtype=t.dtype)
    r_bs, ldr = _bs_ld(residual) if residual is not None else (0, 0)
    if residual is not None:
        _chk(residual)
        assert residual.shape == (batch, rows_out, cout)
    _call("pm_tapgemm_tc", t.data_ptr(), t.stride(0), t.stride(1), lda, batch, rows_a, cin,
          w.t.data_ptr(), w.t.stride(0), w.w_rows, w.ldw, w.taps, pad, nsplit | fmt | (tile // 64) << TC_TILE_SHIFT | (TC_STORE_LOOP if store_loop else 0),
          _ptr(bias), rows_out, cout, _ptr(residual), r_bs, ldr, act, act_cols, float(slope), float(w.acc_scale),
          _ptr(out_f), o_bs, ldo,
          None if out_p is None else out_p.t.data_ptr(), 0 if out_p is None else out_p.t.stride(0),
          0 if out_p is None else out_p.t.stride(1), 0 if out_p is None else out_p.t.stride(2),
          out_nsplit | (fmt if out_nsplit else 0),
          None if prefetch is None else prefetch.data_ptr(),
          0 if prefetch is None else prefetch.numel() * prefetch.element_size(), _stream())
    return out_f, out_p




def lstm_bidir(xproj, whh, barrier, hidden):
    _chk(xproj), _chk(whh)
    assert xproj.is_contiguous() and whh.is_contiguous() and whh.shape == (2, 4 * hidden, hidden)
    batch, t, w = xproj.shape
    assert w == 8 * hidden
    y = torch.empty(batch, t, 2 * hidden, device=xproj.device, dtype=torch.float32)
    _call("pm_lstm_bidir_f32", xproj.data_ptr(), xproj.stride(0), xproj.stride(1), whh.data_ptr(), y.data_ptr(),
          y.stride(0), y.stride(1), barrier.data_ptr(), batch, t, hidden, _stream())
    return y


def rot6d_to_aa(rot6d, slot, n_sel):
    _chk(rot6d)
    assert rot6d.is_contiguous() and rot6d.shape[-1] == n_sel * 6
    rows = rot6d.numel() // (n_sel * 6)
    out = torch.empty(*rot6d.shape[:-1], 165, device=rot6d.device, dtype=torch.float32)
    _call("pm_rot6d_to_aa_f32", rot6d.data_ptr(), rows, n_sel, slot.data_ptr(), out.data_ptr(), _stream())
    return out




def _clip_frame_strides(x):
    return (x.stride(0), x.stride(1)) if x is not None else (0, 0)


def smplx_fk(poses, betas, expression, transl, joint_mask, tables, joints, rel=None, feat=None, planes=None):
    for x in (poses, betas, expression, transl, joints, rel, feat):
        if x is not None:
            _chk(x)
    jt, jd, pm, par, order, lstart = tables
    batch, t, _ = poses.shape
    pb, pt = _clip_frame_strides(poses)
    eb, et = _clip_frame_strides(expression)
    tb, tt = _clip_frame_strides(transl)
    _call("pm_smplx_fk_f32", poses.data_ptr(), pb, pt, _ptr(betas), 0 if betas is None else betas.stride(0),
          _ptr(expression), eb, et, _ptr(transl), tb, tt, int(joint_mask), batch, t,
          jt.data_ptr(), jd.data_ptr(), pm.data_ptr(), par.data_ptr(), order.data_ptr(), lstart.data_ptr(),
          lstart.numel() - 1, joints.data_ptr(), _ptr(rel), _ptr(feat), 0 if feat is None else feat.stride(0),
          *_pargs(planes), _stream())
    return joints


def smplx_skin(verts, n_verts, csr, rel, transl, t):
    _chk(verts), _chk(rel)
    row_ptr, col, val = csr
    tb, tt = _clip_frame_strides(transl)
    if transl is not None:
        _chk(transl)
    _call("pm_smplx_skin_f32", verts.data_ptr(), verts.stride(0), verts.shape[0], int(n_verts), row_ptr.data_ptr(),
          col.data_ptr(), val.data_ptr(), rel.data_ptr(), _ptr(transl), tb, tt, int(t), _stream())
    return verts


def motion_rep(poses, joints, dt, two_dt, out):
    _chk(poses), _chk(joints), _chk(out)
    assert joints.is_contiguous() and out.is_contiguous()
    batch, t, _ = poses.shape
    pb, pt = _clip_frame_strides(poses)
    _call("pm_motion_rep_f32", poses.data_ptr(), pb, pt, joints.data_ptr(), batch, t, float(dt), float(two_dt),
          out.data_ptr(), _stream())
    return out




def mesh_vertex(verts, views, faces, vf_csr, xy, depth, normal):
    nviews = xy.shape[1]
    if len(verts) != nviews or len(views) != nviews:
        raise _lib.PmError(f"mesh_vertex: {nviews} views need {nviews} vertex tensors and transforms")
    for v in verts:
        _chk(v)
    _chk(xy, torch.int32), _chk(depth), _chk(normal), _chk(faces, torch.int32)
    v0, (s0, o0) = verts[0], views[0]
    v1, (s1, o1) = (verts[1], views[1]) if nviews == 2 else (None, (0.0, (0.0, 0.0, 0.0)))
    vf_ptr, vf_face = vf_csr
    _call("pm_mesh_vertex_f32", v0.data_ptr(), v0.stride(0), _ptr(v1), 0 if v1 is None else v1.stride(0),
          v0.shape[1], v0.shape[0], float(s0), float(o0[0]), float(o0[1]), float(o0[2]), float(s1), float(o1[0]),
          float(o1[1]), float(o1[2]), faces.data_ptr(), vf_ptr.data_ptr(), vf_face.data_ptr(), xy.data_ptr(),
          depth.data_ptr(), normal.data_ptr(), nviews, _stream())


def mesh_raster(xy, depth, faces, vis):
    _chk(xy, torch.int32), _chk(depth), _chk(faces, torch.int32), _chk(vis, torch.int64)
    assert xy.is_contiguous() and depth.is_contiguous() and vis.is_contiguous() and vis.shape[1] == xy.shape[1]
    _lib.call("pm_memset_async", vis.data_ptr(), 0xFF, vis.numel() * 8, _stream())
    _call("pm_mesh_raster", xy.data_ptr(), depth.data_ptr(), xy.shape[2], faces.data_ptr(), faces.shape[0],
          xy.shape[0], vis.data_ptr(), xy.shape[1], _stream())


def mesh_shade(vis, xy, normal, faces, out):
    _chk(vis, torch.int64), _chk(xy, torch.int32), _chk(normal), _chk(faces, torch.int32), _chk(out, torch.uint8)
    if out.shape[2] != vis.shape[1] * vis.shape[3]:
        raise _lib.PmError(f"mesh_shade: {vis.shape[1]} views need out {vis.shape[1] * vis.shape[3]} wide, "
                           f"got {out.shape[2]}")
    assert out[0].is_contiguous() and normal.is_contiguous()
    _call("pm_mesh_shade_u8", vis.data_ptr(), xy.data_ptr(), normal.data_ptr(), xy.shape[2], faces.data_ptr(),
          vis.shape[0], out.data_ptr(), out.stride(0), vis.shape[1], _stream())


def time_upsample(x, k, out=None):
    _chk(x)
    batch, t, ch = x.shape
    if out is None:
        out = torch.empty(batch, k * t, ch, device=x.device, dtype=torch.float32)
    _chk(out)
    assert tuple(out.shape) == (batch, k * t, ch) and out.is_contiguous()
    xb, xt = _clip_frame_strides(x)
    _call("pm_time_upsample_f32", x.data_ptr(), xb, xt, batch, t, ch, int(k), out.data_ptr(), _stream())
    return out




def png_encode(frames, data, nbytes, row_bits, row_adler):
    _chk(frames, torch.uint8), _chk(data, torch.uint8), _chk(nbytes, torch.int64)
    _chk(row_bits, torch.int64), _chk(row_adler, torch.int64)
    n, h, w, _ = frames.shape
    assert data.is_contiguous() and row_bits.is_contiguous() and row_adler.is_contiguous() and nbytes.is_contiguous()
    cap, fs = data.shape[1], frames.stride(0) if n > 1 else 3 * h * w
    _lib.call("pm_memset_async", data.data_ptr(), 0, data.numel(), _stream())
    _call("pm_png_count", frames.data_ptr(), fs, n, h, w, row_bits.data_ptr(), row_adler.data_ptr(), _stream())
    _call("pm_png_scan", n, h, w, row_bits.data_ptr(), row_adler.data_ptr(), data.data_ptr(), cap, nbytes.data_ptr(),
          _stream())
    _call("pm_png_emit", frames.data_ptr(), fs, n, h, w, row_bits.data_ptr(), data.data_ptr(), cap, _stream())
    _call("pm_png_crc", n, h, w, data.data_ptr(), cap, nbytes.data_ptr(), _stream())




def h264_encode(frames, clip_len, qp, data, nbytes, scratch, sizes, gop=1, recon=None, search=0, mv=None):
    _chk(frames, torch.uint8), _chk(data, torch.uint8), _chk(nbytes, torch.int64)
    _chk(scratch, torch.uint8), _chk(sizes, torch.int32)
    n, h, w, _ = frames.shape
    assert data.is_contiguous() and nbytes.is_contiguous() and scratch.is_contiguous() and sizes.is_contiguous()
    cap, fs, slice_cap = data.shape[1], frames.stride(0) if n > 1 else 3 * h * w, scratch.shape[2]
    _lib.call("pm_memset_async", data.data_ptr(), 0, data.numel(), _stream())
    if gop == 1:
        _call("pm_h264_encode", frames.data_ptr(), fs, n, clip_len, h, w, qp, scratch.data_ptr(), slice_cap,
              sizes.data_ptr(), _stream())
    elif search > 0:
        _chk(recon, torch.uint8), _chk(mv, torch.int16)
        chains = n // clip_len * -(-clip_len // gop)
        assert 1 < gop <= clip_len and 0 < search <= 32 and n % clip_len == 0
        assert recon.is_contiguous() and recon.shape[0] >= chains and recon.shape[1] >= 3 * h * w
        assert mv.is_contiguous() and mv.shape[0] >= chains and mv.shape[1:] == (h // 16, w // 16, 2)
        _call("pm_h264_encode_me", frames.data_ptr(), fs, n, clip_len, h, w, qp, scratch.data_ptr(), slice_cap,
              sizes.data_ptr(), gop, recon.data_ptr(), recon.stride(0), search, mv.data_ptr(), mv.numel() // 2,
              _stream())
    else:
        _chk(recon, torch.uint8)
        chains = n // clip_len * -(-clip_len // gop)
        assert 1 < gop <= clip_len and n % clip_len == 0 and recon.is_contiguous()
        assert recon.shape[0] >= chains and recon.shape[1] == h // 16 and recon.shape[2] >= 24 * w
        _call("pm_h264_encode_gop", frames.data_ptr(), fs, n, clip_len, h, w, qp, scratch.data_ptr(), slice_cap,
              sizes.data_ptr(), gop, recon.data_ptr(), recon.stride(1), _stream())
    _call("pm_h264_gather", n, h, w, scratch.data_ptr(), slice_cap, sizes.data_ptr(), data.data_ptr(), cap,
          nbytes.data_ptr(), _stream())




def flac_encode(pcm, bps, rate, data, nbytes, rec):
    _chk(pcm, torch.int16 if bps == 16 else torch.int32), _chk(data, torch.uint8), _chk(nbytes, torch.int64)
    _chk(rec, torch.int32)
    b, n, c = pcm.shape
    assert data.is_contiguous() and nbytes.is_contiguous() and rec.is_contiguous()
    cs = pcm.stride(0) if b > 1 else n * c
    _lib.call("pm_memset_async", data.data_ptr(), 0, data.numel(), _stream())
    _call("pm_flac_analyse", pcm.data_ptr(), cs, b, n, c, bps, rec.data_ptr(), _stream())
    _call("pm_flac_emit", pcm.data_ptr(), cs, b, n, c, bps, rate, rec.data_ptr(), data.data_ptr(), data.shape[1],
          nbytes.data_ptr(), _stream())


def softmax2_mix(sel, c1, c2, out=None):
    _chk(sel), _chk(c1), _chk(c2)
    assert sel.is_contiguous() and c1.is_contiguous() and c2.is_contiguous() and sel.shape[-1] == 2
    ch = c1.shape[-1]
    rows = c1.numel() // ch
    if out is None:
        out = torch.empty_like(c1)
    _call("pm_softmax2_mix_f32", sel.data_ptr(), c1.data_ptr(), c2.data_ptr(), out.data_ptr(), rows, ch, out.stride(-2), _stream())
    return out
```

### pantomatrix_b200/pipeline.py

```python
from __future__ import annotations

import torch

from . import _lib, ops
from .emage_audio.engine import PARTS, overflow_flag, select_inputs

_OVERFLOW = ("fp16x3: a GEMM operand exceeded the fp16 range (|x| > 1023 after the x64 pre-scale) and the result is NaN - "
             "use engine.set_precision('bf16x6') for this checkpoint (model.inference() outside a captured graph retries "
             "in bf16x6 by itself)")


def generate(model, motion_vq, audio, speaker_id=None, masked_motion=None, mask=None, ref_trans=None):
    return _generate(model, motion_vq, audio, speaker_id, masked_motion, mask, ref_trans)[:2]


@torch.no_grad()
def _generate(model, motion_vq, audio, speaker_id=None, masked_motion=None, mask=None, ref_trans=None):
    dev = next(model.parameters()).device
    bs = audio.shape[0]
    if speaker_id is None:
        speaker_id = torch.zeros(bs, 1, dtype=torch.long, device=dev)
    lat = model.inference(audio, speaker_id, motion_vq, masked_motion=masked_motion, mask=mask)
    nonfinite = overflow_flag(dev)
    cfg = model.cfg.to_dict()
    idx = {p: ops.row_argmax(lat["cls_" + p], nonfinite=nonfinite) for p in PARTS}
    if nonfinite is not None:
        capturing = lat["rec_face"].is_cuda and torch.cuda.is_current_stream_capturing()
        if not capturing and bool(nonfinite):
            raise _lib.PmError(_OVERFLOW)
    index, latent = select_inputs(cfg, lat, idx)
    if ref_trans is None:
        ref_trans = torch.zeros(1, 3, device=dev)
    pred = motion_vq.decode(
        face_latent=latent["face"], upper_latent=latent["upper"], lower_latent=latent["lower"],
        hands_latent=latent["hands"], face_index=index["face"], upper_index=index["upper"],
        lower_index=index["lower"], hands_index=index["hands"], get_global_motion=True, ref_trans=ref_trans)
    return lat, pred, nonfinite


def _audio_input(batch, n_samples, dev, input_rate, input_channels, input_dtype):
    if (input_rate, input_channels, input_dtype) == (16000, 1, torch.float32):
        return None, None, torch.zeros(batch, n_samples, device=dev)
    from .audio_io import Resampler
    if input_dtype not in (torch.int16, torch.float32) or not 1 <= input_channels <= 8:
        raise ValueError(f"input must be int16 or float32 with 1-8 channels, got {input_dtype} x {input_channels}")
    resampler = Resampler(input_rate, 16000, device=dev)
    pcm = torch.zeros(batch, n_samples, input_channels, device=dev, dtype=input_dtype)
    return pcm, resampler, torch.zeros(batch, resampler.n_out(n_samples), device=dev)


def _stage(dst, src, who, exact):
    if exact:
        want = (tuple(dst.shape), dst.dtype)
        if not torch.is_tensor(src) or (tuple(src.shape), src.dtype) != want:
            got = (tuple(src.shape), src.dtype) if torch.is_tensor(src) else type(src).__name__
            raise ValueError(f"{who} input must be a {want[0]} {want[1]} tensor, got {got}")
        if src.is_cuda and src.device != dst.device:
            raise ValueError(f"{who} input is on {src.device}, the pipeline on {dst.device}")
        if not src.is_cuda and not src.is_pinned():
            raise ValueError(f"{who} host input must be in pinned memory (tensor.pin_memory())")
    dst.copy_(src, non_blocking=True)


class CapturedPipeline:

    def __init__(self, model, motion_vq, batch: int, n_samples: int, warmup: int = 2, body_priority: bool = True,
                 input_rate: int = 16000, input_channels: int = 1, input_dtype=torch.float32):
        self.model, self.vq = model, motion_vq
        dev = next(model.parameters()).device
        self.device = dev
        self.pcm, self.resampler, self.audio = _audio_input(batch, n_samples, dev, input_rate, input_channels, input_dtype)
        self.speaker_id = torch.zeros(batch, 1, dtype=torch.long, device=dev)
        self.ref_trans = torch.zeros(1, 3, device=dev)

        def step():
            if self.resampler is not None:
                self.resampler(self.pcm, out=self.audio)
            return _generate(model, motion_vq, self.audio, self.speaker_id, ref_trans=self.ref_trans)

        side = torch.cuda.Stream(device=dev)
        side.wait_stream(torch.cuda.current_stream(dev))
        with torch.cuda.stream(side):
            for _ in range(warmup):
                step()
        torch.cuda.current_stream(dev).wait_stream(side)
        torch.cuda.synchronize(dev)
        self.graph = torch.cuda.CUDAGraph()
        before = ops.launch_count
        self.capture_stream = torch.cuda.Stream(device=dev, priority=-1) if body_priority else None
        with torch.cuda.graph(self.graph, stream=self.capture_stream):
            self.latent, self.pred, self.nonfinite = step()
        self.kernels_per_replay = ops.launch_count - before

    @torch.no_grad()
    def __call__(self, audio, speaker_id=None):
        if self.pcm is None:
            _stage(self.audio, audio, "CapturedPipeline", exact=False)
        else:
            _stage(self.pcm, audio, "CapturedPipeline", exact=True)
        if speaker_id is not None:
            self.speaker_id.copy_(speaker_id, non_blocking=True)
        self.graph.replay()
        ops.launch_count += self.kernels_per_replay
        if self.nonfinite is not None and bool(self.nonfinite):
            raise _lib.PmError(_OVERFLOW)
        return self.latent, self.pred


def _memset0(t):
    _lib.call("pm_memset_async", t.data_ptr(), 0, t.numel() * t.element_size(), torch.cuda.current_stream(t.device).cuda_stream)


class CapturedLstmPipeline:

    def __init__(self, model, batch: int, n_samples: int, seed_frames: int = 4, warmup: int = 2,
                 input_rate: int = 16000, input_channels: int = 1, input_dtype=torch.float32):
        from .lstm_audio.modeling import wav_frames
        if seed_frames < 0:
            raise ValueError(f"seed_frames must be >= 0, got {seed_frames}")
        dev = next(model.parameters()).device
        self.model, self.device, self.batch, self.seed_frames = model, dev, batch, seed_frames
        self.pcm, self.resampler, self.audio = _audio_input(batch, n_samples, dev, input_rate, input_channels, input_dtype)
        eng = model._eng()
        self.speaker_dims, self.pose_dims = eng.spk.shape[0], eng.pose_dims
        self.speaker_id = torch.zeros(batch, 1, dtype=torch.long, device=dev)
        self.seed = torch.zeros(batch, seed_frames, self.pose_dims, device=dev)
        self.barrier = torch.zeros(4, dtype=torch.int32, device=dev)
        t = wav_frames(self.audio.shape[1])

        @torch.no_grad()
        def step():
            if self.resampler is not None:
                self.resampler(self.pcm, out=self.audio)
            out = eng.forward(self.audio, eng.kernel_cond(self.speaker_id, self.seed, t, seed_frames), True,
                              barrier=self.barrier)
            flag = overflow_flag(dev)
            if flag is not None:
                ops.row_argmax(out["motion"], nonfinite=flag)
            return out, flag

        side = torch.cuda.Stream(device=dev)
        side.wait_stream(torch.cuda.current_stream(dev))
        with torch.cuda.stream(side):
            for _ in range(warmup):
                step()
        torch.cuda.current_stream(dev).wait_stream(side)
        torch.cuda.synchronize(dev)
        self.graph = torch.cuda.CUDAGraph()
        before = ops.launch_count
        with torch.cuda.graph(self.graph):
            self.out, self.nonfinite = step()
        self.kernels_per_replay = ops.launch_count - before

    def _stage_inputs(self, audio, speaker_id, seed_motion):
        if self.pcm is None:
            _stage(self.audio, audio, "CapturedLstmPipeline", exact=False)
        else:
            _stage(self.pcm, audio, "CapturedLstmPipeline", exact=True)
        if speaker_id is None:
            _memset0(self.speaker_id)
        else:
            if not torch.is_tensor(speaker_id) or tuple(speaker_id.shape) != (self.batch, 1) or speaker_id.dtype != torch.int64:
                got = (tuple(speaker_id.shape), speaker_id.dtype) if torch.is_tensor(speaker_id) else type(speaker_id).__name__
                raise ValueError(f"speaker_id must be a ({self.batch}, 1) int64 tensor, got {got}")
            lo, hi = int(speaker_id.min()), int(speaker_id.max())
            if lo < 0 or hi >= self.speaker_dims:
                raise ValueError(f"speaker_id must lie in [0, {self.speaker_dims}), got values in [{lo}, {hi}]")
            self.speaker_id.copy_(speaker_id, non_blocking=True)
        if seed_motion is None:
            _memset0(self.seed)
        else:
            want = (self.batch, self.seed_frames, self.pose_dims)
            if not torch.is_tensor(seed_motion) or tuple(seed_motion.shape) != want or seed_motion.dtype != torch.float32:
                got = (tuple(seed_motion.shape), seed_motion.dtype) if torch.is_tensor(seed_motion) else type(seed_motion).__name__
                raise ValueError(f"seed_motion must be a {want} float32 tensor or None, got {got}")
            self.seed.copy_(seed_motion, non_blocking=True)

    @torch.no_grad()
    def __call__(self, audio, speaker_id=None, seed_motion=None):
        self._stage_inputs(audio, speaker_id, seed_motion)
        self.graph.replay()
        ops.launch_count += self.kernels_per_replay
        if self.nonfinite is not None and bool(self.nonfinite):
            raise _lib.PmError(_OVERFLOW)
        return self.out
```

Before: 340,500.

## Enable programmatic dependent launch across pipeline kernels in captured graph

Routes all kernel launches through a cudaLaunchKernelEx helper that can set the programmatic stream serialization attribute, and adds griddepcontrol wait/launch_dependents calls to each kernel. PDL is turned on only while the CUDA graph is captured, controlled by an environment variable that defaults to on. The tensor-core GEMM also issues its weight TMA loads for the first stages before waiting on the previous grid, so weight prefetch overlaps the prior kernel's tail. The goal is to hide launch gaps and prologue latency between the many small dependent kernels. The risk is correctness: every kernel that reads upstream data must wait before doing so.

Measured after the change: 344,400 (median of 6 runs). +1.2%, better.

```diff
diff --git a/include/pm_emage.h b/include/pm_emage.h
--- a/include/pm_emage.h
+++ b/include/pm_emage.h
@@ -12,6 +12,7 @@
 int pm_abi_version(void);
 int pm_memset_async(void* ptr, int value, long long bytes, void* stream);
 int pm_device_cc(void);
+int pm_set_pdl(int on);
 
 int pm_tapgemm_f32(const float* A, long long a_bs, int lda, int batch, int rows_in, int cin,
                    const float* W, const float* bias, int taps, int stride, int pad,
diff --git a/pantomatrix_b200/_lib.py b/pantomatrix_b200/_lib.py
--- a/pantomatrix_b200/_lib.py
+++ b/pantomatrix_b200/_lib.py
@@ -14,6 +14,7 @@
 SIGNATURES = {
     "pm_abi_version": [],
     "pm_device_cc": [],
+    "pm_set_pdl": [_i],
     "pm_tapgemm_f32": [_p, _ll, _i, _i, _i, _i, _p, _p, _i, _i, _i, _i, _i, _p, _ll, _i, _i, _f, _p, _ll, _i, _p],
     "pm_tapgemm_tc": [_p, _ll, _ll, _i, _i, _i, _i, _p, _ll, _i, _i, _i, _i, _i, _p, _i, _i, _p, _ll, _i,
                       _i, _i, _f, _f, _p, _ll, _i, _p, _ll, _ll, _i, _i, _p, _ll, _p],
diff --git a/pantomatrix_b200/csrc/pm_attention_tc.cu b/pantomatrix_b200/csrc/pm_attention_tc.cu
--- a/pantomatrix_b200/csrc/pm_attention_tc.cu
+++ b/pantomatrix_b200/csrc/pm_attention_tc.cu
@@ -39,6 +39,8 @@
                                                                    const __grid_constant__ CUtensorMap map_k,
                                                                    const __grid_constant__ CUtensorMap map_v,
                                                                    const AttnParams p) {
+  pm_grid_wait();
+  pm_grid_launch_dependents();
   extern __shared__ __align__(1024) uint8_t smem_raw[];
   uint8_t* sm = reinterpret_cast<uint8_t*>((reinterpret_cast<uintptr_t>(smem_raw) + 1023) & ~uintptr_t(1023));
   const uint32_t sm_u = smem_u32(sm);
@@ -246,7 +248,7 @@
     cudaError_t e = cudaFuncSetAttribute(attention_tc_kernel, cudaFuncAttributeMaxDynamicSharedMemorySize, (int)kSmem);
     if (e != cudaSuccess) { configured = 0; return (int)e; }
   }
-  attention_tc_kernel<<<batch * heads, NTHREADS, kSmem, (cudaStream_t)stream>>>(mq, mk, mv, p);
+  pm_launch(attention_tc_kernel, dim3(batch * heads), dim3(NTHREADS), kSmem, (cudaStream_t)stream, mq, mk, mv, p);
   PM_LAUNCH_CHECK();
 }
 
diff --git a/pantomatrix_b200/csrc/pm_audio.cu b/pantomatrix_b200/csrc/pm_audio.cu
--- a/pantomatrix_b200/csrc/pm_audio.cu
+++ b/pantomatrix_b200/csrc/pm_audio.cu
@@ -54,6 +54,8 @@
 resample_poly_kernel(const void* __restrict__ pcm, long long in_bs, long long n_in, int channels,
                      const float* __restrict__ bank, int up, int down, int taps, long long n_pre_remove,
                      float* __restrict__ out, long long out_bs, long long n_out, int rows) {
+  pm_grid_wait();
+  pm_grid_launch_dependents();
   extern __shared__ float stage[];
   const int b = blockIdx.y;
   const void* clip = I16 ? (const void*)(reinterpret_cast<const int16_t*>(pcm) + b * in_bs)
@@ -102,8 +104,8 @@
     if (e != cudaSuccess) return (int)e;
   }
   const long long tiles = (n_out + (long long)up * rows - 1) / ((long long)up * rows);
-  kern<<<dim3((unsigned)tiles, (unsigned)batch), kThreads, smem, st>>>(pcm, in_bs, n_in, channels, bank, up, down, taps,
-                                                                       n_pre_remove, out, out_bs, n_out, rows);
+  pm_launch(kern, dim3((unsigned)tiles, (unsigned)batch), dim3(kThreads), smem, st, pcm, in_bs, n_in, channels, bank, up,
+            down, taps, n_pre_remove, out, out_bs, n_out, rows);
   PM_LAUNCH_CHECK();
 }
 
diff --git a/pantomatrix_b200/csrc/pm_common.cuh b/pantomatrix_b200/csrc/pm_common.cuh
--- a/pantomatrix_b200/csrc/pm_common.cuh
+++ b/pantomatrix_b200/csrc/pm_common.cuh
@@ -3,6 +3,8 @@
 #include <cuda_fp16.h>
 #include <cuda_runtime.h>
 #include <stdint.h>
+
+#include <utility>
 
 #define PM_OK 0
 #define PM_EBADARG (-1)
@@ -20,6 +22,27 @@
   } while (0)
 
 static inline int pm_cdiv(long long a, long long b) { return (int)((a + b - 1) / b); }
+
+extern int pm_pdl_on;
+
+template <typename... KArgs, typename... Args>
+static inline void pm_launch(void (*kernel)(KArgs...), dim3 grid, dim3 block, size_t smem, cudaStream_t stream,
+                             Args&&... args) {
+  cudaLaunchAttribute attr;
+  attr.id = cudaLaunchAttributeProgrammaticStreamSerialization;
+  attr.val.programmaticStreamSerializationAllowed = 1;
+  cudaLaunchConfig_t cfg = {};
+  cfg.gridDim = grid;
+  cfg.blockDim = block;
+  cfg.dynamicSmemBytes = smem;
+  cfg.stream = stream;
+  cfg.attrs = &attr;
+  cfg.numAttrs = pm_pdl_on ? 1 : 0;
+  (void)cudaLaunchKernelEx(&cfg, kernel, std::forward<Args>(args)...);
+}
+
+__device__ __forceinline__ void pm_grid_wait() { asm volatile("griddepcontrol.wait;" ::: "memory"); }
+__device__ __forceinline__ void pm_grid_launch_dependents() { asm volatile("griddepcontrol.launch_dependents;" ::: "memory"); }
 
 static inline bool pm_first_use_on_device(unsigned long long& mask) {
   int d = 0;
diff --git a/pantomatrix_b200/csrc/pm_elementwise.cu b/pantomatrix_b200/csrc/pm_elementwise.cu
--- a/pantomatrix_b200/csrc/pm_elementwise.cu
+++ b/pantomatrix_b200/csrc/pm_elementwise.cu
@@ -28,6 +28,8 @@
     const float* __restrict__ w1, const float* __restrict__ b1, const float* __restrict__ wd,
     const float* __restrict__ bd, int stride, int pad, int rows_out, float slope,
     float* __restrict__ y1, float* __restrict__ sc, const PmPlanes P) {
+  pm_grid_wait();
+  pm_grid_launch_dependents();
   extern __shared__ float sx[];
   constexpr int LPR = COUT / 2;
   constexpr int RW = 32 / LPR;
@@ -110,6 +112,8 @@
 __global__ void __launch_bounds__(256) add_layernorm_kernel(
     const float* __restrict__ x, const float* __restrict__ r, const float* __restrict__ gamma,
     const float* __restrict__ beta, float* __restrict__ out, long long rows, float eps, PmPlanes P) {
+  pm_grid_wait();
+  pm_grid_launch_dependents();
   const int lane = threadIdx.x & 31;
   const long long row = (long long)blockIdx.x * (blockDim.x >> 5) + (threadIdx.x >> 5);
   if (row >= rows) return;
@@ -161,6 +165,8 @@
 __global__ void __launch_bounds__(256) add_rows_kernel(
     const float* __restrict__ x, const float* __restrict__ pe, const float* __restrict__ spk,
     int first, int second, float* __restrict__ out, int batch, int rows, int ch, PmPlanes P) {
+  pm_grid_wait();
+  pm_grid_launch_dependents();
   const int ch4 = ch >> 2;
   const long long total = (long long)batch * rows * ch4;
   for (long long i = (long long)blockIdx.x * blockDim.x + threadIdx.x; i < total;
@@ -187,6 +193,8 @@
                                                    const float* __restrict__ b, long long ldb,
                                                    float* __restrict__ out, long long ldo, long long rows,
                                                    long long ch, long long nv, PmPlanes P) {
+  pm_grid_wait();
+  pm_grid_launch_dependents();
   const long long i0 = (long long)blockIdx.x * blockDim.x + threadIdx.x, step = (long long)gridDim.x * blockDim.x;
   for (long long i = i0; i < rows * nv; i += step) {
     const long long r = rows == 1 ? 0 : i / nv, c = (i - r * nv) * 4;
@@ -210,6 +218,8 @@
     const float* __restrict__ motion, const float* __restrict__ mask, const float* __restrict__ seed,
     const float* __restrict__ mask_embedding, float* __restrict__ out,
     int batch, int total_len, int start, int win_len, int pre, int ch, long long seed_bs, PmPlanes P) {
+  pm_grid_wait();
+  pm_grid_launch_dependents();
   const long long total = (long long)batch * win_len * ch;
   for (long long i = (long long)blockIdx.x * blockDim.x + threadIdx.x; i < total;
        i += (long long)gridDim.x * blockDim.x) {
@@ -256,8 +266,8 @@
   dim3 grid(pm_cdiv(rows_out, STEM_ROWS), batch * windows);
   cudaStream_t st = (cudaStream_t)stream;
 #define PM_STEM(CO, F)                                                                                          \
-  wav_stem_kernel<15, CO, F><<<grid, STEM_THREADS, smem, st>>>(audio, a_bs, a_ws, batch, n_samples, w1, b1, wd, bd, \
-                                                               stride, pad, rows_out, slope, y1, sc, P)
+  pm_launch(wav_stem_kernel<15, CO, F>, grid, dim3(STEM_THREADS), smem, st, audio, a_bs, a_ws, batch, n_samples, w1, b1, \
+            wd, bd, stride, pad, rows_out, slope, y1, sc, P)
   if (cout == 64) { if (f16) PM_STEM(64, true); else PM_STEM(64, false); }
   else { if (f16) PM_STEM(32, true); else PM_STEM(32, false); }
 #undef PM_STEM
@@ -277,20 +287,20 @@
   cudaStream_t st = (cudaStream_t)stream;
   switch (ch) {
     case 256:
-      if (f16) add_layernorm_kernel<2, true><<<grid, warps * 32, 0, st>>>(x, r, gamma, beta, out, rows, eps, P);
-      else add_layernorm_kernel<2, false><<<grid, warps * 32, 0, st>>>(x, r, gamma, beta, out, rows, eps, P);
+      if (f16) pm_launch(add_layernorm_kernel<2, true>, grid, dim3(warps * 32), 0, st, x, r, gamma, beta, out, rows, eps, P);
+      else pm_launch(add_layernorm_kernel<2, false>, grid, dim3(warps * 32), 0, st, x, r, gamma, beta, out, rows, eps, P);
       break;
     case 512:
-      if (f16) add_layernorm_kernel<4, true><<<grid, warps * 32, 0, st>>>(x, r, gamma, beta, out, rows, eps, P);
-      else add_layernorm_kernel<4, false><<<grid, warps * 32, 0, st>>>(x, r, gamma, beta, out, rows, eps, P);
+      if (f16) pm_launch(add_layernorm_kernel<4, true>, grid, dim3(warps * 32), 0, st, x, r, gamma, beta, out, rows, eps, P);
+      else pm_launch(add_layernorm_kernel<4, false>, grid, dim3(warps * 32), 0, st, x, r, gamma, beta, out, rows, eps, P);
       break;
     case 768:
-      if (f16) add_layernorm_kernel<6, true><<<grid, warps * 32, 0, st>>>(x, r, gamma, beta, out, rows, eps, P);
-      else add_layernorm_kernel<6, false><<<grid, warps * 32, 0, st>>>(x, r, gamma, beta, out, rows, eps, P);
+      if (f16) pm_launch(add_layernorm_kernel<6, true>, grid, dim3(warps * 32), 0, st, x, r, gamma, beta, out, rows, eps, P);
+      else pm_launch(add_layernorm_kernel<6, false>, grid, dim3(warps * 32), 0, st, x, r, gamma, beta, out, rows, eps, P);
       break;
     case 1024:
-      if (f16) add_layernorm_kernel<8, true><<<grid, warps * 32, 0, st>>>(x, r, gamma, beta, out, rows, eps, P);
-      else add_layernorm_kernel<8, false><<<grid, warps * 32, 0, st>>>(x, r, gamma, beta, out, rows, eps, P);
+      if (f16) pm_launch(add_layernorm_kernel<8, true>, grid, dim3(warps * 32), 0, st, x, r, gamma, beta, out, rows, eps, P);
+      else pm_launch(add_layernorm_kernel<8, false>, grid, dim3(warps * 32), 0, st, x, r, gamma, beta, out, rows, eps, P);
       break;
     default: return PM_EUNSUPPORTED;
   }
@@ -309,9 +319,9 @@
   PM_REQUIRE((first != 2 && second != 2) || spk);
   const long long total = (long long)batch * rows * (ch >> 2);
   if (total == 0) return PM_OK;
-  if (f16) add_rows_kernel<true><<<grid_for(total, 256), 256, 0, (cudaStream_t)stream>>>(x, pe, spk, first, second, out,
+  if (f16) pm_launch(add_rows_kernel<true>, grid_for(total, 256), dim3(256), 0, (cudaStream_t)stream, x, pe, spk, first, second, out,
                                                                                   batch, rows, ch, P);
-  else add_rows_kernel<false><<<grid_for(total, 256), 256, 0, (cudaStream_t)stream>>>(x, pe, spk, first, second, out,
+  else pm_launch(add_rows_kernel<false>, grid_for(total, 256), dim3(256), 0, (cudaStream_t)stream, x, pe, spk, first, second, out,
                                                                                batch, rows, ch, P);
   PM_LAUNCH_CHECK();
 }
@@ -332,8 +342,8 @@
   const long long nv = vec ? ch / 4 : 0;
   const int grid = grid_for(rows * (nv + (ch - 4 * nv)), 256);
   cudaStream_t st = (cudaStream_t)stream;
-  if (f16) add2_kernel<true><<<grid, 256, 0, st>>>(a, lda, b, ldb, out, ldo, rows, ch, nv, P);
-  else add2_kernel<false><<<grid, 256, 0, st>>>(a, lda, b, ldb, out, ldo, rows, ch, nv, P);
+  if (f16) pm_launch(add2_kernel<true>, grid, dim3(256), 0, st, a, lda, b, ldb, out, ldo, rows, ch, nv, P);
+  else pm_launch(add2_kernel<false>, grid, dim3(256), 0, st, a, lda, b, ldb, out, ldo, rows, ch, nv, P);
   PM_LAUNCH_CHECK();
 }
 
@@ -348,9 +358,9 @@
   PM_REQUIRE(batch >= 0 && win_len >= 0 && start >= 0 && start + win_len <= total_len && pre >= 0 && ch > 0);
   const long long total = (long long)batch * win_len * ch;
   if (total == 0) return PM_OK;
-  if (f16) window_input_kernel<true><<<grid_for(total, 256), 256, 0, (cudaStream_t)stream>>>(
+  if (f16) pm_launch(window_input_kernel<true>, grid_for(total, 256), dim3(256), 0, (cudaStream_t)stream,
       motion, mask, seed, mask_embedding, out, batch, total_len, start, win_len, pre, ch, seed_bs, P);
-  else window_input_kernel<false><<<grid_for(total, 256), 256, 0, (cudaStream_t)stream>>>(
+  else pm_launch(window_input_kernel<false>, grid_for(total, 256), dim3(256), 0, (cudaStream_t)stream,
       motion, mask, seed, mask_embedding, out, batch, total_len, start, win_len, pre, ch, seed_bs, P);
   PM_LAUNCH_CHECK();
 }
diff --git a/pantomatrix_b200/csrc/pm_misc.cu b/pantomatrix_b200/csrc/pm_misc.cu
--- a/pantomatrix_b200/csrc/pm_misc.cu
+++ b/pantomatrix_b200/csrc/pm_misc.cu
@@ -2,6 +2,14 @@
 #include "../../include/pm_emage.h"
 
 extern "C" int pm_abi_version(void) { return PM_ABI_VERSION; }
+
+int pm_pdl_on = 0;
+
+extern "C" int pm_set_pdl(int on) {
+  PM_REQUIRE(on == 0 || on == 1);
+  pm_pdl_on = on;
+  return PM_OK;
+}
 
 extern "C" int pm_memset_async(void* ptr, int value, long long bytes, void* stream) {
   PM_REQUIRE(ptr && bytes >= 0);
diff --git a/pantomatrix_b200/csrc/pm_pose.cu b/pantomatrix_b200/csrc/pm_pose.cu
--- a/pantomatrix_b200/csrc/pm_pose.cu
+++ b/pantomatrix_b200/csrc/pm_pose.cu
@@ -60,6 +60,8 @@
     const float* __restrict__ face, const float* __restrict__ upper, const float* __restrict__ hands,
     const float* __restrict__ lower, float* __restrict__ expression, float* __restrict__ axis_angle,
     float* __restrict__ motion4inf, long long bt) {
+  pm_grid_wait();
+  pm_grid_launch_dependents();
   const long long total = bt * 64;
   for (long long i = (long long)blockIdx.x * blockDim.x + threadIdx.x; i < total;
        i += (long long)gridDim.x * blockDim.x) {
@@ -97,6 +99,8 @@
 __global__ void __launch_bounds__(64) global_trans_kernel(const float* __restrict__ rec, int ld, int vel_off,
                                                           const float* __restrict__ ref_trans, int ref_bs, float dt,
                                                           float* __restrict__ trans, int t) {
+  pm_grid_wait();
+  pm_grid_launch_dependents();
   const int b = blockIdx.x;
   const float* __restrict__ v = rec + (long long)b * t * ld + vel_off;
   float* __restrict__ o = trans + (long long)b * t * 3;
@@ -219,8 +223,8 @@
   if (bt == 0) return PM_OK;
   long long g = (bt * 64 + 255) / 256;
   if (g > 148 * 16) g = 148 * 16;
-  pose_compose_kernel<<<(unsigned)g, 256, 0, (cudaStream_t)stream>>>(face, upper, hands, lower, expression,
-                                                                    axis_angle, motion4inf, bt);
+  pm_launch(pose_compose_kernel, dim3((unsigned)g), dim3(256), 0, (cudaStream_t)stream, face, upper, hands, lower,
+            expression, axis_angle, motion4inf, bt);
   PM_LAUNCH_CHECK();
 }
 
@@ -228,6 +232,7 @@
                                    float* trans, int batch, int t, void* stream) {
   PM_REQUIRE(rec && ref_trans && trans && batch >= 0 && t >= 0 && ld >= vel_off + 3 && ref_bs >= 0);
   if (batch == 0 || t == 0) return PM_OK;
-  global_trans_kernel<<<batch, 64, 0, (cudaStream_t)stream>>>(rec, ld, vel_off, ref_trans, ref_bs, dt, trans, t);
-  PM_LAUNCH_CHECK();
-}
+  pm_launch(global_trans_kernel, dim3(batch), dim3(64), 0, (cudaStream_t)stream, rec, ld, vel_off, ref_trans, ref_bs, dt,
+            trans, t);
+  PM_LAUNCH_CHECK();
+}
diff --git a/pantomatrix_b200/csrc/pm_tapgemm_tc.cu b/pantomatrix_b200/csrc/pm_tapgemm_tc.cu
--- a/pantomatrix_b200/csrc/pm_tapgemm_tc.cu
+++ b/pantomatrix_b200/csrc/pm_tapgemm_tc.cu
@@ -151,6 +151,21 @@
     }
     if (warp != 0) return;
     const uint32_t tx = (uint32_t)stage_bytes;
+    const int pre = n_iter < p.stages ? n_iter : p.stages;
+    if (elect_one()) {
+      int q = p.rot, tap = 0, kb = 0;
+      for (int it = 0; it < pre; ++it) {
+        const uint32_t bar = smem_u32(&full_bar[it]);
+        mbar_expect_tx(bar, tx);
+        for (int pl = 0; pl < p.nsplit; ++pl)
+          tma_load_3d(smem_u32(tiles + (size_t)q * stage_bytes + p.nsplit * A_TILE_BYTES + pl * W_TILE_BYTES), &map_w, bar,
+                      kb * BK, tap * p.w_rows + n0, pl);
+        if (++q == p.stages) q = 0;
+        if (++kb == p.kblocks) { kb = 0; ++tap; }
+      }
+    }
+    __syncwarp();
+    pm_grid_wait();
     int s = 0, q = p.rot, tap = 0, kb = 0;
     uint32_t ph = 0;
     for (int it = 0; it < n_iter; ++it) {
@@ -158,10 +173,11 @@
       if (elect_one()) {
         const uint32_t bar = smem_u32(&full_bar[s]);
         uint8_t* st = tiles + (size_t)q * stage_bytes;
-        mbar_expect_tx(bar, tx);
+        if (it >= pre) mbar_expect_tx(bar, tx);
         for (int pl = 0; pl < p.nsplit; ++pl) {
           tma_load_4d(smem_u32(st + pl * A_TILE_BYTES), &map_a, bar, kb * BK, l0 + tap - p.pad, b0, pl);
-          tma_load_3d(smem_u32(st + p.nsplit * A_TILE_BYTES + pl * W_TILE_BYTES), &map_w, bar, kb * BK, tap * p.w_rows + n0, pl);
+          if (it >= pre)
+            tma_load_3d(smem_u32(st + p.nsplit * A_TILE_BYTES + pl * W_TILE_BYTES), &map_w, bar, kb * BK, tap * p.w_rows + n0, pl);
         }
       }
       __syncwarp();
@@ -187,6 +203,7 @@
   }
 
   setmaxnreg_inc<CONSUMER_REGS>();
+  pm_grid_wait();
   const int ct = threadIdx.x - PRODUCER_THREADS;
   const int wg = ct >> 7;
   float acc0[NACC], acc1[NACC], accc[NACC];
@@ -296,6 +313,7 @@
       }
     }
     if (warp == STAMP_WARP) PM_STAMP(5);
+    pm_grid_launch_dependents();
     if (ct == 0) bulk_wait_read0();
     if (warp == STAMP_WARP) PM_STAMP(6);
     return;
@@ -372,6 +390,7 @@
     }
   }
   if (warp == STAMP_WARP) PM_STAMP(5);
+  pm_grid_launch_dependents();
 #ifdef PM_TC_TIMING
   named_bar_sync(1, CONSUMER_THREADS);
 #endif
@@ -382,6 +401,8 @@
 __global__ void __launch_bounds__(256) split_bf16_kernel(const float* __restrict__ x, long long x_bs, int ldx, int rows,
                                                          int ch, __nv_bfloat16* __restrict__ out, long long o_ps,
                                                          long long o_bs, int ldo, int nsplit) {
+  pm_grid_wait();
+  pm_grid_launch_dependents();
   const int b = blockIdx.y;
   const float* __restrict__ xb = x + (long long)b * x_bs;
   __nv_bfloat16* __restrict__ ob = out + (long long)b * o_bs;
@@ -433,7 +454,7 @@
     cudaError_t e = cudaFuncSetAttribute(tapgemm_tc_kernel<BN, F16, NSPLIT>, cudaFuncAttributeMaxDynamicSharedMemorySize, 227 * 1024);
     if (e != cudaSuccess) { configured = 0; return (int)e; }
   }
-  tapgemm_tc_kernel<BN, F16, NSPLIT><<<grid, NUM_THREADS, smem, st>>>(ma, mw, mr, mo, mp, p);
+  pm_launch(tapgemm_tc_kernel<BN, F16, NSPLIT>, grid, dim3(NUM_THREADS), smem, st, ma, mw, mr, mo, mp, p);
   PM_LAUNCH_CHECK();
 }
 
@@ -598,11 +619,11 @@
   __nv_bfloat16* o = reinterpret_cast<__nv_bfloat16*>(out);
   cudaStream_t st = (cudaStream_t)stream;
   if (f16) {
-    if (vec) split_bf16_kernel<true, true><<<grid, 256, 0, st>>>(x, x_bs, ldx, rows, ch, o, o_ps, o_bs, ldo, nsplit);
-    else split_bf16_kernel<false, true><<<grid, 256, 0, st>>>(x, x_bs, ldx, rows, ch, o, o_ps, o_bs, ldo, nsplit);
+    if (vec) pm_launch(split_bf16_kernel<true, true>, grid, dim3(256), 0, st, x, x_bs, ldx, rows, ch, o, o_ps, o_bs, ldo, nsplit);
+    else pm_launch(split_bf16_kernel<false, true>, grid, dim3(256), 0, st, x, x_bs, ldx, rows, ch, o, o_ps, o_bs, ldo, nsplit);
   } else {
-    if (vec) split_bf16_kernel<true, false><<<grid, 256, 0, st>>>(x, x_bs, ldx, rows, ch, o, o_ps, o_bs, ldo, nsplit);
-    else split_bf16_kernel<false, false><<<grid, 256, 0, st>>>(x, x_bs, ldx, rows, ch, o, o_ps, o_bs, ldo, nsplit);
+    if (vec) pm_launch(split_bf16_kernel<true, false>, grid, dim3(256), 0, st, x, x_bs, ldx, rows, ch, o, o_ps, o_bs, ldo, nsplit);
+    else pm_launch(split_bf16_kernel<false, false>, grid, dim3(256), 0, st, x, x_bs, ldx, rows, ch, o, o_ps, o_bs, ldo, nsplit);
   }
   PM_LAUNCH_CHECK();
 }
diff --git a/pantomatrix_b200/csrc/pm_vq.cu b/pantomatrix_b200/csrc/pm_vq.cu
--- a/pantomatrix_b200/csrc/pm_vq.cu
+++ b/pantomatrix_b200/csrc/pm_vq.cu
@@ -12,6 +12,8 @@
 __global__ void __launch_bounds__(NT) l2_argmin_kernel(
     const float* __restrict__ z, long long rows, int rows_per_batch, long long z_bs, const float* __restrict__ codebook,
     const float* __restrict__ e2, int n_codes, long long* __restrict__ index) {
+  pm_grid_wait();
+  pm_grid_launch_dependents();
   extern __shared__ float smem[];
   float* Zs = smem;
   float* Es = Zs + RT * EDP;
@@ -104,6 +106,8 @@
 __global__ void __launch_bounds__(256) row_argmax_kernel(const float* __restrict__ x, long long rows, int ch,
                                                          int ldx, int rows_per_batch, long long x_bs,
                                                          long long* __restrict__ index, int* __restrict__ nonfinite) {
+  pm_grid_wait();
+  pm_grid_launch_dependents();
   const int lane = threadIdx.x & 31;
   const long long row = (long long)blockIdx.x * (blockDim.x >> 5) + (threadIdx.x >> 5);
   if (row >= rows) return;
@@ -132,6 +136,8 @@
 __global__ void __launch_bounds__(256) gather_rows_kernel(const float* __restrict__ codebook, long long n_table,
                                                           const long long* __restrict__ index, long long rows,
                                                           int ch4, float* __restrict__ out, PmPlanes P) {
+  pm_grid_wait();
+  pm_grid_launch_dependents();
   const long long total = rows * ch4;
   for (long long i = (long long)blockIdx.x * blockDim.x + threadIdx.x; i < total;
        i += (long long)gridDim.x * blockDim.x) {
@@ -172,7 +178,8 @@
   }
   const long long grid = (rows + RT - 1) / RT;
   PM_REQUIRE(grid <= 0x7fffffffLL);
-  l2_argmin_kernel<<<(unsigned)grid, NT, kL2Smem, (cudaStream_t)stream>>>(z, rows, rows_per_batch, z_bs, codebook, e2, n_codes, index);
+  pm_launch(l2_argmin_kernel, dim3((unsigned)grid), dim3(NT), kL2Smem, (cudaStream_t)stream, z, rows, rows_per_batch, z_bs,
+            codebook, e2, n_codes, index);
   PM_LAUNCH_CHECK();
 }
 
@@ -191,8 +198,8 @@
   if (rows == 0) return PM_OK;
   if (rows_per_batch <= 0 || x_bs == (long long)rows_per_batch * ldx) { rows_per_batch = 0x7fffffff; x_bs = 0; }
   PM_REQUIRE(rows_per_batch == 0x7fffffff || rows < 0x7fffffffLL);
-  row_argmax_kernel<<<(unsigned)((rows + 7) / 8), 256, 0, (cudaStream_t)stream>>>(x, rows, ch, ldx, rows_per_batch, x_bs,
-                                                                                  index, nonfinite);
+  pm_launch(row_argmax_kernel, dim3((unsigned)((rows + 7) / 8)), dim3(256), 0, (cudaStream_t)stream, x, rows, ch, ldx,
+            rows_per_batch, x_bs, index, nonfinite);
   PM_LAUNCH_CHECK();
 }
 
@@ -206,8 +213,8 @@
   if (rows == 0) return PM_OK;
   long long g = (rows * (ch >> 2) + 255) / 256;
   if (g > 148 * 16) g = 148 * 16;
-  if (f16) gather_rows_kernel<true><<<(unsigned)g, 256, 0, (cudaStream_t)stream>>>(codebook, n_table, index, rows, ch >> 2, out, P);
-  else gather_rows_kernel<false><<<(unsigned)g, 256, 0, (cudaStream_t)stream>>>(codebook, n_table, index, rows, ch >> 2, out, P);
+  if (f16) pm_launch(gather_rows_kernel<true>, dim3((unsigned)g), dim3(256), 0, (cudaStream_t)stream, codebook, n_table, index, rows, ch >> 2, out, P);
+  else pm_launch(gather_rows_kernel<false>, dim3((unsigned)g), dim3(256), 0, (cudaStream_t)stream, codebook, n_table, index, rows, ch >> 2, out, P);
   PM_LAUNCH_CHECK();
 }
 
diff --git a/pantomatrix_b200/csrc/pm_vq_tc.cu b/pantomatrix_b200/csrc/pm_vq_tc.cu
--- a/pantomatrix_b200/csrc/pm_vq_tc.cu
+++ b/pantomatrix_b200/csrc/pm_vq_tc.cu
@@ -81,6 +81,8 @@
 __global__ void __launch_bounds__(NTHREADS, 1) l2_argmin_tc_kernel(
     const float* __restrict__ z, long long rows, int rows_per_batch, long long z_bs, const float* __restrict__ codebook,
     const float* __restrict__ e2, long long* __restrict__ index) {
+  pm_grid_wait();
+  pm_grid_launch_dependents();
   auto row_ptr = [&](long long g) -> const float* {
     if (rows_per_batch == 0) return z + g * ED;
     const unsigned gb = (unsigned)g / (unsigned)rows_per_batch, gl = (unsigned)g - gb * (unsigned)rows_per_batch;
@@ -400,7 +402,8 @@
   const long long tiles = (rows + TM - 1) / TM;
   long long grid = tiles < sms ? tiles : sms;
   if (max_ctas > 0 && grid > max_ctas) grid = max_ctas;
-  l2_argmin_tc_kernel<<<(unsigned)grid, NTHREADS, kSmem, (cudaStream_t)stream>>>(z, rows, rows_per_batch, z_bs, codebook, e2, index);
+  pm_launch(l2_argmin_tc_kernel, dim3((unsigned)grid), dim3(NTHREADS), kSmem, (cudaStream_t)stream, z, rows, rows_per_batch,
+            z_bs, codebook, e2, index);
   PM_LAUNCH_CHECK();
 }
 
diff --git a/pantomatrix_b200/ops.py b/pantomatrix_b200/ops.py
--- a/pantomatrix_b200/ops.py
+++ b/pantomatrix_b200/ops.py
@@ -53,6 +53,12 @@
     global launch_count
     launch_count += 1
     _lib.call(name, *args)
+
+
+def set_pdl(on: bool) -> None:
+    global launch_count
+    _call("pm_set_pdl", int(bool(on)))
+    launch_count -= 1
 
 
 def _bs_ld(t: torch.Tensor):
diff --git a/pantomatrix_b200/pipeline.py b/pantomatrix_b200/pipeline.py
--- a/pantomatrix_b200/pipeline.py
+++ b/pantomatrix_b200/pipeline.py
@@ -1,4 +1,6 @@
 from __future__ import annotations
+
+import os
 
 import torch
 
@@ -88,8 +90,13 @@
         self.graph = torch.cuda.CUDAGraph()
         before = ops.launch_count
         self.capture_stream = torch.cuda.Stream(device=dev, priority=-1) if body_priority else None
-        with torch.cuda.graph(self.graph, stream=self.capture_stream):
-            self.latent, self.pred, self.nonfinite = step()
+        self.pdl = os.environ.get("PM_PDL", "1") != "0"
+        ops.set_pdl(self.pdl)
+        try:
+            with torch.cuda.graph(self.graph, stream=self.capture_stream):
+                self.latent, self.pred, self.nonfinite = step()
+        finally:
+            ops.set_pdl(False)
         self.kernels_per_replay = ops.launch_count - before
 
     @torch.no_grad()
```
